# avianphysics/avian

Measured on NVIDIA H100. Metric: physics steps/sec on 100k-cube stack (broad phase + solver stage per step), higher is better.
Workload: dtype f32

## Files before the change

### avian_b200/_build.py

```python
from __future__ import annotations

import os
import shutil
import subprocess
from pathlib import Path

ROOT = Path(__file__).resolve().parent
REPO = ROOT.parent
LIB_DIR = ROOT / "lib"
CUDA_LIB = LIB_DIR / "libavian_b200.so"
HOST_LIB = LIB_DIR / "libavian_host.so"

CUDA_SOURCES = ["abi.cu", "comm.cu", "solver_host.cu", "broadphase.cu", "aabb.cu", "narrow.cu", "contacts.cu", "queries.cu", "ccd.cu"]
CUDA_HEADERS = ["avn_math.cuh", "solver_dev.cuh", "joints_dev.cuh", "solver_kernels.cuh", "context.hpp", "joint_schedule.hpp", "broadphase_cells.cuh", "narrow_math.hpp", "contact_rows.hpp", "query_math.hpp", "ccd_math.hpp", "move_math.hpp"]
GENCODE = ["-gencode", "arch=compute_90a,code=sm_90a"]
NVCC_FLAGS = [
    *GENCODE, "-lineinfo", "-O3", "-std=c++17", "-fmad=false",
    "-Xcompiler", "-fPIC", "-shared",
]
HOST_SOURCES = ["host_api.cpp"]
HOST_FLAGS = ["-O2", "-std=c++17", "-fPIC", "-shared", "-ffp-contract=off", "-Wall"]


def _newer(target: Path, deps: list[Path]) -> bool:
    if not target.exists():
        return False
    t = target.stat().st_mtime
    return all(d.stat().st_mtime <= t for d in deps if d.exists())


def find_nvcc() -> str | None:
    for cand in (os.environ.get("NVCC"), shutil.which("nvcc"), "/usr/local/cuda/bin/nvcc"):
        if cand and Path(cand).exists():
            return cand
    return None


_UNIT_HEADERS = {
    "comm.cu": ["context.hpp"],
    "aabb.cu": ["avn_math.cuh", "context.hpp"],
    "broadphase.cu": ["avn_math.cuh", "context.hpp", "broadphase_cells.cuh", "device_prims.cuh"],
    "narrow.cu": ["avn_math.cuh", "context.hpp", "narrow_math.hpp"],
    "contacts.cu": ["avn_math.cuh", "context.hpp", "narrow_math.hpp", "contact_rows.hpp", "device_prims.cuh"],
    "queries.cu": ["context.hpp", "narrow_math.hpp", "query_math.hpp", "move_math.hpp", "device_prims.cuh"],
    "ccd.cu": ["avn_math.cuh", "context.hpp", "narrow_math.hpp", "query_math.hpp", "ccd_math.hpp", "device_prims.cuh"],
}


def build_cuda(force: bool = False, verbose: bool = False) -> Path:
    src = ROOT / "csrc"
    header = REPO / "include" / "avian_b200.h"
    all_headers = sorted(p.name for p in src.glob("*.cuh")) + sorted(p.name for p in src.glob("*.hpp"))
    deps = [src / s for s in CUDA_SOURCES] + [src / h for h in all_headers] + [header]
    if not force and _newer(CUDA_LIB, deps):
        return CUDA_LIB
    nvcc = find_nvcc()
    if nvcc is None:
        if CUDA_LIB.exists():
            return CUDA_LIB
        raise RuntimeError("nvcc not found and no prebuilt libavian_b200.so: the CUDA path cannot be built")
    LIB_DIR.mkdir(exist_ok=True)
    obj_dir = LIB_DIR / "obj"
    obj_dir.mkdir(exist_ok=True)
    compile_flags = [f for f in NVCC_FLAGS if f != "-shared"]
    jobs = []
    for unit in CUDA_SOURCES:
        obj = obj_dir / (unit + ".o")
        unit_deps = [src / unit, header, Path(__file__)] + [src / h for h in _UNIT_HEADERS.get(unit, all_headers)]
        if force or not _newer(obj, unit_deps):
            jobs.append((unit, [nvcc, *compile_flags, *(["-Xptxas", "-v"] if verbose else []), "-c", "-o", str(obj), str(src / unit)]))
    if jobs:
        from concurrent.futures import ThreadPoolExecutor
        with ThreadPoolExecutor(max_workers=min(len(jobs), os.cpu_count() or 2)) as pool:
            results = list(pool.map(lambda j: (j[0], subprocess.run(j[1], cwd=src, capture_output=True, text=True)), jobs))
        for unit, r in results:
            if verbose or r.returncode != 0:
                print(f"---- {unit}\n{r.stdout}{r.stderr}")
            if r.returncode != 0:
                raise RuntimeError(f"nvcc failed on {unit}")
    subprocess.run([nvcc, "-shared", *GENCODE, "-o", str(CUDA_LIB), *[str(obj_dir / (u + ".o")) for u in CUDA_SOURCES], "-ldl"],
                   check=True, cwd=src)
    return CUDA_LIB


def build_variant(name: str, defines: list[str]) -> Path:
    build_cuda()
    nvcc = find_nvcc()
    src, obj_dir = ROOT / "csrc", LIB_DIR / "obj"
    obj = obj_dir / f"solver_host.{name}.o"
    flags = [f for f in NVCC_FLAGS if f != "-shared"]
    subprocess.run([nvcc, *flags, *[f"-D{d}" for d in defines], "-c", "-o", str(obj), str(src / "solver_host.cu")], check=True, cwd=src)
    out = LIB_DIR / f"libavian_b200_{name}.so"
    objs = [str(obj if u == "solver_host.cu" else obj_dir / (u + ".o")) for u in CUDA_SOURCES]
    subprocess.run([nvcc, "-shared", *GENCODE, "-o", str(out), *objs, "-ldl"], check=True, cwd=src)
    return out


def build_host(force: bool = False) -> Path:
    src = ROOT / "host"
    deps = [p for p in src.glob("*.[ch]pp")] + [REPO / "include" / "avian_b200.h", ROOT / "csrc" / "narrow_math.hpp", ROOT / "csrc" / "contact_rows.hpp",
            ROOT / "csrc" / "query_math.hpp", ROOT / "csrc" / "ccd_math.hpp", ROOT / "csrc" / "move_math.hpp"]
    if not force and _newer(HOST_LIB, deps):
        return HOST_LIB
    cxx = os.environ.get("CXX") or shutil.which("g++")
    if cxx is None:
        if HOST_LIB.exists():
            return HOST_LIB
        raise RuntimeError("g++ not found and no prebuilt libavian_host.so")
    LIB_DIR.mkdir(exist_ok=True)
    subprocess.run([cxx, *HOST_FLAGS, "-o", str(HOST_LIB), *[str(src / s) for s in HOST_SOURCES]], check=True, cwd=src)
    return HOST_LIB


def build_oracle(force: bool = False) -> Path:
    odir = REPO / "oracle"
    target = odir / "_build" / "liboracle.so"
    if force and target.exists():
        target.unlink()
    if shutil.which("make") and (shutil.which("g++") or os.environ.get("CXX")):
        subprocess.run(["make", "-s"], check=True, cwd=odir)
    if not target.exists():
        raise RuntimeError("oracle/_build/liboracle.so missing and cannot be built")
    return target


# ... 5 lines not shown
```

### avian_b200/csrc/broadphase.cu

```cuda
#include <algorithm>
#include <cmath>
#include <cstdlib>
#include <cstring>
#include <vector>

#include "avn_math.cuh"
#include "context.hpp"

#include "device_prims.cuh"

namespace avn {
namespace {

template <class S> struct KeyOf;
template <> struct KeyOf<float> { using type = uint32_t; static constexpr int passes = 4; };
template <> struct KeyOf<double> { using type = uint64_t; static constexpr int passes = 8; };

__device__ __forceinline__ uint32_t sortable(float f) {
    uint32_t b = __float_as_uint(f);
    if (b == 0x80000000u) b = 0;
    return (b & 0x80000000u) ? ~b : (b | 0x80000000u);
}
__device__ __forceinline__ uint64_t sortable(double f) {
    uint64_t b = (uint64_t)__double_as_longlong(f);
    if (b == 0x8000000000000000ull) b = 0;
    return (b & 0x8000000000000000ull) ? ~b : (b | 0x8000000000000000ull);
}

template <class S>
__global__ void make_keys(const S* __restrict__ aabb_min, const S* __restrict__ aabb_max, int n, typename KeyOf<S>::type* __restrict__ keys,
                          uint32_t* __restrict__ vals, unsigned long long* __restrict__ nonfinite) {
    int i = blockIdx.x * blockDim.x + threadIdx.x;
    if (i < n) {
        const S a = aabb_min[3 * i], b = aabb_min[3 * i + 1], c = aabb_min[3 * i + 2], d = aabb_max[3 * i], e = aabb_max[3 * i + 1], f = aabb_max[3 * i + 2];
        const S z = (a - a) + (b - b) + (c - c) + (d - d) + (e - e) + (f - f);
        if (!(z == S(0))) *nonfinite = 1ull;
        keys[i] = sortable(a);
        vals[i] = uint32_t(i);
    }
}

template <class S>
struct Sweep {
    int n;
    const S* minx; const S* maxx;
    const Vec4<S>* yz;
    const uint4* meta;
    const uint8_t* flags;
    const int* end;
    const uint8_t* is_wide;
    const uint64_t* existing; uint64_t existing_mask;
    const uint64_t* jdis; uint64_t jdis_mask;
};

template <class S>
__global__ void gather_sorted(const uint32_t* __restrict__ order, int n, const S* __restrict__ mn, const S* __restrict__ mx,
                              const uint32_t* __restrict__ collider, const uint32_t* __restrict__ body, const uint32_t* __restrict__ memberships,
                              const uint32_t* __restrict__ filters, const uint8_t* __restrict__ flags, S* __restrict__ minx, S* __restrict__ maxx,
                              Vec4<S>* __restrict__ yz, uint4* __restrict__ meta, uint8_t* __restrict__ sflags) {
    int r = blockIdx.x * blockDim.x + threadIdx.x;
    if (r >= n) return;
    uint32_t p = order[r];
    minx[r] = mn[3 * p];
    maxx[r] = mx[3 * p];
    yz[r] = mk4<S>(mn[3 * p + 1], mx[3 * p + 1], mn[3 * p + 2], mx[3 * p + 2]);
    meta[r] = make_uint4(collider[p], body[p], memberships ? memberships[p] : 1u, filters ? filters[p] : 0xFFFFFFFFu);
    sflags[r] = flags ? flags[p] : uint8_t(AVN_AABB_GENERATE_CONSTRAINTS);
}

constexpr int SW_WIDE = 4096;
constexpr int SW_WIDE_CAP = 1 << 14;
template <class S> struct CellGrid;
template <class S> __device__ __forceinline__ long long query_cell_count(const CellGrid<S>& g, Vec4<S> yi);
template <class S>
__global__ void sweep_bounds(const S* __restrict__ minx, const S* __restrict__ maxx, const Vec4<S>* __restrict__ yz, const CellGrid<S>* __restrict__ grid,
                             int n, int* __restrict__ end, int* __restrict__ wide_list, int* __restrict__ wide_count, uint8_t* __restrict__ is_wide,
                             const uint8_t* __restrict__ sflags) {
    int i = blockIdx.x * blockDim.x + threadIdx.x;
    if (i >= n) return;
    if (sflags[i] & AVN_AABB_HALO) {
        end[i] = i + 1;
        is_wide[i] = 0;
        return;
    }
    S m = maxx[i];
    int lo = i + 1, hi = n;
    while (lo < hi) {
        int mid = (lo + hi) >> 1;
        if (minx[mid] > m) hi = mid; else lo = mid + 1;
    }
    end[i] = lo;
    uint8_t wide = 0;
    if (lo - i - 1 > SW_WIDE && query_cell_count(*grid, yz[i]) > 32) {
        int slot = atomicAdd(wide_count, 1);
        if (slot < SW_WIDE_CAP) { wide_list[slot] = i; wide = 1; }
    }
    is_wide[i] = wide;
}

__device__ __forceinline__ uint64_t pair_key(uint32_t a, uint32_t b) {
    return a < b ? (uint64_t(a) << 32) | b : (uint64_t(b) << 32) | a;
}

template <class S>
__device__ __forceinline__ bool pair_filters(const Sweep<S>& s, uint4 mi, uint32_t fi, int j, uint32_t& pair_flags, uint4& mj) {
    mj = s.meta[j];
    uint32_t fj = s.flags[j];
    bool interacts = (mi.z & mj.w) != 0 && (mj.z & mi.w) != 0;
    if ((fi & fj & AVN_AABB_IS_INACTIVE) || !interacts || mi.y == mj.y) return false;
    if ((fj & AVN_AABB_NOT_J) || ((fi & AVN_AABB_SPLIT_I) && (fj & AVN_AABB_HALO))) return false;
    if (s.existing && hash_contains(s.existing, s.existing_mask, pair_key(mi.x, mj.x))) return false;
    if (s.jdis && hash_contains(s.jdis, s.jdis_mask, pair_key(mi.y, mj.y))) return false;
    uint32_t u = fi | fj;
    pair_flags = ((u & AVN_AABB_CONTACT_EVENTS) ? AVN_PAIR_CONTACT_EVENTS : 0u) | ((u & AVN_AABB_MODIFY_CONTACTS) ? AVN_PAIR_MODIFY_CONTACTS : 0u) |
                 ((u & AVN_AABB_GENERATE_CONSTRAINTS) ? AVN_PAIR_GENERATE_CONSTRAINTS : 0u) | ((u & AVN_AABB_CUSTOM_FILTER) ? AVN_PAIR_NEEDS_HOOK : 0u);
    return true;
}

constexpr int SW_THREADS = 256, SW_WARPS = SW_THREADS / 32;

// ... 161 lines not shown
    const uint32_t* d_collider_ = nullptr; const uint32_t* d_body_ = nullptr; const uint32_t* d_memb_ = nullptr; const uint32_t* d_filt_ = nullptr;
    const uint8_t* d_flags_ = nullptr;
    const uint64_t* d_existing_ = nullptr; uint64_t existing_mask_ = 0;
    const uint64_t* d_jdis_ = nullptr; uint64_t jdis_mask_ = 0;
    DevBuf b_min_, b_max_, b_col_, b_body_, b_memb_, b_filt_, b_flags_, b_exk_, b_ext_, b_jdk_, b_jdt_;
    DevBuf k0_, k1_, v0_, v1_, hist_;
    DevBuf s_minx_, s_maxx_, s_yz_, s_meta_, s_flags_, s_end_, counts_, offsets_, block_sums_, wide_, wide_sub_, wide_flag_, grid_, ck0_, ck1_, cv0_, cv1_, cbounds_, pairs_, stats_, stats2_;
    DevBuf o_c1_, o_c2_, o_b1_, o_b2_, o_fl_;
    uint32_t* d_order_ = nullptr;
};

template <class S>
AvnStatus Broadphase<S>::build_set(DevBuf& keys_buf, DevBuf& table_buf, const uint64_t* host_keys, uint64_t count, const uint64_t** table, uint64_t* mask) {
    *table = nullptr;
    *mask = 0;
    if (!host_keys || count == 0) return AVN_OK;
    uint64_t cap = 64;
    while (cap < count * 2) cap <<= 1;
    const uint64_t* dkeys;
    AvnStatus st = up<uint64_t>(keys_buf, host_keys, count, &dkeys);
    if (st != AVN_OK) return st;
    AVN_CUDA(table_buf.ensure(cap * sizeof(uint64_t)));
    AVN_CUDA(cudaMemsetAsync(table_buf.p, 0, cap * sizeof(uint64_t), stream_));
    hash_insert<<<unsigned((count + 255) / 256), 256, 0, stream_>>>(dkeys, count, table_buf.as<uint64_t>(), cap - 1);
    ++launches_;
    *table = table_buf.as<uint64_t>();
    *mask = cap - 1;
    return AVN_OK;
}

template <class S>
AvnStatus Broadphase<S>::upload(AvnAabbColumns* a) {
    if (!a) return err_->fail(AVN_ERR_INVALID_ARGUMENT, "aabbs is required");
    if (a->count && (!a->collider || !a->body || !a->aabb_min || !a->aabb_max))
        return err_->fail(AVN_ERR_INVALID_ARGUMENT, "aabbs: collider, body, aabb_min and aabb_max are required");
    a->retained_count = a->count;
    if (a->count > 0x7fffffffu - RS_TILE) return err_->fail(AVN_ERR_INVALID_ARGUMENT, "aabbs: too many intervals");
    uploaded_ = ran_ = false;
    launches_ = 0;
    upload_launches_ = 0;
    dropped_ = false;
    n_ = int(a->count);
    host_ = *a;
    caller_ = a;
    const size_t n = a->count;
    AvnStatus st;
#define UPB(buf, host, cnt, T, dst) if ((st = up<T>(buf, host, cnt, &dst)) != AVN_OK) return st
    UPB(b_min_, a->aabb_min, 3 * n, S, d_min_);
    UPB(b_max_, a->aabb_max, 3 * n, S, d_max_);
    UPB(b_col_, a->collider, n, uint32_t, d_collider_);
    UPB(b_body_, a->body, n, uint32_t, d_body_);
    UPB(b_memb_, a->memberships, n, uint32_t, d_memb_);
    UPB(b_filt_, a->filters, n, uint32_t, d_filt_);
    UPB(b_flags_, a->flags, n, uint8_t, d_flags_);
#undef UPB
    if ((st = build_set(b_exk_, b_ext_, a->existing_pairs, a->existing_pair_count, &d_existing_, &existing_mask_)) != AVN_OK) return st;
    if (!d_existing_ && ext_existing_) { d_existing_ = ext_existing_; existing_mask_ = ext_existing_mask_; }
    if ((st = build_set(b_jdk_, b_jdt_, a->joint_disabled_body_pairs, a->joint_disabled_pair_count, &d_jdis_, &jdis_mask_)) != AVN_OK) return st;
    upload_launches_ = launches_;
    uploaded_ = true;
    return AVN_OK;
}

template <class S>
AvnStatus Broadphase<S>::ensure_buffers(int n) {
    const int nblocks = (n + RS_TILE - 1) / RS_TILE;
    AVN_CUDA(k0_.ensure(size_t(n) * sizeof(K))); AVN_CUDA(k1_.ensure(size_t(n) * sizeof(K)));
    AVN_CUDA(v0_.ensure(size_t(n) * 4)); AVN_CUDA(v1_.ensure(size_t(n) * 4));
    AVN_CUDA(hist_.ensure(size_t(256) * nblocks * 4));
    AVN_CUDA(s_minx_.ensure(size_t(n) * sizeof(S))); AVN_CUDA(s_maxx_.ensure(size_t(n) * sizeof(S)));
    AVN_CUDA(s_yz_.ensure(size_t(n) * sizeof(Vec4<S>))); AVN_CUDA(s_meta_.ensure(size_t(n) * sizeof(uint4)));
    AVN_CUDA(s_flags_.ensure(size_t(n))); AVN_CUDA(s_end_.ensure(size_t(n) * 4));
    AVN_CUDA(counts_.ensure(size_t(n) * 4)); AVN_CUDA(offsets_.ensure((size_t(n) + 1) * 8));
    AVN_CUDA(grid_.ensure(sizeof(CellGrid<S>)));
    AVN_CUDA(ck0_.ensure(size_t(n) * 4)); AVN_CUDA(ck1_.ensure(size_t(n) * 4)); AVN_CUDA(cv0_.ensure(size_t(n) * 4)); AVN_CUDA(cv1_.ensure(size_t(n) * 4));
    AVN_CUDA(cbounds_.ensure(size_t(2) * 0x10000 * 4));
    AVN_CUDA(stats_.ensure(size_t(YZ_BLOCKS) * sizeof(YzPartial<S>)));
    AVN_CUDA(stats2_.ensure(size_t(2) * YZ_BLOCKS * sizeof(S)));
    AVN_CUDA(wide_.ensure((size_t(SW_WIDE_CAP) + 1) * 4));
    AVN_CUDA(wide_flag_.ensure(size_t(n)));
    const int nsub = (n + SW_SUB - 1) / SW_SUB;
    AVN_CUDA(wide_sub_.ensure(size_t(nsub) * size_t(std::min(n, SW_WIDE_CAP)) * 4));
    AVN_CUDA(block_sums_.ensure(size_t((n + 1023) / 1024) * 8));
    AVN_CUDA(nf_flag_.ensure(8));
    pair_capacity_ = std::max<uint64_t>(pair_capacity_, uint64_t(4) * uint64_t(n) + 1024);
    AVN_CUDA(o_c1_.ensure(pair_capacity_ * 4)); AVN_CUDA(o_c2_.ensure(pair_capacity_ * 4)); AVN_CUDA(o_b1_.ensure(pair_capacity_ * 4)); AVN_CUDA(o_b2_.ensure(pair_capacity_ * 4));
    AVN_CUDA(o_fl_.ensure(pair_capacity_));
    AVN_CUDA(pairs_.ensure(pair_capacity_ * sizeof(uint2)));
    return AVN_OK;
}

template <class S>
typename Broadphase<S>::GraphKey Broadphase<S>::graph_key() const {
    GraphKey k;
    k.n = n_;
    const void* ptrs[] = {d_min_, d_max_, d_collider_, d_body_, d_memb_, d_filt_, d_flags_, d_existing_, d_jdis_, k0_.p, k1_.p, v0_.p, v1_.p, hist_.p,
                          s_minx_.p, s_maxx_.p, s_yz_.p, s_meta_.p, s_flags_.p, s_end_.p, counts_.p, offsets_.p, grid_.p, ck0_.p};
    static_assert(sizeof ptrs == sizeof k.p, "graph key size");
    memcpy(k.p, ptrs, sizeof ptrs);
    k.m[0] = existing_mask_ ^ (uint64_t(uintptr_t(cv0_.p)) << 1) ^ (uint64_t(uintptr_t(wide_sub_.p)) << 2);
    k.m[0] ^= (pair_capacity_ * 0x9e3779b97f4a7c15ull) ^ (uint64_t(uintptr_t(pairs_.p)) << 3) ^ (uint64_t(uintptr_t(o_c1_.p)) << 4) ^ (uint64_t(uintptr_t(o_fl_.p)) << 5);
    k.m[1] = jdis_mask_ ^ (uint64_t(uintptr_t(cbounds_.p)) << 1) ^ (uint64_t(uintptr_t(block_sums_.p)) << 2) ^ (uint64_t(uintptr_t(wide_flag_.p)) << 3);
    return k;
}

template <class S>
void Broadphase<S>::enqueue_front(int n) {
    const int nblocks = (n + RS_TILE - 1) / RS_TILE;
    uint32_t launches = 0;
    K* ka = k0_.as<K>(); K* kb = k1_.as<K>();
    uint32_t* va = v0_.as<uint32_t>(); uint32_t* vb = v1_.as<uint32_t>();
    cudaMemsetAsync(nf_flag_.p, 0, 8, stream_);
    make_keys<S><<<(n + 255) / 256, 256, 0, stream_>>>(d_min_, d_max_, n, ka, va, nf_flag_.as<unsigned long long>());
    ++launches;
    for (int pass = 0; pass < KeyOf<S>::passes; ++pass) {
        const int shift = 8 * pass;
        rs_histogram<K><<<nblocks, RS_THREADS, 0, stream_>>>(ka, n, shift, hist_.as<uint32_t>(), nblocks);
        if (nblocks <= RS_FUSE_MAX_BLOCKS) {
            rs_scatter<K, true><<<nblocks, RS_THREADS, 0, stream_>>>(ka, va, n, shift, hist_.as<uint32_t>(), nblocks, kb, vb);
        } else {
            rs_scan<<<1, 1024, 0, stream_>>>(hist_.as<uint32_t>(), 256 * nblocks);
            rs_scatter<K, false><<<nblocks, RS_THREADS, 0, stream_>>>(ka, va, n, shift, hist_.as<uint32_t>(), nblocks, kb, vb);
        }
        launches += nblocks <= RS_FUSE_MAX_BLOCKS ? 2 : 3;
        std::swap(ka, kb);
        std::swap(va, vb);
    }
    d_order_ = va;
    gather_sorted<S><<<(n + 255) / 256, 256, 0, stream_>>>(d_order_, n, d_min_, d_max_, d_collider_, d_body_, d_memb_, d_filt_, d_flags_,
                                                           s_minx_.as<S>(), s_maxx_.as<S>(), s_yz_.as<Vec4<S>>(), s_meta_.as<uint4>(),
                                                           s_flags_.as<uint8_t>());
    CellGrid<S>* d_grid = grid_.as<CellGrid<S>>();
    int* cstart = cbounds_.as<int>();
    int* cend = cbounds_.as<int>() + 0x10000;
    yz_stats<S><<<YZ_BLOCKS, 256, 0, stream_>>>(s_yz_.as<Vec4<S>>(), n, stats_.as<YzPartial<S>>());
    yz_fold<S><<<1, 32, 0, stream_>>>(stats_.as<YzPartial<S>>(), YZ_BLOCKS, n, d_grid);
    yz_small_max<S><<<YZ_BLOCKS, 256, 0, stream_>>>(s_yz_.as<Vec4<S>>(), n, d_grid, stats2_.as<S>());
    yz_grid<S><<<1, 32, 0, stream_>>>(stats_.as<YzPartial<S>>(), stats2_.as<S>(), YZ_BLOCKS, n, d_grid);
    int* wide_count = wide_.as<int>();
    int* wide_list = wide_.as<int>() + 1;
    cudaMemsetAsync(wide_count, 0, 4, stream_);
    sweep_bounds<S><<<(n + 255) / 256, 256, 0, stream_>>>(s_minx_.as<S>(), s_maxx_.as<S>(), s_yz_.as<Vec4<S>>(), d_grid, n, s_end_.as<int>(), wide_list, wide_count,
                                                          wide_flag_.as<uint8_t>(), s_flags_.as<uint8_t>());
    const Sweep<S> sw = sweep_desc();
    cell_keys<S><<<(n + 255) / 256, 256, 0, stream_>>>(s_yz_.as<Vec4<S>>(), n, d_grid, ck0_.as<uint32_t>(), cv0_.as<uint32_t>());
    {
        uint32_t* cka = ck0_.as<uint32_t>(); uint32_t* ckb = ck1_.as<uint32_t>();
        uint32_t* cva = cv0_.as<uint32_t>(); uint32_t* cvb = cv1_.as<uint32_t>();
        for (int pass = 0; pass < 2; ++pass) {
            rs_histogram<uint32_t><<<nblocks, RS_THREADS, 0, stream_>>>(cka, n, 8 * pass, hist_.as<uint32_t>(), nblocks);
            if (nblocks <= RS_FUSE_MAX_BLOCKS) {
                rs_scatter<uint32_t, true><<<nblocks, RS_THREADS, 0, stream_>>>(cka, cva, n, 8 * pass, hist_.as<uint32_t>(), nblocks, ckb, cvb);
            } else {
                rs_scan<<<1, 1024, 0, stream_>>>(hist_.as<uint32_t>(), 256 * nblocks);
                rs_scatter<uint32_t, false><<<nblocks, RS_THREADS, 0, stream_>>>(cka, cva, n, 8 * pass, hist_.as<uint32_t>(), nblocks, ckb, cvb);
            }
            std::swap(cka, ckb);
            std::swap(cva, cvb);
        }
    }
    cudaMemsetAsync(cstart, 0x7f, size_t(0x10000) * 4, stream_);
    cudaMemsetAsync(cend, 0, size_t(0x10000) * 4, stream_);
    cell_bounds<<<(n + 255) / 256, 256, 0, stream_>>>(ck0_.as<uint32_t>(), n, cstart, cend);
    const CellSweep<S> cs = cell_desc();
    const int grid = std::min((n + (256 / CG_GROUP) - 1) / (256 / CG_GROUP), sm_count_ * 32);
    sweep_cells_kernel<S, false><<<grid, 256, 0, stream_>>>(sw, cs, counts_.as<uint32_t>(), nullptr, nullptr);
    const int nsub = (n + SW_SUB - 1) / SW_SUB;
    sweep_wide_kernel<S, false><<<dim3(nsub, WIDE_ROWS), SW_THREADS, 0, stream_>>>(sw, wide_list, wide_count, wide_sub_.as<uint32_t>(), nsub, nullptr, nullptr, 0);
    wide_finish<<<1, 256, 0, stream_>>>(wide_list, wide_count, wide_sub_.as<uint32_t>(), nsub, counts_.as<uint32_t>());
    launches += nblocks <= RS_FUSE_MAX_BLOCKS ? 15 : 17;
    const int sblocks = (n + 1023) / 1024;
    scan_block_sums<<<sblocks, 1024, 0, stream_>>>(counts_.as<uint32_t>(), n, block_sums_.as<uint64_t>());
    scan_block_offsets<<<1, 1024, 0, stream_>>>(block_sums_.as<uint64_t>(), sblocks, offsets_.as<uint64_t>() + n);
    scan_apply<<<sblocks, 1024, 0, stream_>>>(counts_.as<uint32_t>(), n, block_sums_.as<uint64_t>(), offsets_.as<uint64_t>());
    launches += 3;
    {
        uint2* pairs = pairs_.as<uint2>();
        sweep_cells_kernel<S, true><<<grid, 256, 0, stream_>>>(sw, cs, nullptr, offsets_.as<uint64_t>(), pairs);
        sweep_wide_kernel<S, true><<<dim3(nsub, WIDE_ROWS), SW_THREADS, 0, stream_>>>(sw, wide_list, wide_count, wide_sub_.as<uint32_t>(), nsub,
                                                                                      offsets_.as<uint64_t>(), pairs, pair_capacity_);
        segment_sort<<<(n + 255) / 256, 256, 0, stream_>>>(offsets_.as<uint64_t>(), wide_flag_.as<uint8_t>(), n, pairs, pair_capacity_);
        const unsigned mblocks = unsigned(std::min<uint64_t>((pair_capacity_ + 255) / 256, uint64_t(sm_count_) * 16));
        materialize_pairs<S><<<mblocks, 256, 0, stream_>>>(sw, pairs, offsets_.as<uint64_t>() + n, pair_capacity_, o_c1_.as<uint32_t>(), o_c2_.as<uint32_t>(),
                                                           o_b1_.as<uint32_t>(), o_b2_.as<uint32_t>(), o_fl_.as<uint8_t>());
        launches += 4;
    }
    cudaMemcpyAsync(h_total_, offsets_.as<uint64_t>() + n, sizeof(uint64_t), cudaMemcpyDeviceToHost, stream_);
    cudaMemcpyAsync(h_total_ + 1, nf_flag_.p, sizeof(uint64_t), cudaMemcpyDeviceToHost, stream_);
    front_launches_ = launches;
}

template <class S>
AvnStatus Broadphase<S>::run() {
    if (!uploaded_) return err_->fail(AVN_ERR_INVALID_ARGUMENT, "avn_broadphase_run before avn_broadphase_upload");
    const int n = n_;
    launches_ = upload_launches_;
    cudaEventRecord(ev0_, stream_);
    h_total_[0] = 0;
    h_total_[1] = 0;
    if (n > 0) {
        AvnStatus st = ensure_buffers(n);
        if (st != AVN_OK) return st;
        if (use_graph_) {
            const GraphKey key = graph_key();
            if (!graph_exec_ || !(key == graph_key_)) {
// ... 164 lines not shown
```

### avian_b200/csrc/ccd_math.hpp

```cpp
#pragma once
#include <cmath>
#include <cstdint>

#include "query_math.hpp"

namespace ccd {

using nm::S;
using nm::V3;
using nm::Q;

constexpr int CCD_MAX_ITERATIONS = 64;
constexpr double CCD_EPS_PER_LENGTH_UNIT = 1e-4;
constexpr int MODE_LINEAR = 0, MODE_NON_LINEAR = 1;

NM_HD inline void ccd_sincos(double x, double& s, double& c) {
    const double PIO2_1 = 1.57079632673412561417e+00, PIO2_1T = 6.07710050650619224932e-11, INV_PIO2 = 6.36619772367581382433e-01;
    const double k = rint(x * INV_PIO2);
    const double r = (x - k * PIO2_1) - k * PIO2_1T;
    const double r2 = r * r;
    double ps = 1.0 / 355687428096000.0;
    ps = ps * r2 - 1.0 / 1307674368000.0;
    ps = ps * r2 + 1.0 / 6227020800.0;
    ps = ps * r2 - 1.0 / 39916800.0;
    ps = ps * r2 + 1.0 / 362880.0;
    ps = ps * r2 - 1.0 / 5040.0;
    ps = ps * r2 + 1.0 / 120.0;
    ps = ps * r2 - 1.0 / 6.0;
    const double sr = r + r * (r2 * ps);
    double pc = 1.0 / 6402373705728000.0;
    pc = pc * r2 - 1.0 / 20922789888000.0;
    pc = pc * r2 + 1.0 / 87178291200.0;
    pc = pc * r2 - 1.0 / 479001600.0;
    pc = pc * r2 + 1.0 / 3628800.0;
    pc = pc * r2 - 1.0 / 40320.0;
    pc = pc * r2 + 1.0 / 720.0;
    pc = pc * r2 - 1.0 / 24.0;
    pc = pc * r2 + 0.5;
    const double cr = 1.0 - r2 * pc;
    const long long q = ((static_cast<long long>(k) % 4) + 4) % 4;
    if (q == 0) { s = sr; c = cr; }
    else if (q == 1) { s = cr; c = -sr; }
    else if (q == 2) { s = -sr; c = -cr; }
    else { s = -cr; c = sr; }
}

template <class T> struct V3T { T x, y, z; };
template <class T> struct QT { T x, y, z, w; };
template <class T> NM_HD inline T dot3(V3T<T> a, V3T<T> b) { return (a.x * b.x + a.y * b.y) + a.z * b.z; }
template <class T> NM_HD inline V3T<T> sub3(V3T<T> a, V3T<T> b) { return {a.x - b.x, a.y - b.y, a.z - b.z}; }
template <class T> NM_HD inline V3T<T> scale3(V3T<T> a, T s) { return {a.x * s, a.y * s, a.z * s}; }

template <class T> NM_HD inline QT<T> from_scaled_axis(V3T<T> v) {
    const T l = static_cast<T>(sqrt(static_cast<double>(dot3(v, v))));
    if (l == T(0)) return {T(0), T(0), T(0), T(1)};
    const V3T<T> a{v.x / l, v.y / l, v.z / l};
    double s, c;
    ccd_sincos(static_cast<double>(l * T(0.5)), s, c);
    const T ts = static_cast<T>(s), tc = static_cast<T>(c);
    return {a.x * ts, a.y * ts, a.z * ts, tc};
}
NM_HD inline QT<float> qmul(QT<float> a, QT<float> b) {
    return {(a.w * b.x + a.x * b.w) + (a.y * b.z - a.z * b.y), (a.w * b.y - a.x * b.z) + (a.y * b.w + a.z * b.x),
            (a.w * b.z + a.x * b.y) + (a.z * b.w - a.y * b.x), (a.w * b.w - a.x * b.x) + (-(a.y * b.y) - a.z * b.z)};
}
NM_HD inline QT<double> qmul(QT<double> a, QT<double> b) {
    return {a.w * b.x + a.x * b.w + a.y * b.z - a.z * b.y, a.w * b.y - a.x * b.z + a.y * b.w + a.z * b.x,
            a.w * b.z + a.x * b.y - a.y * b.x + a.z * b.w, a.w * b.w - a.x * b.x - a.y * b.y - a.z * b.z};
}

struct Motion {
    int shape;
    V3 he;
    V3 p;
    Q q;
    V3 lc;
    V3 v, w;
};

NM_HD inline S motion_radius(const Motion& m) {
    if (m.shape == nm::SHAPE_SPHERE) return nm::len(m.lc) + m.he.x;
    const V3 e{fabs(m.lc.x) + m.he.x, fabs(m.lc.y) + m.he.y, fabs(m.lc.z) + m.he.z};
    return nm::len(e);
}

NM_HD inline void pose_at(const Motion& m, S t, V3& origin, nm::M3& r) {
    const QT<double> dq = from_scaled_axis<double>({m.w.x * t, m.w.y * t, m.w.z * t});
    const QT<double> q = qmul(dq, QT<double>{m.q.x, m.q.y, m.q.z, m.q.w});
    const Q qt{q.x, q.y, q.z, q.w};
    const V3 com = (m.p + nm::rot(m.q, m.lc)) + m.v * t;
    origin = com - nm::rot(qt, m.lc);
    r = qm::rot_mat(qt);
}

NM_COLD inline S shape_distance(int sa, V3 ha, V3 ca, const nm::M3& ra, int sb, V3 hb, V3 cb, const nm::M3& rb, V3& n) {
    n = V3{0, 1, 0};
    if (sa == nm::SHAPE_SPHERE && sb == nm::SHAPE_SPHERE) {
        const V3 e = cb - ca;
        const S l = nm::len(e);
        if (l > 0) n = e * (1 / l);
        return nm::smax(l - ha.x - hb.x, 0);
    }
    if (sa == nm::SHAPE_SPHERE || sb == nm::SHAPE_SPHERE) {
        const bool box_a = sb == nm::SHAPE_SPHERE;
        const nm::Box box = box_a ? nm::Box{ca, ra, ha} : nm::Box{cb, rb, hb};
        const V3 centre = box_a ? cb : ca;
        const S r = box_a ? hb.x : ha.x;
        V3 on;
        const S l = sqrt(nm::box_point_closest(box, centre, on));
        if (l > 0) n = (box_a ? centre - on : on - centre) * (1 / l);
        return nm::smax(l - r, 0);
    }
    const V3 s = cb - ca;
    bool separated = false;
NM_ROLLED
    for (int k = 0; k < 15 && !separated; ++k) {
        const V3 L = qm::sat_axis(ra, rb, k);
        if (qm::is_zero3(L)) continue;
        separated = fabs(nm::dot(L, s)) > qm::box_extent(ra, ha, L) + qm::box_extent(rb, hb, L);
    }
    if (!separated) return 0;
    V3 on_a, on_b;
    const S l = nm::box_box_closest(nm::Box{ca, ra, ha}, nm::Box{cb, rb, hb}, on_a, on_b);
    if (l > 0) n = (on_b - on_a) * (1 / l);
    return l;
}

NM_HD inline bool nonlinear_toi(const Motion& A, const Motion& B, S t_max, S eps, S& toi, int* iterations = nullptr) {
    const V3 rel = B.v - A.v;
    const S spin = nm::len(A.w) * motion_radius(A) + nm::len(B.w) * motion_radius(B);
    S t = 0;
NM_ROLLED
    for (int it = 0; it < CCD_MAX_ITERATIONS; ++it) {
        V3 ca, cb, n;
        nm::M3 ra, rb;
        pose_at(A, t, ca, ra);
        pose_at(B, t, cb, rb);
        const S d = shape_distance(A.shape, A.he, ca, ra, B.shape, B.he, cb, rb, n);
        if (iterations) *iterations = it + 1;
        if (d != d) return false;
        if (d <= eps) { toi = t; return true; }
        const S mu = nm::smax(0, -nm::dot(rel, n)) + spin;
        if (!(mu > 0)) return false;
        t = t + d / mu;
        if (!(t <= t_max)) return false;
    }
    toi = t;
    return true;
}

NM_HD inline bool linear_toi(const Motion& A, const Motion& B, S t_max, S& toi) {
    int axis;
    return qm::cast_toi(A.shape, A.he, A.p, A.q, A.v - B.v, t_max, B.shape, B.he, B.p, B.q, toi, axis);
}

template <class T> NM_HD inline T pair_toi(int mode, const Motion& A, const Motion& B, T dt, S eps, S prediction_distance) {
    S t = 0;
    const bool hit = mode == MODE_LINEAR ? linear_toi(A, B, S(dt), t) : nonlinear_toi(A, B, S(dt), eps, t);
    if (!hit) return T(-1);
    const T tt = static_cast<T>(t);
    if (tt != T(0)) return tt;
    Motion ball = B;
    ball.shape = nm::SHAPE_SPHERE;
    ball.he = V3{prediction_distance, 0, 0};
    const bool hit2 = mode == MODE_LINEAR ? linear_toi(A, ball, S(dt), t) : nonlinear_toi(A, ball, S(dt), eps, t);
    return hit2 ? static_cast<T>(t) : T(-1);
}

template <class T> NM_HD inline bool below_thresholds(V3T<T> v1, V3T<T> w1, V3T<T> v2, V3T<T> w2, T linear_threshold, T angular_threshold) {
    const V3T<T> dw = sub3(w1, w2), dv = sub3(v1, v2);
    return dot3(dw, dw) < angular_threshold * angular_threshold && dot3(dv, dv) < linear_threshold * linear_threshold;
}

template <class T> NM_HD inline T overshoot(T min_toi) { return min_toi * T(1.0001); }

template <class T> NM_HD inline void apply_record(T m, V3T<T> v, V3T<T> w, V3T<T>& dp, QT<T>& dq) {
    dp = V3T<T>{m * v.x, m * v.y, m * v.z};
    dq = qmul(from_scaled_axis<T>(V3T<T>{w.x * m, w.y * m, w.z * m}), dq);
// ... 4 lines not shown
```

### avian_b200/csrc/contact_rows.hpp

```cpp
#pragma once
#include <cstdint>

#include "narrow_math.hpp"

namespace avn {

template <class S>
struct EdgeRows {
    int E;
    uint32_t* c1; uint32_t* c2; uint32_t* b1; uint32_t* b2; uint8_t* live;
    uint8_t* count; uint8_t* disjoint; S* normal; S* a1; S* a2; S* pen; S* ns;
    uint8_t* prev_count; double* prev_a1; double* prev_a2;
    S* ws_n_in; S* ws_t_in; S* ws_n_out; S* ws_t_out; S* nimp_in; S* nimp_out;
    const uint8_t* asleep;
};

template <class S>
struct NarrowEdgeArgs {
    EdgeRows<S> r;
    const uint8_t* shape; const S* dims; const S* pos; const S* rot; const S* lv; const S* av; const S* amin; const S* amax;
    double dt, tol, thr2;
    int match;
};

template <class S> NM_HD inline nm::V3 ldd3(const S* p, size_t i) { return {double(p[3 * i]), double(p[3 * i + 1]), double(p[3 * i + 2])}; }
template <class S> NM_HD inline void std3(S* p, size_t i, nm::V3 v) { p[3 * i] = S(v.x); p[3 * i + 1] = S(v.y); p[3 * i + 2] = S(v.z); }

template <class S>
struct BodyFrameCols { const S* pos; const S* rot; const S* com; };

template <class S>
NM_HD inline nm::PairFrames pair_frames(const BodyFrameCols<S>& f, uint32_t ba, nm::V3 pa, uint32_t bb, nm::V3 pb) {
    nm::PairFrames fr;
    fr.offset1 = pa - ldd3(f.pos, ba);
    fr.offset2 = pb - ldd3(f.pos, bb);
    fr.com1 = nm::V3{0, 0, 0};
    fr.com2 = nm::V3{0, 0, 0};
    if (f.com) {
        const nm::Q q1{double(f.rot[4 * size_t(ba)]), double(f.rot[4 * size_t(ba) + 1]), double(f.rot[4 * size_t(ba) + 2]), double(f.rot[4 * size_t(ba) + 3])};
        const nm::Q q2{double(f.rot[4 * size_t(bb)]), double(f.rot[4 * size_t(bb) + 1]), double(f.rot[4 * size_t(bb) + 2]), double(f.rot[4 * size_t(bb) + 3])};
        fr.com1 = nm::rot(q1, ldd3(f.com, ba));
        fr.com2 = nm::rot(q2, ldd3(f.com, bb));
    }
    return fr;
}

template <class S>
NM_HD inline bool capsule_row(const NarrowEdgeArgs<S>& a, int e) {
    return a.shape && a.r.live[e] && (a.shape[a.r.c1[e]] == nm::SHAPE_CAPSULE || a.shape[a.r.c2[e]] == nm::SHAPE_CAPSULE);
}

template <class S, bool CAPSULES = true, bool FRAMES = false>
NM_HD inline void narrow_edge_row(const NarrowEdgeArgs<S>& a, int e, const BodyFrameCols<S>& f = BodyFrameCols<S>{}) {
    const EdgeRows<S>& r = a.r;
    if (r.asleep && r.asleep[e]) return;
    if (!r.live[e]) { r.count[e] = 0; r.disjoint[e] = 0; return; }
    const uint32_t ca = r.c1[e], cb = r.c2[e], ba = r.b1[e], bb = r.b2[e];
    int np = 0;
    nm::V3 normal{0, 0, 0};
    nm::PointOut out[4];
    bool disjoint = false;
    {
        const nm::V3 mina = ldd3(a.amin, ca), maxa = ldd3(a.amax, ca), minb = ldd3(a.amin, cb), maxb = ldd3(a.amax, cb);
        disjoint = (mina.x > maxb.x || maxa.x < minb.x || mina.y > maxb.y || maxa.y < minb.y || mina.z > maxb.z || maxa.z < minb.z);
    }
    r.disjoint[e] = disjoint ? 1 : 0;
    if (!disjoint) {
        const nm::V3 pa = ldd3(a.pos, ca), pb = ldd3(a.pos, cb);
        const nm::Q qa{double(a.rot[4 * size_t(ca)]), double(a.rot[4 * size_t(ca) + 1]), double(a.rot[4 * size_t(ca) + 2]), double(a.rot[4 * size_t(ca) + 3])};
        const nm::Q qb{double(a.rot[4 * size_t(cb)]), double(a.rot[4 * size_t(cb) + 1]), double(a.rot[4 * size_t(cb) + 2]), double(a.rot[4 * size_t(cb) + 3])};
        const nm::V3 v1 = ldd3(a.lv, ba), v2 = ldd3(a.lv, bb), w1 = ldd3(a.av, ba), w2 = ldd3(a.av, bb);
        const nm::V3 rel = v2 - v1;
        const double eff_margin = a.dt * nm::len(rel);
        const double max_dist = nm::smax(eff_margin, a.tol);
        nm::Contacts pts;
        const int ta = a.shape ? a.shape[ca] : nm::SHAPE_CUBOID, tb = a.shape ? a.shape[cb] : nm::SHAPE_CUBOID;
        if (nm::collide<CAPSULES>(ta, ldd3(a.dims, ca), pa, qa, tb, ldd3(a.dims, cb), pb, qb, max_dist, normal, pts)) {
            if (FRAMES) np = nm::manifold_points(pts, normal, pa, pb, rel, w1, w2, a.dt, eff_margin, pair_frames(f, ba, pa, bb, pb), out);
            else np = nm::manifold_points(pts, normal, pa, pb, rel, w1, w2, a.dt, eff_margin, out);
        } else
            normal = nm::V3{0, 0, 0};
    }
    const int oc = r.prev_count[e];
    nm::V3 oa1[4], oa2[4];
    S on[4], otx[4], oty[4];
    for (int k = 0; k < oc; ++k) {
        const size_t q = size_t(e) * 4 + k;
        oa1[k] = nm::V3{r.prev_a1[3 * q], r.prev_a1[3 * q + 1], r.prev_a1[3 * q + 2]};
        oa2[k] = nm::V3{r.prev_a2[3 * q], r.prev_a2[3 * q + 1], r.prev_a2[3 * q + 2]};
        on[k] = r.ws_n_out[q]; otx[k] = r.ws_t_out[2 * q]; oty[k] = r.ws_t_out[2 * q + 1];
    }
    r.count[e] = uint8_t(np);
    std3(r.normal, size_t(e), normal);
    for (int k = 0; k < 4; ++k) {
        const size_t q = size_t(e) * 4 + k;
        S vn = S(0), vx = S(0), vy = S(0);
        if (k < np) {
            const int j = a.match ? nm::match_point(out[k].anchor1, out[k].anchor2, oa1, oa2, oc, a.thr2) : -1;
            if (j >= 0) { vn = on[j]; vx = otx[j]; vy = oty[j]; }
            std3(r.a1, q, out[k].anchor1);
            std3(r.a2, q, out[k].anchor2);
            r.pen[q] = S(out[k].penetration);
            r.ns[q] = S(out[k].normal_speed);
            r.prev_a1[3 * q] = out[k].anchor1.x; r.prev_a1[3 * q + 1] = out[k].anchor1.y; r.prev_a1[3 * q + 2] = out[k].anchor1.z;
            r.prev_a2[3 * q] = out[k].anchor2.x; r.prev_a2[3 * q + 1] = out[k].anchor2.y; r.prev_a2[3 * q + 2] = out[k].anchor2.z;
        } else {
            std3(r.a1, q, nm::V3{0, 0, 0});
            std3(r.a2, q, nm::V3{0, 0, 0});
            r.pen[q] = S(0);
            r.ns[q] = S(0);
        }
        r.ws_n_in[q] = vn;
        r.ws_t_in[2 * q] = vx;
        r.ws_t_in[2 * q + 1] = vy;
        r.ws_n_out[q] = vn;
        r.ws_t_out[2 * q] = vx;
        r.ws_t_out[2 * q + 1] = vy;
    }
    r.prev_count[e] = uint8_t(np);
}


}
```

### avian_b200/csrc/contacts.cu

```cuda
#include <cooperative_groups.h>

#include <algorithm>
#include <cstdlib>
#include <cstring>

#include "context.hpp"
#include "contact_rows.hpp"
#include "device_prims.cuh"

namespace avn {
namespace {
namespace cg = cooperative_groups;

enum { CH_NONE = 0, CH_PUSH = 1, CH_POP = 2, CH_REMOVE = 3, CH_MASK = 3, CH_DONE = 0x10 };
enum { ISL_NONE = 0, ISL_ADD = 1, ISL_REMOVE = 2 };

struct GraphCounters {
    uint32_t removed, started, stopped, changed, rounds, ovf_dirty, manifolds, any_restitution, aborted, bad_pairs;
    uint32_t rows_woken, rows_slept, bodies_asleep;
    uint32_t round_left[3];
    uint32_t color_offsets[AVN_GRAPH_COLOR_COUNT + 1];
    uint32_t ovf_count;
    uint32_t rows_asleep;
};
// ... 282 lines not shown
        if (S(re) != S(0)) g.ctr->any_restitution = 1;
    }
}

__global__ void pair_set_kernel(GraphRows g, uint64_t* __restrict__ table, uint64_t mask) {
    const int e = blockIdx.x * blockDim.x + threadIdx.x;
    if (e >= g.hw || !g.live[e]) return;
    const uint32_t a = g.c1[e], b = g.c2[e];
    const uint64_t k = (a < b ? (uint64_t(a) << 32) | b : (uint64_t(b) << 32) | a) + 1;
    uint64_t h = hash64(k) & mask;
    for (;;) {
        unsigned long long prev = atomicCAS((unsigned long long*)&table[h], 0ull, (unsigned long long)k);
        if (prev == 0ull || prev == k) return;
        h = (h + 1) & mask;
    }
}

__global__ void event_keys_kernel(const uint8_t* __restrict__ event, int n, uint32_t* __restrict__ keys, uint32_t* __restrict__ vals) {
    const int e = blockIdx.x * blockDim.x + threadIdx.x;
    if (e >= n) return;
    const uint8_t v = event[e];
    keys[e] = (v & EV_STARTED) ? 0u : (v & EV_ENDED) ? 1u : 2u;
    vals[e] = uint32_t(e);
}
__global__ void report_keys_kernel(GraphRows g, uint32_t flags, uint32_t* __restrict__ keys, uint32_t* __restrict__ vals) {
    const int e = blockIdx.x * blockDim.x + threadIdx.x;
    if (e >= g.hw) return;
    const bool sel = g.live[e] && g.touching[e] && (!(flags & AVN_REPORT_EVENTS_ONLY) || (g.pflags[e] & AVN_PAIR_CONTACT_EVENTS));
    keys[e] = sel ? 0u : 1u;
    vals[e] = uint32_t(e);
}
__global__ void key_bounds_kernel(const uint32_t* __restrict__ sorted_keys, int n, int nb, uint32_t* __restrict__ out) {
    const int k = threadIdx.x + 1;
    if (k > nb) return;
    int lo = 0, hi = n;
    while (lo < hi) { const int mid = (lo + hi) >> 1; if (sorted_keys[mid] < uint32_t(k)) lo = mid + 1; else hi = mid; }
    out[k - 1] = uint32_t(lo);
}
__global__ void event_gather_kernel(GraphRows g, const uint32_t* __restrict__ list, uint32_t n_started, uint32_t n, uint32_t skip, uint32_t N,
                                    uint32_t* __restrict__ out) {
    const uint32_t i = blockIdx.x * blockDim.x + threadIdx.x;
    if (i >= n) return;
    const uint32_t e = list[i], j = i < n_started ? i : i + skip;
    out[j] = g.c1[e]; out[N + j] = g.c2[e]; out[2 * size_t(N) + j] = g.b1[e]; out[3 * size_t(N) + j] = g.b2[e];
    reinterpret_cast<uint8_t*>(out + 4 * size_t(N))[j] = g.event[e] & EV_FLAGS;
}
__global__ void mark_colliders_kernel(const uint32_t* __restrict__ ids, uint32_t n, uint8_t* __restrict__ removed) {
    const uint32_t k = blockIdx.x * blockDim.x + threadIdx.x;
    if (k < n) removed[ids[k]] = 1;
}
__global__ void queue_ends_kernel(GraphRows g, const uint32_t* __restrict__ list, uint32_t n, uint32_t base, uint32_t cap, uint32_t* __restrict__ pend) {
    const uint32_t i = blockIdx.x * blockDim.x + threadIdx.x;
    if (i >= n) return;
    const uint32_t e = list[i], j = base + i;
    pend[j] = g.c1[e]; pend[cap + j] = g.c2[e]; pend[2 * size_t(cap) + j] = g.b1[e]; pend[3 * size_t(cap) + j] = g.b2[e];
    reinterpret_cast<uint8_t*>(pend + 4 * size_t(cap))[j] = g.pflags[e] & EV_FLAGS;
}
template <class S>
__global__ void report_gather_kernel(GraphRows g, const uint32_t* __restrict__ list, uint32_t n, const S* __restrict__ normal, const S* __restrict__ pen,
                                     const S* __restrict__ nimp, void* __restrict__ out) {
    const uint32_t i = blockIdx.x * blockDim.x + threadIdx.x;
    if (i >= n) return;
    const uint32_t e = list[i];
    S* os = static_cast<S*>(out);
    uint32_t* ou = reinterpret_cast<uint32_t*>(os + 6 * size_t(n));
    uint8_t* ob = reinterpret_cast<uint8_t*>(ou + 5 * size_t(n));
    const int cnt = g.count[e];
    const bool solved = g.colour[e] != 0 || g.asleep[e] != 0;
    S total = S(0), mx = S(0), deep = S(0);
    for (int k = 0; k < cnt; ++k) {
        const S v = solved ? nimp[4 * size_t(e) + k] : S(0);
        total = total + v;
        if (v > mx) mx = v;
        const S p = pen[4 * size_t(e) + k];
        if (k == 0 || p >= deep) deep = p;
    }
    for (int c = 0; c < 3; ++c) os[3 * size_t(i) + c] = normal[3 * size_t(e) + c];
    os[3 * size_t(n) + i] = total; os[4 * size_t(n) + i] = mx; os[5 * size_t(n) + i] = deep;
    ou[i] = e; ou[n + i] = g.c1[e]; ou[2 * size_t(n) + i] = g.c2[e]; ou[3 * size_t(n) + i] = g.b1[e]; ou[4 * size_t(n) + i] = g.b2[e];
    ob[i] = g.pflags[e] & EV_FLAGS; ob[n + i] = uint8_t(cnt);
}

template <class S>
__global__ void __launch_bounds__(128) narrow_edges_kernel(const __grid_constant__ NarrowEdgeArgs<S> a, uint8_t* fresh, int only_fresh, int capsules) {
    const int e = blockIdx.x * blockDim.x + threadIdx.x;
    if (e >= a.r.E) return;
    if (capsules && capsule_row(a, e)) return;
    if (only_fresh) {
        if (!fresh[e]) return;
        fresh[e] = 0;
    }
    narrow_edge_row<S, false>(a, e);
}

template <class S>
__global__ void __launch_bounds__(128) narrow_capsule_edges_kernel(const __grid_constant__ NarrowEdgeArgs<S> a, uint8_t* fresh, int only_fresh) {
    const int e = blockIdx.x * blockDim.x + threadIdx.x;
    if (e >= a.r.E || !capsule_row(a, e)) return;
    if (only_fresh) {
        if (!fresh[e]) return;
        fresh[e] = 0;
    }
    narrow_edge_row<S, true>(a, e);
}

template <class S, bool CAPSULES>
__global__ void __launch_bounds__(128) narrow_framed_edges_kernel(const __grid_constant__ NarrowEdgeArgs<S> a, const BodyFrameCols<S> f, uint8_t* fresh,
                                                                  int only_fresh, int capsules) {
    const int e = blockIdx.x * blockDim.x + threadIdx.x;
    if (e >= a.r.E) return;
    if (capsules && capsule_row(a, e) != CAPSULES) return;
    if (only_fresh) {
        if (!fresh[e]) return;
        fresh[e] = 0;
    }
    narrow_edge_row<S, CAPSULES, true>(a, e, f);
}


struct IslandCounters {
    uint32_t islands, sleeping, put_to_sleep, woken, split_bodies, merges, split_root;
    uint32_t absorbed;
    unsigned long long cand;
};
constexpr uint32_t ISL_NONE_BODY = 0xffffffffu;

struct IslandState {
    int B;
    const uint8_t* kind;
    uint32_t* parent; uint32_t* root; uint32_t* root_prev; uint32_t* removed;
    uint8_t* isl_sleeping; uint8_t* awake; uint8_t* need_wake; uint8_t* touched; uint8_t* in_split;
    float* timer;
    const float* thr_lin; const float* thr_ang; const uint8_t* disabled; const uint8_t* host_wake;
    uint32_t* cand_body;
    IslandCounters* ctr;
    float time_to_sleep, delta_secs;
};
__device__ __forceinline__ bool isl_static(const IslandState& s, uint32_t b) { return b >= uint32_t(s.B) || s.kind[b] == AVN_BODY_STATIC; }
__device__ __forceinline__ uint32_t isl_find(uint32_t* parent, uint32_t x) {
    uint32_t p = *reinterpret_cast<volatile uint32_t*>(&parent[x]);
    while (p != x) {
        const uint32_t gp = *reinterpret_cast<volatile uint32_t*>(&parent[p]);
        if (gp != p) parent[x] = gp;
        x = p; p = gp;
    }
    return x;
}
__device__ __forceinline__ bool isl_union(uint32_t* parent, uint32_t u, uint32_t v) {
    for (;;) {
        uint32_t ru = isl_find(parent, u), rv = isl_find(parent, v);
        if (ru == rv) return false;
        if (ru < rv) { const uint32_t t = ru; ru = rv; rv = t; }
        if (atomicCAS(&parent[ru], ru, rv) == ru) return true;
    }
}
__global__ void isl_init_kernel(IslandState s) {
    const int b = blockIdx.x * blockDim.x + threadIdx.x;
    if (b >= s.B) return;
    s.parent[b] = uint32_t(b); s.root[b] = uint32_t(b); s.root_prev[b] = uint32_t(b); s.removed[b] = 0;
    s.isl_sleeping[b] = 0; s.awake[b] = 0; s.need_wake[b] = 0; s.touched[b] = 0; s.in_split[b] = 0; s.timer[b] = 0.f;
    if (b == 0) { *s.cand_body = ISL_NONE_BODY; }
}
__global__ void isl_joint_kernel(IslandState s, const uint32_t* __restrict__ j1, const uint32_t* __restrict__ j2, int J, int only_split) {
    const int j = blockIdx.x * blockDim.x + threadIdx.x;
    if (j >= J) return;
    const uint32_t a = j1[j], b = j2[j];
    if (isl_static(s, a) || isl_static(s, b)) return;
    if (only_split && !(s.in_split[a] && s.in_split[b])) return;
    isl_union(s.parent, a, b);
}
__global__ void isl_link_existing_kernel(IslandState s, GraphRows g) {
    const int e = blockIdx.x * blockDim.x + threadIdx.x;
    if (e >= g.hw || !g.live[e] || !g.touching[e] || !(g.pflags[e] & AVN_PAIR_GENERATE_CONSTRAINTS)) return;
    const uint32_t a = g.b1[e], b = g.b2[e];
    if (!isl_static(s, a) && !isl_static(s, b)) isl_union(s.parent, a, b);
}
__global__ void isl_add_kernel(IslandState s, GraphRows g) {
    const int e = blockIdx.x * blockDim.x + threadIdx.x;
    if (e >= g.hw || g.isl_event[e] != ISL_ADD) return;
    const uint32_t a = g.b1[e], b = g.b2[e];
    const bool sa = isl_static(s, a), sb = isl_static(s, b);
    if (!sa) s.touched[a] = 1;
    if (!sb) s.touched[b] = 1;
    if (!sa && !sb && isl_union(s.parent, a, b)) atomicAdd(&s.ctr->merges, 1u);
}
__global__ void isl_flatten_kernel(IslandState s, int split_only) {
    const int b = blockIdx.x * blockDim.x + threadIdx.x;
    if (b >= s.B || isl_static(s, uint32_t(b))) return;
    if (split_only) {
        if (!s.in_split[b]) return;
        s.root[b] = isl_find(s.parent, uint32_t(b));
        s.removed[b] = 0;
        return;
    }
    const uint32_t r = isl_find(s.parent, uint32_t(b));
    s.root[b] = r;
    if (s.root_prev[b] == uint32_t(b) && r != uint32_t(b)) {
        if (s.removed[b]) { atomicAdd(&s.removed[r], s.removed[b]); s.removed[b] = 0; }
        if (s.isl_sleeping[b]) { s.isl_sleeping[b] = 0; s.need_wake[r] = 1; s.touched[b] = 1; atomicAdd(&s.ctr->absorbed, 1u); }
// ... 742 lines not shown
                      {&prev_a2_, 12 * sizeof(double)}, {&ws_n_in_, 4 * sizeof(S)}, {&ws_t_in_, 8 * sizeof(S)}, {&ws_n_out_, 4 * sizeof(S)},
                      {&ws_t_out_, 8 * sizeof(S)}, {&nimp_in_, 4 * sizeof(S)}, {&nimp_out_, 4 * sizeof(S)},
                      {&pflags_, 1}, {&touching_, 1}, {&colour_, 1}, {&change_, 1}, {&old_colour_, 1}, {&ovf_pos_, 4}, {&ovf_, 4}, {&isl_event_, 1}, {&fresh_, 1},
                      {&event_, 1}, {&asleep_, 1}};
        for (Col& c : cols) {
            void* fresh = nullptr;
            AVN_CUDA(cudaMalloc(&fresh, n * c.bytes_per_row));
            AVN_CUDA(cudaMemsetAsync(fresh, 0, n * c.bytes_per_row, stream_));
            if (c.buf->p && E_) AVN_CUDA(cudaMemcpyAsync(fresh, c.buf->p, size_t(E_) * c.bytes_per_row, cudaMemcpyDeviceToDevice, stream_));
            AVN_CUDA(cudaStreamSynchronize(stream_));
            if (c.buf->p) cudaFree(c.buf->p);
            c.buf->p = fresh;
            c.buf->cap = n * c.bytes_per_row;
        }
        E_ = capacity;
        const size_t nblocks = (n + RS_TILE - 1) / RS_TILE;
        AVN_CUDA(k0_.ensure(n * 4)); AVN_CUDA(k1_.ensure(n * 4)); AVN_CUDA(v0_.ensure(n * 4)); AVN_CUDA(v1_.ensure(n * 4)); AVN_CUDA(list_.ensure(n * 4));
        AVN_CUDA(evl_.ensure(n * 4));
        AVN_CUDA(hist_.ensure(256 * nblocks * 4));
        AVN_CUDA(m_b1_.ensure(n * 4)); AVN_CUDA(m_b2_.ensure(n * 4)); AVN_CUDA(m_fr_.ensure(n * sizeof(S))); AVN_CUDA(m_re_.ensure(n * sizeof(S)));
        uint64_t cap = 1024;
        while (cap < uint64_t(n) * 2) cap <<= 1;
        AVN_CUDA(table_.ensure(cap * sizeof(uint64_t)));
        table_mask_ = cap - 1;
        table_dirty_ = true;
        return AVN_OK;
    }
    AvnStatus upload_inputs(const AvnNarrowInput* in, bool keep_shapes, cudaStream_t s) {
        const size_t C = in->collider_count, B = in->body_count;
        if (!in->dims || !in->position || !in->rotation || !in->linear_velocity || !in->angular_velocity || !in->aabb_min || !in->aabb_max)
            return err_->fail(AVN_ERR_INVALID_ARGUMENT, "contacts_step: dims, position, rotation, velocities and AABBs are required");
        keep_shapes = keep_shapes && in_.colliders == C && in_.dims != nullptr;
        AvnStatus st;
        up_stream_ = s;
#define UPC(buf, host, cnt, T, dst) if ((st = up<T>(buf, host, cnt, &dst)) != AVN_OK) { up_stream_ = stream_; return st; }
        if (!keep_shapes) {
            UPC(i_shape_, in->shape, C, uint8_t, in_.shape);
            UPC(i_dims_, in->dims, 3 * C, S, in_.dims);
            if (checked_ == in) has_capsule_ = checked_capsule_;
        }
        UPC(i_pos_, in->position, 3 * C, S, in_.pos);
        UPC(i_rot_, in->rotation, 4 * C, S, in_.rot);
        UPC(i_lv_, in->linear_velocity, 3 * B, S, in_.lv);
        UPC(i_av_, in->angular_velocity, 3 * B, S, in_.av);
        UPC(i_amin_, in->aabb_min, 3 * C, S, in_.amin);
        UPC(i_amax_, in->aabb_max, 3 * C, S, in_.amax);
        in_.framed = frames_set_;
        if (frames_set_) {
            UPC(i_fpos_, frames_.position.data(), 3 * B, S, in_.frames.pos);
            UPC(i_frot_, frames_.rotation.data(), 4 * B, S, in_.frames.rot);
            UPC(i_fcom_, frames_.com.empty() ? nullptr : frames_.com.data(), 3 * B, S, in_.frames.com);
        }
#undef UPC
        up_stream_ = stream_;
        in_.colliders = C;
        return AVN_OK;
    }
    AvnStatus launch_narrow(const AvnNarrowParams* prm, const AvnNarrowInput* in, uint32_t match_contacts, double length_unit, uint32_t n) {
        bool only_fresh = false;
        if (prefetched_ == in) {
            AVN_CUDA(cudaStreamWaitEvent(stream_, ev_in_, 0));
            only_fresh = early_rows_ > 0;
            if (only_fresh && n == early_rows_ && !added_this_step_) { prefetched_ = nullptr; early_rows_ = 0; return AVN_OK; }
        } else {
            if (prefetched_) AVN_CUDA(cudaStreamWaitEvent(stream_, ev_in_, 0));
            AvnStatus st = upload_inputs(in, false, stream_);
            if (st != AVN_OK) return st;
        }
        prefetched_ = nullptr;
        early_rows_ = 0;
        AvnStatus st = enqueue_narrow(prm, match_contacts, length_unit, n, stream_, only_fresh);
        if (st == AVN_OK && !only_fresh && n) AVN_CUDA(cudaMemsetAsync(fresh_.p, 0, n, stream_));
        return st;
    }
    AvnStatus enqueue_narrow(const AvnNarrowParams* prm, uint32_t match_contacts, double length_unit, uint32_t n, cudaStream_t s, bool only_fresh) {
        NarrowEdgeArgs<S> a{};
        a.r = rows();
        a.r.E = int(n);
        a.shape = in_.shape; a.dims = in_.dims; a.pos = in_.pos; a.rot = in_.rot; a.lv = in_.lv; a.av = in_.av; a.amin = in_.amin; a.amax = in_.amax;
        a.dt = prm->dt;
        a.tol = prm->contact_tolerance;
        a.thr2 = (0.1 * length_unit) * (0.1 * length_unit);
        a.match = match_contacts ? 1 : 0;
        if (in_.framed) {
            narrow_framed_edges_kernel<S, false><<<(n + 127) / 128, 128, 0, s>>>(a, in_.frames, fresh_.as<uint8_t>(), only_fresh ? 1 : 0, has_capsule_ ? 1 : 0);
            if (has_capsule_) narrow_framed_edges_kernel<S, true><<<(n + 127) / 128, 128, 0, s>>>(a, in_.frames, fresh_.as<uint8_t>(), only_fresh ? 1 : 0, 1);
        } else {
            narrow_edges_kernel<S><<<(n + 127) / 128, 128, 0, s>>>(a, fresh_.as<uint8_t>(), only_fresh ? 1 : 0, has_capsule_ ? 1 : 0);
            if (has_capsule_) narrow_capsule_edges_kernel<S><<<(n + 127) / 128, 128, 0, s>>>(a, fresh_.as<uint8_t>(), only_fresh ? 1 : 0);
        }
        AVN_CUDA(cudaGetLastError());
        return AVN_OK;
    }
    void radix_pass(int n, uint32_t* vals_out = nullptr) {
        uint32_t* vo = vals_out ? vals_out : v1_.as<uint32_t>();
        const int nblocks = (n + RS_TILE - 1) / RS_TILE;
        rs_histogram<uint32_t><<<nblocks, RS_THREADS, 0, stream_>>>(k0_.as<uint32_t>(), n, 0, hist_.as<uint32_t>(), nblocks);
        if (nblocks <= RS_FUSE_MAX_BLOCKS) {
            rs_scatter<uint32_t, true><<<nblocks, RS_THREADS, 0, stream_>>>(k0_.as<uint32_t>(), v0_.as<uint32_t>(), n, 0, hist_.as<uint32_t>(), nblocks, k1_.as<uint32_t>(), vo);
        } else {
            rs_scan<<<1, 1024, 0, stream_>>>(hist_.as<uint32_t>(), 256 * nblocks);
            rs_scatter<uint32_t, false><<<nblocks, RS_THREADS, 0, stream_>>>(k0_.as<uint32_t>(), v0_.as<uint32_t>(), n, 0, hist_.as<uint32_t>(), nblocks, k1_.as<uint32_t>(), vo);
        }
    }
    AvnStatus small_bounds(int nb, uint32_t* out) {
        AVN_CUDA(bounds_.ensure(16));
        key_bounds_kernel<<<1, 32, 0, stream_>>>(k1_.as<uint32_t>(), int(hw_), nb, bounds_.as<uint32_t>());
        AVN_CUDA(cudaGetLastError());
        AVN_CUDA(cudaMemcpyAsync(out, bounds_.p, size_t(nb) * 4, cudaMemcpyDeviceToHost, stream_));
        AVN_CUDA(cudaStreamSynchronize(stream_));
        return AVN_OK;
    }
    AvnStatus pend_reserve(int i, uint32_t need) {
        if (need <= pend_cap_[i]) return AVN_OK;
        const uint32_t cap = std::max(need, std::max(2 * pend_cap_[i], 256u)), old = pend_cap_[i];
        void* p = nullptr;
        AVN_CUDA(cudaMalloc(&p, size_t(cap) * 17));
        if (pend_n_[i]) {
            const uint32_t* src = pend_[i].as<uint32_t>();
            uint32_t* dst = static_cast<uint32_t*>(p);
            for (int c = 0; c < 4; ++c)
                AVN_CUDA(cudaMemcpyAsync(dst + size_t(c) * cap, src + size_t(c) * old, size_t(pend_n_[i]) * 4, cudaMemcpyDeviceToDevice, stream_));
            AVN_CUDA(cudaMemcpyAsync(dst + 4 * size_t(cap), src + 4 * size_t(old), pend_n_[i], cudaMemcpyDeviceToDevice, stream_));
            AVN_CUDA(cudaStreamSynchronize(stream_));
        }
        if (pend_[i].p) cudaFree(pend_[i].p);
        pend_[i].p = p;
        pend_[i].cap = size_t(cap) * 17;
        pend_cap_[i] = cap;
        return AVN_OK;
    }
    AvnStatus remove_rows(uint32_t n, const uint32_t* colliders) {
        if (n == 0 || hw_ == 0) return AVN_OK;
        AVN_CUDA(rm_.ensure(std::max<size_t>(n_colliders_, 1)));
        AVN_CUDA(cudaMemsetAsync(rm_.p, 0, std::max<size_t>(n_colliders_, 1), stream_));
        AVN_CUDA(stage_.ensure(size_t(n) * 4));
        AVN_CUDA(cudaMemcpyAsync(stage_.p, colliders, size_t(n) * 4, cudaMemcpyHostToDevice, stream_));
        mark_colliders_kernel<<<(n + 255) / 256, 256, 0, stream_>>>(stage_.as<uint32_t>(), n, rm_.as<uint8_t>());
        AVN_CUDA(cudaMemsetAsync(ctr_.p, 0, offsetof(GraphCounters, ovf_count), stream_));
        GraphRows g = graph_rows();
        const unsigned rb = (hw_ + 255) / 256;
        const int islands = !isl_configured_ ? 0 : (isl_pending_ && !(apply_ && wake_done_)) ? 2 : 1;
        remove_rows_kernel<<<rb, 256, 0, stream_>>>(g, rm_.as<uint8_t>(), isl_, islands, k0_.as<uint32_t>(), v0_.as<uint32_t>());
        radix_pass(int(hw_), evl_.as<uint32_t>());
        AVN_CUDA(cudaMemcpyAsync(h_ctr_, ctr_.p, sizeof(GraphCounters), cudaMemcpyDeviceToHost, stream_));
        AVN_CUDA(cudaStreamSynchronize(stream_));
        const uint32_t n_rm = h_ctr_->removed, n_end = h_ctr_->stopped;
        if (n_rm == 0) return AVN_OK;
        AvnStatus st = pend_reserve(pend_cur_, pend_n_[pend_cur_] + n_end);
        if (st != AVN_OK) return st;
        if (n_end) {
            queue_ends_kernel<<<(n_end + 255) / 256, 256, 0, stream_>>>(g, evl_.as<uint32_t>(), n_end, pend_n_[pend_cur_], pend_cap_[pend_cur_],
                                                                         pend_[pend_cur_].as<uint32_t>());
            pend_n_[pend_cur_] += n_end;
        }
        overflow_list_kernel<<<1, 32, 0, stream_>>>(g, evl_.as<uint32_t>());
        rebuild_list(g);
        AVN_CUDA(cudaMemsetAsync(table_.p, 0, (table_mask_ + 1) * sizeof(uint64_t), stream_));
        pair_set_kernel<<<rb, 256, 0, stream_>>>(g, table_.as<uint64_t>(), table_mask_);
        AVN_CUDA(cudaGetLastError());
        table_dirty_ = false;
        AVN_CUDA(cudaMemcpyAsync(h_ctr_, ctr_.p, sizeof(GraphCounters), cudaMemcpyDeviceToHost, stream_));
        AVN_CUDA(cudaStreamSynchronize(stream_));
        live_n_ -= n_rm;
        rows_asleep_ = h_ctr_->rows_asleep;
        take_list_counters();
        return AVN_OK;
    }
    AvnStatus apply_pass(bool wakes, bool sleeps) {
        AVN_CUDA(cudaMemsetAsync(ctr_.p, 0, offsetof(GraphCounters, ovf_count), stream_));
        GraphRows g = graph_rows();
        uint8_t* body_asleep = body_asleep_.as<uint8_t>();
// ... 151 lines not shown
```

### avian_b200/csrc/device_prims.cuh

```cuda
#pragma once
#include <cstdint>

namespace avn {
namespace {

constexpr int RS_THREADS = 256;
constexpr int RS_WARPS = RS_THREADS / 32;
constexpr int RS_ROUNDS = 8;
constexpr int RS_TILE = RS_THREADS * RS_ROUNDS;

template <class K>
__global__ void __launch_bounds__(RS_THREADS) rs_histogram(const K* __restrict__ keys, int n, int shift, uint32_t* __restrict__ hist, int nblocks) {
    __shared__ uint32_t cnt[256];
    cnt[threadIdx.x] = 0;
    __syncthreads();
    const int base = blockIdx.x * RS_TILE;
#pragma unroll
    for (int r = 0; r < RS_ROUNDS; ++r) {
        int i = base + r * RS_THREADS + threadIdx.x;
        if (i < n) atomicAdd(&cnt[(keys[i] >> shift) & 0xff], 1u);
    }
    __syncthreads();
    hist[threadIdx.x * nblocks + blockIdx.x] = cnt[threadIdx.x];
}

constexpr int RS_SCAN_ITEMS = 16;
__global__ void __launch_bounds__(1024) rs_scan(uint32_t* data, int len) {
    __shared__ uint32_t warp_sums[32];
    __shared__ uint32_t carry;
    if (threadIdx.x == 0) carry = 0;
    __syncthreads();
    for (int base = 0; base < len; base += 1024 * RS_SCAN_ITEMS) {
        const int i0 = base + threadIdx.x * RS_SCAN_ITEMS;
        uint32_t item[RS_SCAN_ITEMS];
        uint32_t v = 0;
#pragma unroll
        for (int k = 0; k < RS_SCAN_ITEMS; ++k) {
            item[k] = (i0 + k < len) ? data[i0 + k] : 0u;
            v += item[k];
        }
        uint32_t x = v;
#pragma unroll
        for (int o = 1; o < 32; o <<= 1) {
            uint32_t y = __shfl_up_sync(0xffffffffu, x, o);
            if ((threadIdx.x & 31) >= o) x += y;
        }
        if ((threadIdx.x & 31) == 31) warp_sums[threadIdx.x >> 5] = x;
        __syncthreads();
        if (threadIdx.x < 32) {
            uint32_t w = warp_sums[threadIdx.x], z = w;
#pragma unroll
            for (int o = 1; o < 32; o <<= 1) {
                uint32_t y = __shfl_up_sync(0xffffffffu, z, o);
                if (threadIdx.x >= o) z += y;
            }
            warp_sums[threadIdx.x] = z - w;
        }
        __syncthreads();
        uint32_t run = x - v + warp_sums[threadIdx.x >> 5] + carry;
#pragma unroll
        for (int k = 0; k < RS_SCAN_ITEMS; ++k) {
            if (i0 + k < len) data[i0 + k] = run;
            run += item[k];
        }
        __syncthreads();
        if (threadIdx.x == 1023) carry = run;
        __syncthreads();
    }
}

constexpr int RS_FUSE_MAX_BLOCKS = 128;
template <class K, bool FUSED>
__global__ void __launch_bounds__(RS_THREADS) rs_scatter(const K* __restrict__ keys_in, const uint32_t* __restrict__ vals_in, int n, int shift,
                                                         const uint32_t* __restrict__ offsets, int nblocks, K* __restrict__ keys_out,
                                                         uint32_t* __restrict__ vals_out) {
    __shared__ uint32_t wcnt[RS_WARPS][256];
    __shared__ uint32_t digit_base[256];
    __shared__ uint32_t scan_warp[8];
    if (FUSED) {
        const int d = threadIdx.x;
        uint32_t total = 0, before_blk = 0;
        const uint32_t* row = offsets + size_t(d) * nblocks;
        for (int b = 0; b < nblocks; ++b) {
            const uint32_t c = row[b];
            total += c;
            if (b < int(blockIdx.x)) before_blk += c;
        }
        uint32_t x = total;
#pragma unroll
        for (int o = 1; o < 32; o <<= 1) {
            uint32_t y = __shfl_up_sync(0xffffffffu, x, o);
            if ((threadIdx.x & 31) >= o) x += y;
        }
        if ((threadIdx.x & 31) == 31) scan_warp[threadIdx.x >> 5] = x;
        __syncthreads();
        uint32_t warp_before = 0;
        for (int w = 0; w < (threadIdx.x >> 5); ++w) warp_before += scan_warp[w];
        digit_base[d] = (x - total) + warp_before + before_blk;
    }
    const int warp = threadIdx.x >> 5, lane = threadIdx.x & 31;
    for (int d = threadIdx.x; d < RS_WARPS * 256; d += RS_THREADS) (&wcnt[0][0])[d] = 0;
    __syncthreads();
    const int base = blockIdx.x * RS_TILE + warp * (32 * RS_ROUNDS);
    K key[RS_ROUNDS];
    uint32_t val[RS_ROUNDS], rank[RS_ROUNDS];
#pragma unroll
    for (int r = 0; r < RS_ROUNDS; ++r) {
        int i = base + r * 32 + lane;
        bool ok = i < n;
        key[r] = ok ? keys_in[i] : K(0);
        val[r] = ok ? vals_in[i] : 0u;
        uint32_t digit = uint32_t(key[r] >> shift) & 0xff;
        uint32_t active = __ballot_sync(0xffffffffu, ok);
        uint32_t same = __match_any_sync(0xffffffffu, ok ? digit : 0x100u + lane) & active;
        uint32_t before = __popc(same & ((1u << lane) - 1u));
        uint32_t prev = ok ? wcnt[warp][digit] : 0u;
        rank[r] = prev + before;
        __syncwarp();
        if (ok && before == 0) wcnt[warp][digit] = prev + __popc(same);
        __syncwarp();
    }
    __syncthreads();
    {
        const int d = threadIdx.x;
        uint32_t run = FUSED ? digit_base[d] : offsets[d * nblocks + blockIdx.x];
#pragma unroll
        for (int w = 0; w < RS_WARPS; ++w) {
            uint32_t c = wcnt[w][d];
            wcnt[w][d] = run;
            run += c;
        }
    }
    __syncthreads();
#pragma unroll
    for (int r = 0; r < RS_ROUNDS; ++r) {
        int i = base + r * 32 + lane;
        if (i < n) {
            uint32_t digit = uint32_t(key[r] >> shift) & 0xff;
            uint32_t pos = wcnt[warp][digit] + rank[r];
            keys_out[pos] = key[r];
            vals_out[pos] = val[r];
        }
    }
}

__device__ __forceinline__ uint64_t block_exclusive_scan_1024(uint64_t v, uint64_t* warp_sums, uint64_t& block_total) {
    uint64_t x = v;
#pragma unroll
    for (int o = 1; o < 32; o <<= 1) {
        uint64_t y = __shfl_up_sync(0xffffffffu, x, o);
        if ((threadIdx.x & 31) >= o) x += y;
    }
    if ((threadIdx.x & 31) == 31) warp_sums[threadIdx.x >> 5] = x;
    __syncthreads();
    if (threadIdx.x < 32) {
        uint64_t w = warp_sums[threadIdx.x], z = w;
#pragma unroll
        for (int o = 1; o < 32; o <<= 1) {
// ... 71 lines not shown
```

### avian_b200/csrc/move_math.hpp

```cpp
#pragma once
#include <cmath>
#include <cstdint>

#include "narrow_math.hpp"
#include "query_math.hpp"

namespace mv {

using nm::Q;
using nm::V3;

constexpr int MAX_PLANES = 32;
constexpr int MOVE_WINDOW = 16;
constexpr double DOT_EPSILON = 0.005;
constexpr double MIN_DISTANCE = 1e-4;

template <class T> struct T3 { T x, y, z; };
template <class T> NM_HD inline T3<T> add(T3<T> a, T3<T> b) { return {a.x + b.x, a.y + b.y, a.z + b.z}; }
template <class T> NM_HD inline T3<T> sub(T3<T> a, T3<T> b) { return {a.x - b.x, a.y - b.y, a.z - b.z}; }
template <class T> NM_HD inline T3<T> neg(T3<T> a) { return {-a.x, -a.y, -a.z}; }
template <class T> NM_HD inline T3<T> scale(T s, T3<T> a) { return {s * a.x, s * a.y, s * a.z}; }
template <class T> NM_HD inline T3<T> divs(T3<T> a, T s) { return {a.x / s, a.y / s, a.z / s}; }
template <class T> NM_HD inline T dot(T3<T> a, T3<T> b) { return a.x * b.x + a.y * b.y + a.z * b.z; }
template <class T> NM_HD inline T3<T> cross(T3<T> a, T3<T> b) { return {a.y * b.z - b.y * a.z, a.z * b.x - b.z * a.x, a.x * b.y - b.x * a.y}; }
template <class T> NM_HD inline T3<T> wide(T3<float> a) { return {T(a.x), T(a.y), T(a.z)}; }
template <class T> NM_HD inline T3<float> narrow(T3<T> a) { return {float(a.x), float(a.y), float(a.z)}; }
template <class T> NM_HD inline V3 to_v3(T3<T> a) { return V3{double(a.x), double(a.y), double(a.z)}; }
template <class T> NM_HD inline T3<T> from_v3(V3 a) { return {T(a.x), T(a.y), T(a.z)}; }
template <class T> NM_HD inline T smax0(T a) { return a < T(0) ? T(0) : a; }
template <class T> NM_HD inline bool total_lt(T a, T b) { return a < b || (a == b && std::signbit(a) && !std::signbit(b)); }

template <class T>
struct Config {
    T dt, length_unit, skin_width, max_depenetration_error, penetration_rejection_threshold, plane_similarity_dot_threshold;
    uint32_t iterations, depenetration_iterations, max_planes;
};

template <class T>
NM_HD inline T3<T> project_velocity(T3<T> v, const T3<float>* normals, int n) {
    const T eps = T(DOT_EPSILON);
    const T3<T> x0 = neg(v);
    int kind = 0;
    T3<float> n1{0, 0, 0}, n2{0, 0, 0};
    T3<T> sv = x0;
    int iters = 0;
    for (;;) {
        if (dot(sv, sv) < eps * eps) break;
        if (n == 0) break;
        int bi = 0;
        T best = dot(wide<T>(normals[0]), sv);
        for (int k = 1; k < n; ++k) {
            const T d = dot(wide<T>(normals[k]), sv);
            if (!total_lt(d, best)) { best = d; bi = k; }
        }
        if (best <= eps) break;
        const T3<float> nd = normals[bi];
        const T3<T> ndv = wide<T>(nd);
        if (kind == 0) {
            const T d = dot(ndv, x0);
            sv = sub(x0, scale(d, ndv));
            n1 = nd;
            kind = 1;
        } else if (kind == 1) {
            const T3<T> c = cross(ndv, wide<T>(n1));
            const T d = dot(x0, c);
            sv = divs(scale(d, c), dot(c, c));
            if (d > T(0)) { n2 = n1; n1 = nd; } else { n2 = nd; }
            kind = 2;
        } else {
            const T3<T> c1 = cross(wide<T>(n1), ndv);
            const T c1sq = dot(c1, c1), d1 = dot(x0, c1);
            const T3<T> c2 = cross(ndv, wide<T>(n2));
            const T c2sq = dot(c2, c2), d2 = dot(x0, c2);
            if (d1 <= T(0) && d2 <= T(0)) { sv = T3<T>{0, 0, 0}; break; }
            if (d1 * std::fabs(d1) * c2sq > d2 * std::fabs(d2) * c1sq) {
                sv = divs(scale(d1, c1), c1sq);
                n2 = nd;
            } else {
                sv = divs(scale(d2, c2), c2sq);
                n1 = nd;
            }
        }
        if (++iters >= 10) break;
    }
    return neg(sv);
}

template <class T>
NM_COLD inline bool contact_plane(int sa, V3 ha, V3 pa, Q qa, int sb, V3 hb, V3 pb, Q qb, double prediction, T3<float>& normal, T& penetration) {
    V3 n;
    nm::Contacts pts;
    if (!nm::collide<false>(sa, ha, pa, qa, sb, hb, pb, qb, prediction, n, pts) || pts.n == 0) return false;
    T best = T(nm::dot(pts.p[0].a - pts.p[0].b, n));
    for (int k = 1; k < pts.n; ++k) {
        const T p = T(nm::dot(pts.p[k].a - pts.p[k].b, n));
        if (!(p < best)) best = p;
    }
    penetration = best;
    normal = T3<float>{float(-n.x), float(-n.y), float(-n.z)};
    return true;
}

template <class T> NM_HD inline T3<float> plane_dir(T3<T> p) { const T3<float> f = narrow(p); return divs(f, std::sqrt(dot(f, f))); }

struct Body { int shape; V3 he; Q q; };

template <class T>
NM_HD inline void grown_aabb(const Body& b, T3<T> pos, T grow, T lo[3], T hi[3]) {
    V3 mn, mx;
    qm::collider_aabb(b.shape, b.he, to_v3(pos), b.q, mn, mx);
    lo[0] = T(mn.x) - grow; lo[1] = T(mn.y) - grow; lo[2] = T(mn.z) - grow;
    hi[0] = T(mx.x) + grow; hi[1] = T(mx.y) + grow; hi[2] = T(mx.z) + grow;
}

template <class T, class Scene, class Fn>
NM_HD inline void intersections(const Scene& sc, const Body& b, T3<T> pos, T pred, Fn fn) {
    T lo[3], hi[3];
    grown_aabb(b, pos, pred, lo, hi);
    const V3 p = to_v3(pos);
    sc.candidates(lo, hi, [&](uint32_t c) {
        int s;
        V3 he, cp;
        Q cq;
        sc.collider(c, s, he, cp, cq);
        T3<float> n;
        T pen;
        if (contact_plane<T>(b.shape, b.he, p, b.q, s, he, cp, cq, double(pred), n, pen)) fn(n, pen);
    });
}

template <class T, class Scene>
NM_HD inline T3<T> depenetrate(const Scene& sc, const Config<T>& cfg, const Body& b, T3<T> pos) {
    T3<T> fixup{0, 0, 0};
    if (cfg.depenetration_iterations == 0) return fixup;
    const T skin = cfg.length_unit * cfg.skin_width;
    const T reject = cfg.length_unit * cfg.penetration_rejection_threshold;
    const T target = cfg.length_unit * cfg.max_depenetration_error;
    T3<float> ln[MOVE_WINDOW];
    T ld[MOVE_WINDOW];
    uint32_t count = 0;
    intersections<T>(sc, b, pos, skin, [&](T3<float> n, T pen) {
        if (count < uint32_t(MOVE_WINDOW)) { ln[count] = n; ld[count] = pen + skin; }
        ++count;
    });
    const bool kept = count <= uint32_t(MOVE_WINDOW);
    T total = T(0);
    auto relax = [&](T3<float> n, T dist) {
        if (dist > reject) return;
        const T3<T> nv = wide<T>(n);
        const T err = smax0(dist - dot(fixup, nv));
        total += err;
        fixup = add(fixup, scale(err, nv));
    };
NM_ROLLED
    for (uint32_t it = 0; it < cfg.depenetration_iterations; ++it) {
        total = T(0);
        if (kept) {
            for (uint32_t k = 0; k < count; ++k) relax(ln[k], ld[k]);
        } else {
            intersections<T>(sc, b, pos, skin, [&](T3<float> n, T pen) { relax(n, pen + skin); });
        }
        if (total < target) break;
    }
    return fixup;
}

template <class T, class Scene, class Hits>
NM_HD inline void move_and_slide(const Scene& sc, const Config<T>& cfg, const Body& b, T3<T>& pos, T3<T>& vel, const T3<float>* init, int n_init,
                                 Hits& hits) {
    T time_left = cfg.dt;
    const T skin = cfg.length_unit * cfg.skin_width;
    pos = add(pos, depenetrate(sc, cfg, b, pos));
    T3<float> planes[MAX_PLANES + 1];
NM_ROLLED
    for (uint32_t it = 0; it < cfg.iterations; ++it) {
        const T3<T> sweep = scale(time_left, vel);
        const T3<float> sf = narrow(sweep);
        const float lf = std::sqrt(dot(sf, sf));
// ... 95 lines not shown
```

### avian_b200/csrc/narrow.cu

```cuda
#include "context.hpp"
#include "contact_rows.hpp"

namespace avn {
namespace {

template <class S>
struct NarrowArgs {
    int n;
    const uint32_t* c1; const uint32_t* c2; const uint32_t* b1; const uint32_t* b2;
    const uint8_t* shape; const S* dims; const S* pos; const S* rot;
    const S* lv; const S* av;
    const S* amin; const S* amax;
    uint8_t* count; uint8_t* disjoint; S* normal; S* anchor1; S* anchor2; S* penetration; S* normal_speed;
    double dt, tol;
};

template <class S> __device__ __forceinline__ nm::V3 ld3(const S* p, uint32_t i) { return {double(p[3 * i]), double(p[3 * i + 1]), double(p[3 * i + 2])}; }
template <class S> __device__ __forceinline__ void st3(S* p, size_t i, nm::V3 v) { p[3 * i] = S(v.x); p[3 * i + 1] = S(v.y); p[3 * i + 2] = S(v.z); }

template <class S, bool CAPSULES, bool FRAMES = false>
__device__ __forceinline__ void narrow_pair(const NarrowArgs<S>& a, int capsules, const BodyFrameCols<S>& f = BodyFrameCols<S>{}) {
    const int k = blockIdx.x * blockDim.x + threadIdx.x;
    if (k >= a.n) return;
    const uint32_t ca = a.c1[k], cb = a.c2[k], ba = a.b1[k], bb = a.b2[k];
    if (capsules && (a.shape[ca] == nm::SHAPE_CAPSULE || a.shape[cb] == nm::SHAPE_CAPSULE) != CAPSULES) return;
    a.count[k] = 0;
    if (a.amin) {
        const nm::V3 mina = ld3(a.amin, ca), maxa = ld3(a.amax, ca), minb = ld3(a.amin, cb), maxb = ld3(a.amax, cb);
        const bool overlap = !(mina.x > maxb.x || maxa.x < minb.x || mina.y > maxb.y || maxa.y < minb.y || mina.z > maxb.z || maxa.z < minb.z);
        a.disjoint[k] = overlap ? 0 : 1;
        if (!overlap) return;
    } else if (a.disjoint) {
        a.disjoint[k] = 0;
    }
    const nm::V3 pa = ld3(a.pos, ca), pb = ld3(a.pos, cb);
    const nm::Q qa{double(a.rot[4 * ca]), double(a.rot[4 * ca + 1]), double(a.rot[4 * ca + 2]), double(a.rot[4 * ca + 3])};
    const nm::Q qb{double(a.rot[4 * cb]), double(a.rot[4 * cb + 1]), double(a.rot[4 * cb + 2]), double(a.rot[4 * cb + 3])};
    const nm::V3 v1 = ld3(a.lv, ba), v2 = ld3(a.lv, bb), w1 = ld3(a.av, ba), w2 = ld3(a.av, bb);
    const nm::V3 rel = v2 - v1;
    const double eff_margin = a.dt * nm::len(rel);
    const double max_dist = nm::smax(eff_margin, a.tol);
    nm::V3 normal;
    nm::Contacts pts;
    const int ta = a.shape ? a.shape[ca] : nm::SHAPE_CUBOID, tb = a.shape ? a.shape[cb] : nm::SHAPE_CUBOID;
    if (!nm::collide<CAPSULES>(ta, ld3(a.dims, ca), pa, qa, tb, ld3(a.dims, cb), pb, qb, max_dist, normal, pts)) return;
    nm::PointOut out[4];
    const int np = FRAMES ? nm::manifold_points(pts, normal, pa, pb, rel, w1, w2, a.dt, eff_margin, pair_frames(f, ba, pa, bb, pb), out)
                          : nm::manifold_points(pts, normal, pa, pb, rel, w1, w2, a.dt, eff_margin, out);
    a.count[k] = uint8_t(np);
    st3(a.normal, k, normal);
    for (int p = 0; p < np; ++p) {
        st3(a.anchor1, size_t(4) * k + p, out[p].anchor1);
        st3(a.anchor2, size_t(4) * k + p, out[p].anchor2);
        a.penetration[size_t(4) * k + p] = S(out[p].penetration);
        a.normal_speed[size_t(4) * k + p] = S(out[p].normal_speed);
    }
}

template <class S>
__global__ void __launch_bounds__(128) narrow_phase_kernel(const __grid_constant__ NarrowArgs<S> a, int capsules) { narrow_pair<S, false>(a, capsules); }
template <class S>
__global__ void __launch_bounds__(128) narrow_capsule_kernel(const __grid_constant__ NarrowArgs<S> a) { narrow_pair<S, true>(a, 1); }
template <class S, bool CAPSULES>
__global__ void __launch_bounds__(128) narrow_framed_kernel(const __grid_constant__ NarrowArgs<S> a, const BodyFrameCols<S> f, int capsules) {
    narrow_pair<S, CAPSULES, true>(a, capsules, f);
}

template <class S>
class Narrow final : public NarrowBase {
   public:
    Narrow(cudaStream_t stream, ErrorSink* err) : stream_(stream), err_(err) {}
    AvnStatus run(const AvnNarrowParams* prm, const AvnNarrowInput* in, AvnRawManifolds* out, const BodyFrames* frames) override {
        if (!prm || !in || !out) return err_->fail(AVN_ERR_INVALID_ARGUMENT, "params, input and output are required");
        const size_t n = in->pair_count, C = in->collider_count, B = in->body_count;
        if (n == 0) return AVN_OK;
        if (!in->collider1 || !in->collider2 || !in->body1 || !in->body2 || !in->dims || !in->position || !in->rotation || !in->linear_velocity ||
            !in->angular_velocity)
            return err_->fail(AVN_ERR_INVALID_ARGUMENT, "narrow phase: pair columns, dims, position, rotation and the body velocities are required");
        if (!out->point_count || !out->normal || !out->anchor1 || !out->anchor2 || !out->penetration || !out->normal_speed)
            return err_->fail(AVN_ERR_INVALID_ARGUMENT, "narrow phase: every output column except disjoint is required");
        if ((in->aabb_min == nullptr) != (in->aabb_max == nullptr)) return err_->fail(AVN_ERR_INVALID_ARGUMENT, "narrow phase: aabb_min and aabb_max go together");
        if (frames && frames->body_count != B)
            return err_->fail(AVN_ERR_INVALID_ARGUMENT, "narrow phase: the body frames have %u bodies, the input %zu", frames->body_count, B);
        for (size_t k = 0; k < n; ++k)
            if (in->collider1[k] >= C || in->collider2[k] >= C || in->body1[k] >= B || in->body2[k] >= B)
                return err_->fail(AVN_ERR_INVALID_ARGUMENT, "narrow phase: pair %zu indexes past the collider / body columns", k);
        size_t at = 0;
        bool capsules = false;
        if (const char* why = check_shape_column(in->shape, in->dims, C, sizeof(S) == 8 ? 64 : 32, &at, &capsules))
            return err_->fail(AVN_ERR_INVALID_ARGUMENT, "narrow phase: collider %zu: %s", at, why);
        NarrowArgs<S> a{};
        a.n = int(n);
        AvnStatus st;
#define UPN(buf, host, cnt, T, dst) if ((st = up<T>(buf, host, cnt, &dst)) != AVN_OK) return st
        UPN(i_c1_, in->collider1, n, uint32_t, a.c1);
        UPN(i_c2_, in->collider2, n, uint32_t, a.c2);
        UPN(i_b1_, in->body1, n, uint32_t, a.b1);
        UPN(i_b2_, in->body2, n, uint32_t, a.b2);
        UPN(i_shape_, in->shape, C, uint8_t, a.shape);
        UPN(i_dims_, in->dims, 3 * C, S, a.dims);
        UPN(i_pos_, in->position, 3 * C, S, a.pos);
        UPN(i_rot_, in->rotation, 4 * C, S, a.rot);
        UPN(i_lv_, in->linear_velocity, 3 * B, S, a.lv);
        UPN(i_av_, in->angular_velocity, 3 * B, S, a.av);
        UPN(i_amin_, in->aabb_min, 3 * C, S, a.amin);
        UPN(i_amax_, in->aabb_max, 3 * C, S, a.amax);
        BodyFrameCols<S> f{};
        if (frames) {
            UPN(i_fpos_, frames->position.data(), 3 * B, S, f.pos);
            UPN(i_frot_, frames->rotation.data(), 4 * B, S, f.rot);
            if (!frames->com.empty()) UPN(i_fcom_, frames->com.data(), 3 * B, S, f.com);
        }
#undef UPN
        AVN_CUDA(o_cnt_.ensure(n));
        AVN_CUDA(o_dis_.ensure(n));
        AVN_CUDA(o_nrm_.ensure(3 * n * sizeof(S)));
        AVN_CUDA(o_a1_.ensure(12 * n * sizeof(S)));
        AVN_CUDA(o_a2_.ensure(12 * n * sizeof(S)));
        AVN_CUDA(o_pen_.ensure(4 * n * sizeof(S)));
        AVN_CUDA(o_ns_.ensure(4 * n * sizeof(S)));
        a.count = o_cnt_.as<uint8_t>(); a.disjoint = o_dis_.as<uint8_t>(); a.normal = o_nrm_.as<S>(); a.anchor1 = o_a1_.as<S>(); a.anchor2 = o_a2_.as<S>();
        a.penetration = o_pen_.as<S>(); a.normal_speed = o_ns_.as<S>();
        a.dt = prm->dt;
        a.tol = prm->contact_tolerance;
        AVN_CUDA(cudaMemsetAsync(a.normal, 0, 3 * n * sizeof(S), stream_));
        AVN_CUDA(cudaMemsetAsync(a.anchor1, 0, 12 * n * sizeof(S), stream_));
        AVN_CUDA(cudaMemsetAsync(a.anchor2, 0, 12 * n * sizeof(S), stream_));
        AVN_CUDA(cudaMemsetAsync(a.penetration, 0, 4 * n * sizeof(S), stream_));
        AVN_CUDA(cudaMemsetAsync(a.normal_speed, 0, 4 * n * sizeof(S), stream_));
        if (frames) {
            narrow_framed_kernel<S, false><<<unsigned((n + 127) / 128), 128, 0, stream_>>>(a, f, capsules ? 1 : 0);
            if (capsules) narrow_framed_kernel<S, true><<<unsigned((n + 127) / 128), 128, 0, stream_>>>(a, f, 1);
        } else {
            narrow_phase_kernel<S><<<unsigned((n + 127) / 128), 128, 0, stream_>>>(a, capsules ? 1 : 0);
            if (capsules) narrow_capsule_kernel<S><<<unsigned((n + 127) / 128), 128, 0, stream_>>>(a);
        }
        AVN_CUDA(cudaGetLastError());
        AVN_CUDA(cudaMemcpyAsync(out->point_count, a.count, n, cudaMemcpyDeviceToHost, stream_));
        if (out->disjoint) AVN_CUDA(cudaMemcpyAsync(out->disjoint, a.disjoint, n, cudaMemcpyDeviceToHost, stream_));
        AVN_CUDA(cudaMemcpyAsync(out->normal, a.normal, 3 * n * sizeof(S), cudaMemcpyDeviceToHost, stream_));
        AVN_CUDA(cudaMemcpyAsync(out->anchor1, a.anchor1, 12 * n * sizeof(S), cudaMemcpyDeviceToHost, stream_));
        AVN_CUDA(cudaMemcpyAsync(out->anchor2, a.anchor2, 12 * n * sizeof(S), cudaMemcpyDeviceToHost, stream_));
        AVN_CUDA(cudaMemcpyAsync(out->penetration, a.penetration, 4 * n * sizeof(S), cudaMemcpyDeviceToHost, stream_));
        AVN_CUDA(cudaMemcpyAsync(out->normal_speed, a.normal_speed, 4 * n * sizeof(S), cudaMemcpyDeviceToHost, stream_));
        AVN_CUDA(cudaStreamSynchronize(stream_));
        return AVN_OK;
    }

   private:
    template <class T> AvnStatus up(DevBuf& buf, const void* host, size_t count, const T** dev) {
        *dev = nullptr;
        if (!host || count == 0) return AVN_OK;
        AVN_CUDA(buf.ensure(count * sizeof(T)));
        AVN_CUDA(cudaMemcpyAsync(buf.p, host, count * sizeof(T), cudaMemcpyHostToDevice, stream_));
        *dev = buf.as<T>();
        return AVN_OK;
    }
    cudaStream_t stream_;
    ErrorSink* err_;
    DevBuf i_c1_, i_c2_, i_b1_, i_b2_, i_shape_, i_dims_, i_pos_, i_rot_, i_lv_, i_av_, i_amin_, i_amax_, i_fpos_, i_frot_, i_fcom_;
    DevBuf o_cnt_, o_dis_, o_nrm_, o_a1_, o_a2_, o_pen_, o_ns_;
};

}

NarrowBase* make_narrow(uint32_t scalar_bits, cudaStream_t stream, ErrorSink* err) {
    if (scalar_bits == 32) return new Narrow<float>(stream, err);
    if (scalar_bits == 64) return new Narrow<double>(stream, err);
    return nullptr;
}

}
```

### avian_b200/csrc/narrow_math.hpp

```cpp
#pragma once
#include <cmath>

#if defined(__CUDACC__)
#define NM_HD __host__ __device__
#define NM_COLD __host__ __device__ __noinline__
#define NM_ROLLED _Pragma("unroll 1")
#else
#define NM_HD
#define NM_COLD
#define NM_ROLLED
#endif

namespace nm {

using S = double;

struct V3 { S x, y, z; };
NM_HD inline V3 operator+(V3 a, V3 b) { return {a.x + b.x, a.y + b.y, a.z + b.z}; }
NM_HD inline V3 operator-(V3 a, V3 b) { return {a.x - b.x, a.y - b.y, a.z - b.z}; }
NM_HD inline V3 operator-(V3 a) { return {-a.x, -a.y, -a.z}; }
NM_HD inline V3 operator*(V3 a, S s) { return {a.x * s, a.y * s, a.z * s}; }
NM_HD inline S dot(V3 a, V3 b) { return a.x * b.x + a.y * b.y + a.z * b.z; }
NM_HD inline V3 cross(V3 a, V3 b) { return {a.y * b.z - a.z * b.y, a.z * b.x - a.x * b.z, a.x * b.y - a.y * b.x}; }
NM_HD inline S len(V3 a) { return sqrt(dot(a, a)); }
NM_HD inline S comp(V3 a, int i) { return i == 0 ? a.x : (i == 1 ? a.y : a.z); }
NM_HD inline S smax(S a, S b) { return a < b ? b : a; }
NM_HD inline S smin(S a, S b) { return b < a ? b : a; }

struct Q { S x, y, z, w; };
NM_HD inline V3 rot(Q q, V3 v) {
    V3 b{q.x, q.y, q.z};
    S b2 = dot(b, b);
    return v * (q.w * q.w - b2) + b * (dot(v, b) * 2) + cross(b, v) * (q.w * 2);
}
struct M3 { V3 c[3]; };
NM_HD inline M3 to_mat(Q q) { return {{rot(q, {1, 0, 0}), rot(q, {0, 1, 0}), rot(q, {0, 0, 1})}}; }

enum ShapeType { SHAPE_CUBOID = 0, SHAPE_SPHERE = 1, SHAPE_CAPSULE = 2 };
struct Box { V3 c; M3 r; V3 he; };

constexpr int MAX_RAW_POINTS = 8;
struct Witness { V3 a, b; };
struct Contacts {
    int n;
    Witness p[MAX_RAW_POINTS];
    NM_HD void clear() { n = 0; }
    NM_HD void push(V3 on_a, V3 on_b) { p[n].a = on_a; p[n].b = on_b; ++n; }
};

NM_HD inline void box_face(const Box& b, int axis, S sign, V3 out[4]) {
    int u = (axis + 1) % 3, v = (axis + 2) % 3;
    V3 n = b.r.c[axis] * (sign * comp(b.he, axis));
    V3 eu = b.r.c[u] * comp(b.he, u), ev = b.r.c[v] * comp(b.he, v);
    V3 fc = b.c + n;
    out[0] = fc + eu + ev; out[1] = fc - eu + ev; out[2] = fc - eu - ev; out[3] = fc + eu - ev;
}

NM_HD inline int clip_poly(const V3* in, int n, V3 plane_n, S plane_d, V3* out) {
    int m = 0;
    for (int i = 0; i < n; ++i) {
        V3 a = in[i], b = in[(i + 1) % n];
        S da = dot(plane_n, a) - plane_d, db = dot(plane_n, b) - plane_d;
        if (da <= 0) out[m++] = a;
        if ((da < 0 && db > 0) || (da > 0 && db < 0)) out[m++] = a + (b - a) * (da / (da - db));
    }
    return m;
}

NM_HD inline S box_radius(const Box& b, V3 n) {
    return fabs(dot(b.r.c[0], n)) * b.he.x + fabs(dot(b.r.c[1], n)) * b.he.y + fabs(dot(b.r.c[2], n)) * b.he.z;
}

NM_HD inline bool segment_closest(V3 p, V3 u, S hu, V3 q, V3 w, S hw, S& s, S& t) {
    V3 r = p - q;
    S a = dot(u, u), e = dot(w, w), f = dot(w, r), c = dot(u, r), b = dot(u, w);
    S den = a * e - b * b;
    S s0 = den > 1e-12 ? (b * f - c * e) / den : 0;
    s = smax(-hu, smin(hu, s0));
    bool end = den <= 1e-12 || s != s0;
    t = (b * s + f) / e;
    if (t < -hw || t > hw) {
        t = t < -hw ? -hw : hw;
        s = smax(-hu, smin(hu, (b * t - c) / a));
        end = true;
    }
    return end;
}

NM_HD inline S box_point_closest(const Box& b, V3 p, V3& on) {
    V3 d = p - b.c;
    on = b.c;
    for (int k = 0; k < 3; ++k) on = on + b.r.c[k] * smax(-comp(b.he, k), smin(comp(b.he, k), dot(d, b.r.c[k])));
    V3 e = p - on;
    return dot(e, e);
}

NM_COLD inline S box_box_closest(const Box& A, const Box& B, V3& on_a, V3& on_b) {
    S best = 1e300;
NM_ROLLED
    for (int side = 0; side < 2; ++side) {
        const Box& P = side == 0 ? A : B;
        const Box& O = side == 0 ? B : A;
NM_ROLLED
        for (int m = 0; m < 8; ++m) {
            V3 v = P.c + P.r.c[0] * (m & 1 ? P.he.x : -P.he.x) + P.r.c[1] * (m & 2 ? P.he.y : -P.he.y) + P.r.c[2] * (m & 4 ? P.he.z : -P.he.z);
            V3 on;
            S d2 = box_point_closest(O, v, on);
            if (d2 < best) { best = d2; on_a = side == 0 ? v : on; on_b = side == 0 ? on : v; }
        }
    }
    auto edge_mid = [](const Box& b, int k, int m) {
        int u = (k + 1) % 3, v = (k + 2) % 3;
        return b.c + b.r.c[u] * (m & 1 ? comp(b.he, u) : -comp(b.he, u)) + b.r.c[v] * (m & 2 ? comp(b.he, v) : -comp(b.he, v));
    };
NM_ROLLED
    for (int ei = 0; ei < 12; ++ei) {
        const int i = ei >> 2, mi = ei & 3;
        V3 pa = edge_mid(A, i, mi);
NM_ROLLED
        for (int ej = 0; ej < 12; ++ej) {
            const int j = ej >> 2, mj = ej & 3;
            V3 pb = edge_mid(B, j, mj);
            S s, t;
            segment_closest(pa, A.r.c[i], comp(A.he, i), pb, B.r.c[j], comp(B.he, j), s, t);
            V3 qa = pa + A.r.c[i] * s, qb = pb + B.r.c[j] * t, e = qb - qa;
            S d2 = dot(e, e);
            if (d2 < best) { best = d2; on_a = qa; on_b = qb; }
        }
    }
    return sqrt(best);
}

NM_HD inline bool closest_pair(V3 on_a, V3 on_b, S dist, S max_dist, V3& normal, Contacts& pts) {
    pts.clear();
    if (dist > max_dist) return false;
    if (dist > 1e-12) normal = (on_b - on_a) * (1 / dist);
    pts.push(on_a, on_b);
    return true;
}

constexpr S FACE_GAP_SLACK = 1e-4;

NM_HD inline bool box_box(const Box& A, const Box& B, S max_dist, V3& normal, Contacts& pts) {
    pts.clear();
    V3 d = B.c - A.c;
    S best_sep = -1e300;
    int best_kind = -1, best_i = 0, best_j = 0;
    V3 best_n{0, 1, 0};
    auto consider = [&](V3 n, int kind, int i, int j, S bias) {
        S l = len(n);
        if (l < 1e-9) return;
        n = n * (1 / l);
        if (dot(n, d) < 0) n = -n;
        S sep = dot(n, d) - box_radius(A, n) - box_radius(B, n);
        if (sep - bias > best_sep + 1e-9) { best_sep = sep - bias; best_kind = kind; best_i = i; best_j = j; best_n = n; }
    };
    for (int i = 0; i < 3; ++i) consider(A.r.c[i], 0, i, 0, 0);
    for (int i = 0; i < 3; ++i) consider(B.r.c[i], 1, i, 0, 0);
    const S face_sep = best_sep;
    const int face_kind = best_kind, face_i = best_i;
    const V3 face_n = best_n;
    for (int i = 0; i < 3; ++i)
        for (int j = 0; j < 3; ++j) consider(cross(A.r.c[i], B.r.c[j]), 2, i, j, 1e-4);
    S sep = best_kind == 2 ? best_sep + 1e-4 : best_sep;
    if (sep > max_dist) return false;
    normal = best_n;
    if (best_kind == 2) {
        V3 ea = A.r.c[best_i], eb = B.r.c[best_j];
        V3 pa = A.c, pb = B.c;
        for (int k = 0; k < 3; ++k) {
            if (k != best_i) pa = pa + A.r.c[k] * (comp(A.he, k) * (dot(A.r.c[k], normal) > 0 ? 1 : -1));
            if (k != best_j) pb = pb + B.r.c[k] * (comp(B.he, k) * (dot(B.r.c[k], normal) < 0 ? 1 : -1));
        }
        S s, t;
        if (!segment_closest(pa, ea, comp(A.he, best_i), pb, eb, comp(B.he, best_j), s, t)) {
            pts.push(pa + ea * s, pb + eb * t);
            return true;
        }
        if (sep > 0) {
            V3 on_a, on_b;
            S dist = box_box_closest(A, B, on_a, on_b);
            return closest_pair(on_a, on_b, dist, max_dist, normal, pts);
        }
        sep = face_sep; best_kind = face_kind; best_i = face_i; normal = face_n;
    }
    const bool ref_is_a = best_kind == 0;
    const Box& R = ref_is_a ? A : B;
    const Box& I = ref_is_a ? B : A;
    V3 rn = ref_is_a ? normal : -normal;
    int inc_axis = 0;
    S inc_best = -1;
    for (int k = 0; k < 3; ++k) {
        S v = fabs(dot(I.r.c[k], rn));
        if (v > inc_best) { inc_best = v; inc_axis = k; }
    }
    S isign = dot(I.r.c[inc_axis], rn) > 0 ? -1 : 1;
    V3 poly[16], tmp[16];
    box_face(I, inc_axis, isign, poly);
    int np = 4;
    int u = (best_i + 1) % 3, v = (best_i + 2) % 3;
    const int axes[2] = {u, v};
    for (int a = 0; a < 2 && np > 0; ++a) {
        V3 sn = R.r.c[axes[a]];
        S he = comp(R.he, axes[a]);
        np = clip_poly(poly, np, sn, dot(sn, R.c) + he, tmp);
        np = clip_poly(tmp, np, -sn, -dot(sn, R.c) + he, poly);
    }
    S face_d = dot(rn, R.c) + comp(R.he, best_i) * 1.0;
    S nearest = 1e300;
    for (int k = 0; k < np; ++k) {
        S dist = dot(rn, poly[k]) - face_d;
        if (dist > max_dist) continue;
        nearest = smin(nearest, dist);
        V3 on_ref = poly[k] - rn * dist;
        bool dup = false;
        for (int q = 0; q < pts.n; ++q) {
            V3 e = (ref_is_a ? pts.p[q].b : pts.p[q].a) - poly[k];
            if (dot(e, e) < 1e-12) { dup = true; break; }
        }
        if (dup) continue;
        if (pts.n == MAX_RAW_POINTS) break;
        if (ref_is_a) pts.push(on_ref, poly[k]); else pts.push(poly[k], on_ref);
    }
    if (sep > 0 && nearest > sep + FACE_GAP_SLACK) {
        V3 on_a, on_b;
        S dist = box_box_closest(A, B, on_a, on_b);
        if (nearest > dist + FACE_GAP_SLACK) return closest_pair(on_a, on_b, dist, max_dist, normal, pts);
    }
    return pts.n != 0;
}

NM_HD inline void prune4(Contacts& pts, V3 n) {
    if (pts.n <= 4) return;
    auto depth = [&](int i) { return dot(pts.p[i].a - pts.p[i].b, n); };
    int p0 = 0;
    for (int i = 1; i < pts.n; ++i) if (depth(i) > depth(p0) + 1e-12) p0 = i;
    int p1 = p0;
    S best = -1;
    for (int i = 0; i < pts.n; ++i) { V3 e = pts.p[i].a - pts.p[p0].a; S v = dot(e, e); if (v > best) { best = v; p1 = i; } }
    V3 dir = cross(pts.p[p1].a - pts.p[p0].a, n);
    int p2 = p0, p3 = p0;
    S mx = 0, mn = 0;
    for (int i = 0; i < pts.n; ++i) {
        S v = dot(pts.p[i].a - pts.p[p0].a, dir);
        if (v > mx) { mx = v; p2 = i; }
        if (v < mn) { mn = v; p3 = i; }
    }
    bool keep[MAX_RAW_POINTS] = {false, false, false, false, false, false, false, false};
    keep[p0] = keep[p1] = keep[p2] = keep[p3] = true;
    int m = 0;
    for (int i = 0; i < pts.n; ++i)
        if (keep[i]) pts.p[m++] = pts.p[i];
    pts.n = m;
}

NM_HD inline bool sphere_sphere(V3 ca, S ra, V3 cb, S rb, S max_dist, V3& normal, Contacts& pts) {
    pts.clear();
    V3 d = cb - ca;
    S l = len(d);
    if (l - ra - rb > max_dist) return false;
    normal = l > 1e-12 ? d * (1 / l) : V3{0, 1, 0};
    pts.push(ca + normal * ra, cb - normal * rb);
    return true;
}

NM_HD inline bool box_sphere(const Box& A, V3 cs, S rs, S max_dist, V3& normal, Contacts& pts) {
    pts.clear();
    V3 d = cs - A.c;
    V3 local{dot(d, A.r.c[0]), dot(d, A.r.c[1]), dot(d, A.r.c[2])};
    V3 cl{smax(-A.he.x, smin(A.he.x, local.x)), smax(-A.he.y, smin(A.he.y, local.y)), smax(-A.he.z, smin(A.he.z, local.z))};
    V3 on_box = A.c + A.r.c[0] * cl.x + A.r.c[1] * cl.y + A.r.c[2] * cl.z;
    V3 e = cs - on_box;
    S l = len(e);
    const bool inside = fabs(local.x) <= A.he.x && fabs(local.y) <= A.he.y && fabs(local.z) <= A.he.z;
    if (!inside && l > 1e-9) {
        if (l - rs > max_dist) return false;
        normal = e * (1 / l);
    } else {
        int ax = 0; S best = 1e300;
        for (int k = 0; k < 3; ++k) { S v = comp(A.he, k) - fabs(comp(local, k)); if (v < best) { best = v; ax = k; } }
        S sgn = comp(local, ax) >= 0 ? 1 : -1;
        normal = A.r.c[ax] * sgn;
        on_box = cs + normal * best;
    }
    pts.push(on_box, cs - normal * rs);
    return true;
}


constexpr S CAPSULE_PARALLEL_SIN = 1e-3;
constexpr S CAPSULE_EDGE_AXIS_MIN = 1e-6;

struct Capsule { V3 c, u; S h, r; };

NM_HD inline V3 capsule_perpendicular(V3 u) {
    const V3 e = (fabs(u.x) <= fabs(u.y) && fabs(u.x) <= fabs(u.z)) ? V3{1, 0, 0} : (fabs(u.y) <= fabs(u.z) ? V3{0, 1, 0} : V3{0, 0, 1});
    const V3 n = cross(u, e);
    return n * (1 / len(n));
}

NM_COLD inline bool capsule_round(const Capsule& A, V3 q, V3 w, S hw, S rb, S max_dist, V3& normal, Contacts& pts) {
    S s, t;
    segment_closest(A.c, A.u, A.h, q, w, hw, s, t);
    const V3 p = A.c + A.u * s, qq = q + w * t, d = qq - p;
    const S l = len(d);
    if (l - A.r - rb > max_dist) return false;
    const V3 x = cross(A.u, w);
    const S lx = len(x);
    const bool parallel = !(hw > 0) || lx <= CAPSULE_PARALLEL_SIN;
    if (l > 1e-12) {
        normal = d * (1 / l);
    } else if (!parallel) {
        normal = x * (1 / lx);
        if (dot(normal, q - A.c) < 0) normal = -normal;
    } else {
        normal = capsule_perpendicular(A.u);
    }
    if (hw > 0 && parallel) {
        const S t0 = dot(q - w * hw - A.c, A.u), t1 = dot(q + w * hw - A.c, A.u);
        const S lo = smax(-A.h, smin(t0, t1)), hi = smin(A.h, smax(t0, t1));
        if (lo < hi) {
NM_ROLLED
            for (int i = 0; i < 2; ++i) {
                const V3 pi = A.c + A.u * (i == 0 ? lo : hi);
                const S ti = smax(-hw, smin(hw, dot(pi - q, w)));
                pts.push(pi + normal * A.r, q + w * ti - normal * rb);
            }
            return true;
        }
    }
    pts.push(p + normal * A.r, qq - normal * rb);
    return true;
}

NM_COLD inline S segment_box_closest(const Box& b, const Capsule& C, V3& on_seg, V3& on_box) {
    S best = 1e300;
NM_ROLLED
    for (int i = 0; i < 2; ++i) {
        const V3 p = C.c + C.u * (i == 0 ? -C.h : C.h);
        V3 on;
        const S d2 = box_point_closest(b, p, on);
        if (d2 < best) { best = d2; on_seg = p; on_box = on; }
    }
NM_ROLLED
    for (int ei = 0; ei < 12; ++ei) {
        const int k = ei >> 2, m = ei & 3, u = (k + 1) % 3, v = (k + 2) % 3;
        const V3 e = b.c + b.r.c[u] * (m & 1 ? comp(b.he, u) : -comp(b.he, u)) + b.r.c[v] * (m & 2 ? comp(b.he, v) : -comp(b.he, v));
        S s, t;
        segment_closest(C.c, C.u, C.h, e, b.r.c[k], comp(b.he, k), s, t);
        const V3 qs = C.c + C.u * s, qe = e + b.r.c[k] * t, d = qs - qe;
        const S d2 = dot(d, d);
        if (d2 < best) { best = d2; on_seg = qs; on_box = qe; }
    }
    return sqrt(best);
}

NM_HD inline bool capsule_face_clip(const Box& b, int k, const Capsule& C, S& lo, S& hi) {
    lo = -C.h; hi = C.h;
NM_ROLLED
    for (int i = 1; i < 3; ++i) {
        const int j = (k + i) % 3;
        const S a = dot(b.r.c[j], C.c - b.c), g = dot(b.r.c[j], C.u), he = comp(b.he, j);
        if (fabs(g) < 1e-12) {
            if (fabs(a) > he) return false;
            continue;
        }
        const S s0 = (-he - a) / g, s1 = (he - a) / g;
        lo = smax(lo, smin(s0, s1));
        hi = smin(hi, smax(s0, s1));
    }
    return lo <= hi;
}

NM_COLD inline bool box_capsule(const Box& b, const Capsule& C, S max_dist, V3& normal, Contacts& pts) {
    const V3 d = C.c - b.c;
    S max_sep = -1e300, best = -1e300, face_best = -1e300;
    int best_k = 0, face_k = 0;
    bool best_edge = false;
    V3 best_n{0, 1, 0}, face_n{0, 1, 0};
NM_ROLLED
    for (int i = 0; i < 6; ++i) {
        V3 n = i < 3 ? b.r.c[i] : cross(b.r.c[i - 3], C.u);
        const S l = len(n);
        if (l < CAPSULE_EDGE_AXIS_MIN) continue;
        n = n * (1 / l);
        if (dot(n, d) < 0) n = -n;
        const S sep = dot(n, d) - box_radius(b, n) - C.h * fabs(dot(C.u, n));
        max_sep = smax(max_sep, sep);
        const S biased = i < 3 ? sep : sep - 1e-4;
        if (biased > best + 1e-9) { best = biased; best_k = i % 3; best_edge = i >= 3; best_n = n; }
        if (i < 3 && sep > face_best + 1e-9) { face_best = sep; face_k = i; face_n = n; }
    }
    int fk = -1;
    if (max_sep > 0) {
        V3 on_seg, on_box;
        const S dist = segment_box_closest(b, C, on_seg, on_box);
        if (dist - C.r > max_dist) return false;
        normal = (on_seg - on_box) * (1 / dist);
NM_ROLLED
        for (int k = 0; k < 3; ++k)
            if (fabs(dot(normal, b.r.c[k])) >= 1 - 0.5 * CAPSULE_PARALLEL_SIN * CAPSULE_PARALLEL_SIN) fk = k;
        if (fk < 0 || fabs(dot(C.u, b.r.c[fk])) > CAPSULE_PARALLEL_SIN) {
            pts.push(on_box, on_seg - normal * C.r);
            return true;
        }
        normal = b.r.c[fk] * (dot(normal, b.r.c[fk]) < 0 ? -1 : 1);
    } else {
        if (best_edge) {
            const V3 n = best_n;
            V3 e = b.c;
NM_ROLLED
            for (int j = 0; j < 3; ++j)
                if (j != best_k) e = e + b.r.c[j] * (comp(b.he, j) * (dot(b.r.c[j], n) > 0 ? 1 : -1));
            S s, t;
            if (!segment_closest(C.c, C.u, C.h, e, b.r.c[best_k], comp(b.he, best_k), s, t)) {
                normal = n;
                pts.push(e + b.r.c[best_k] * t, C.c + C.u * s - n * C.r);
                return true;
            }
        }
        fk = face_k;
        normal = face_n;
    }
    const S face_d = dot(normal, b.c) + comp(b.he, fk);
    S lo, hi;
    if (!capsule_face_clip(b, fk, C, lo, hi)) {
        lo = hi = dot(C.u, normal) > 0 ? -C.h : C.h;
    } else if (fabs(dot(C.u, normal)) > CAPSULE_PARALLEL_SIN || !(lo < hi)) {
        lo = hi = dot(C.u, normal) > 0 ? lo : hi;
    }
NM_ROLLED
    for (int i = 0; i < (lo < hi ? 2 : 1); ++i) {
        const V3 q = C.c + C.u * (i == 0 ? lo : hi);
        pts.push(q - normal * (dot(normal, q) - face_d), q - normal * C.r);
    }
    return true;
}

NM_COLD inline V3 capsule_pair(int type_a, V3 dims_a, Q qa, int type_b, V3 dims_b, V3 pb, Q qb, S max_dist, Contacts& pts) {
    pts.clear();
    const bool cap_b = type_a != SHAPE_CAPSULE;
    const int to = cap_b ? type_a : type_b;
    const V3 dc = cap_b ? dims_b : dims_a, dn = cap_b ? dims_a : dims_b;
    const Q qc = cap_b ? qb : qa, qo = cap_b ? qa : qb;
    const V3 pc = cap_b ? pb : V3{0, 0, 0}, po = cap_b ? V3{0, 0, 0} : pb;
    const Capsule C{pc, rot(qc, {0, 1, 0}), dc.y, dc.x};
    V3 normal{0, 1, 0};
    bool flip;
    if (to == SHAPE_CUBOID) {
        const Box X{po, to_mat(qo), dn};
        box_capsule(X, C, max_dist, normal, pts);
        flip = !cap_b;
    } else {
        if (to == SHAPE_CAPSULE) capsule_round(C, po, rot(qo, {0, 1, 0}), dn.y, dn.x, max_dist, normal, pts);
        else capsule_round(C, po, C.u, 0, dn.x, max_dist, normal, pts);
        flip = cap_b;
    }
    if (flip) {
        normal = -normal;
NM_ROLLED
        for (int k = 0; k < pts.n; ++k) { V3 t = pts.p[k].a; pts.p[k].a = pts.p[k].b; pts.p[k].b = t; }
    }
    return normal;
}

template <bool CAPSULES = true>
NM_HD inline bool collide(int type_a, V3 he_a, V3 pa, Q qa, int type_b, V3 he_b, V3 pb, Q qb, S max_dist, V3& normal, Contacts& pts) {
    pb = pb - pa;
    pa = V3{0, 0, 0};
    bool hit;
    if (type_a == SHAPE_CUBOID && type_b == SHAPE_CUBOID) {
        Box A{pa, to_mat(qa), he_a}, B{pb, to_mat(qb), he_b};
        hit = box_box(A, B, max_dist, normal, pts);
        if (hit) prune4(pts, normal);
    } else if (type_a == SHAPE_SPHERE && type_b == SHAPE_SPHERE) {
        hit = sphere_sphere(pa, he_a.x, pb, he_b.x, max_dist, normal, pts);
    } else if (CAPSULES && (type_a == SHAPE_CAPSULE || type_b == SHAPE_CAPSULE)) {
        normal = capsule_pair(type_a, he_a, qa, type_b, he_b, pb, qb, max_dist, pts);
        hit = pts.n != 0;
    } else if (type_a == SHAPE_CUBOID) {
        Box A{pa, to_mat(qa), he_a};
        hit = box_sphere(A, pb, he_b.x, max_dist, normal, pts);
    } else {
        Box B{pb, to_mat(qb), he_b};
        hit = box_sphere(B, pa, he_a.x, max_dist, normal, pts);
        if (hit) {
            normal = -normal;
            for (int k = 0; k < pts.n; ++k) { V3 t = pts.p[k].a; pts.p[k].a = pts.p[k].b; pts.p[k].b = t; }
        }
    }
    return hit;
}

struct PointOut { V3 anchor1, anchor2; S penetration, normal_speed; };

struct PairFrames { V3 offset1, com1, offset2, com2; };

template <bool FRAMES>
NM_HD inline int manifold_points_in(const Contacts& pts, V3 normal, V3 pa, V3 pb, V3 rel, V3 w1, V3 w2, S dt, S eff_margin, const PairFrames* fr,
                                    PointOut out[4]) {
    int m = 0;
    for (int k = 0; k < pts.n && m < 4; ++k) {
        PointOut pt;
        pt.anchor1 = pts.p[k].a;
        pt.anchor2 = pts.p[k].b - (pb - pa);
        if (FRAMES) {
            pt.anchor1 = (pt.anchor1 + fr->offset1) - fr->com1;
            pt.anchor2 = (pt.anchor2 + fr->offset2) - fr->com2;
        }
        pt.penetration = dot(pts.p[k].a - pts.p[k].b, normal);
        V3 rv = rel + cross(w2, pt.anchor2) - cross(w1, pt.anchor1);
        pt.normal_speed = dot(rv, normal);
        bool keep = -pt.penetration < eff_margin || (pt.normal_speed * dt - pt.penetration < eff_margin);
        if (!keep) continue;
        out[m++] = pt;
    }
    return m;
}
NM_HD inline int manifold_points(const Contacts& pts, V3 normal, V3 pa, V3 pb, V3 rel, V3 w1, V3 w2, S dt, S eff_margin, PointOut out[4]) {
    return manifold_points_in<false>(pts, normal, pa, pb, rel, w1, w2, dt, eff_margin, nullptr, out);
}
NM_HD inline int manifold_points(const Contacts& pts, V3 normal, V3 pa, V3 pb, V3 rel, V3 w1, V3 w2, S dt, S eff_margin, const PairFrames& fr,
                                 PointOut out[4]) {
    return manifold_points_in<true>(pts, normal, pa, pb, rel, w1, w2, dt, eff_margin, &fr, out);
}

NM_HD inline int match_point(V3 anchor1, V3 anchor2, const V3* old_anchor1, const V3* old_anchor2, int n_old, S thr2) {
    for (int k = 0; k < n_old; ++k) {
        V3 e11 = anchor1 - old_anchor1[k], e22 = anchor2 - old_anchor2[k], e12 = anchor1 - old_anchor2[k], e21 = anchor2 - old_anchor1[k];
        if ((dot(e11, e11) < thr2 && dot(e22, e22) < thr2) || (dot(e12, e12) < thr2 && dot(e21, e21) < thr2)) return k;
    }
    return -1;
}

}
```

### avian_b200/host/host_api.cpp

```cpp
#include <algorithm>
#include <cmath>
#include <cstdint>
#include <cstdio>
#include <cstring>
#include <queue>
#include <unordered_map>
#include <vector>

#include "../../include/avian_b200.h"
#include "../csrc/narrow_math.hpp"
#include "../csrc/contact_rows.hpp"
#include "../csrc/query_math.hpp"
#include "../csrc/ccd_math.hpp"
#include "../csrc/move_math.hpp"

namespace {

using namespace nm;

inline Q qmul(Q a, Q b) {
    return {a.w * b.x + a.x * b.w + a.y * b.z - a.z * b.y, a.w * b.y - a.x * b.z + a.y * b.w + a.z * b.x,
            a.w * b.z + a.x * b.y - a.y * b.x + a.z * b.w, a.w * b.w - a.x * b.x - a.y * b.y - a.z * b.z};
}
inline Q q_from_scaled_axis(V3 v) {
// ... 42 lines not shown
    void unset(uint32_t i) { if (i < body_set.size()) body_set[i] = 0; }
};

struct Pipeline {
    uint32_t n = 0;
    std::vector<Shape> shapes;
    std::vector<uint32_t> order;
    std::vector<Pair> pairs;
    std::priority_queue<uint32_t, std::vector<uint32_t>, std::greater<uint32_t>> free_ids;
    std::unordered_map<uint64_t, uint32_t> pair_set;
    std::vector<uint32_t> active;
    std::vector<uint8_t> sensor;
    struct Event { uint32_t c1, c2, b1, b2; uint8_t flags; };
    std::vector<Event> started, ended;
    std::vector<Event> pending_ended;
    Color colors[AVN_GRAPH_COLOR_COUNT];
    S contact_tolerance = 0.005, length_unit = 1.0;
    struct Ref { uint32_t id, mi, pi; };
    std::vector<Ref> export_refs;
};

inline uint64_t pair_key(uint32_t a, uint32_t b) { return a < b ? (uint64_t(a) << 32) | b : (uint64_t(b) << 32) | a; }

void push_manifold(Pipeline& P, uint32_t id) {
    Pair& pr = P.pairs[id];
    int color = AVN_COLOR_OVERFLOW;
    if (!pr.static1 && !pr.static2) {
        for (int i = 0; i < AVN_DYNAMIC_COLOR_COUNT; ++i) {
            Color& c = P.colors[i];
            if (c.get(pr.body1) || c.get(pr.body2)) continue;
            c.set(pr.body1); c.set(pr.body2); color = i; break;
        }
    } else if (!pr.static1) {
        for (int i = AVN_COLOR_OVERFLOW - 1; i >= 1; --i) {
            Color& c = P.colors[i];
            if (c.get(pr.body1)) continue;
            c.set(pr.body1); color = i; break;
        }
    } else if (!pr.static2) {
        for (int i = AVN_COLOR_OVERFLOW - 1; i >= 1; --i) {
            Color& c = P.colors[i];
            if (c.get(pr.body2)) continue;
            c.set(pr.body2); color = i; break;
        }
    }
    Color& c = P.colors[color];
    uint32_t manifold_index = uint32_t(pr.handles.size());
    pr.handles.push_back({color, uint32_t(c.handles.size())});
    c.handles.push_back({id, manifold_index});
}
void pop_manifold(Pipeline& P, uint32_t id) {
    Pair& pr = P.pairs[id];
    if (pr.handles.empty()) return;
    Handle h = pr.handles.back();
    pr.handles.pop_back();
    Color& c = P.colors[h.color];
    if (h.color != AVN_COLOR_OVERFLOW) { c.unset(pr.body1); c.unset(pr.body2); }
    uint32_t moved = uint32_t(c.handles.size()) - 1;
    c.handles[h.local] = c.handles[moved];
    c.handles.pop_back();
    if (moved != h.local) {
        auto mh = c.handles[h.local];
        P.pairs[mh.first].handles[mh.second].local = h.local;
    }
}

template <class T>
static void rows_narrow(uint32_t E, uint32_t* c1, uint32_t* c2, uint32_t* b1, uint32_t* b2, uint8_t* live, uint8_t* count, uint8_t* disjoint, void* normal, void* a1,
                        void* a2, void* pen, void* ns, uint8_t* prev_count, double* prev_a1, double* prev_a2, void* ws_n_in, void* ws_t_in, void* ws_n_out,
                        void* ws_t_out, const uint8_t* shape, const void* dims, const void* pos, const void* rot, const void* lv, const void* av,
                        const void* amin, const void* amax, double dt, double tol, double length_unit, uint32_t match, const void* body_pos = nullptr,
                        const void* body_rot = nullptr, const void* body_com = nullptr) {
    avn::NarrowEdgeArgs<T> a{};
    a.r.E = int(E);
    a.r.c1 = c1; a.r.c2 = c2; a.r.b1 = b1; a.r.b2 = b2; a.r.live = live; a.r.count = count; a.r.disjoint = disjoint;
    a.r.normal = static_cast<T*>(normal); a.r.a1 = static_cast<T*>(a1); a.r.a2 = static_cast<T*>(a2); a.r.pen = static_cast<T*>(pen); a.r.ns = static_cast<T*>(ns);
    a.r.prev_count = prev_count; a.r.prev_a1 = prev_a1; a.r.prev_a2 = prev_a2;
    a.r.ws_n_in = static_cast<T*>(ws_n_in); a.r.ws_t_in = static_cast<T*>(ws_t_in); a.r.ws_n_out = static_cast<T*>(ws_n_out); a.r.ws_t_out = static_cast<T*>(ws_t_out);
    a.r.nimp_in = nullptr; a.r.nimp_out = nullptr;
    a.shape = shape; a.dims = static_cast<const T*>(dims); a.pos = static_cast<const T*>(pos); a.rot = static_cast<const T*>(rot);
    a.lv = static_cast<const T*>(lv); a.av = static_cast<const T*>(av); a.amin = static_cast<const T*>(amin); a.amax = static_cast<const T*>(amax);
    a.dt = dt; a.tol = tol; a.thr2 = (0.1 * length_unit) * (0.1 * length_unit); a.match = match ? 1 : 0;
    const avn::BodyFrameCols<T> f{static_cast<const T*>(body_pos), static_cast<const T*>(body_rot), static_cast<const T*>(body_com)};
    for (uint32_t e = 0; e < E; ++e) {
        if (body_pos) avn::narrow_edge_row<T, true, true>(a, int(e), f);
        else avn::narrow_edge_row<T>(a, int(e));
    }
}

nm::PairFrames host_pair_frames(bool f64, const void* body_pos, const void* body_rot, const void* body_com, uint32_t ba, V3 pa, uint32_t bb, V3 pb) {
    if (f64) return avn::pair_frames(avn::BodyFrameCols<double>{static_cast<const double*>(body_pos), static_cast<const double*>(body_rot),
                                                                static_cast<const double*>(body_com)}, ba, pa, bb, pb);
    return avn::pair_frames(avn::BodyFrameCols<float>{static_cast<const float*>(body_pos), static_cast<const float*>(body_rot),
                                                      static_cast<const float*>(body_com)}, ba, pa, bb, pb);
}

}

extern "C" {

struct AvhPipeline;

AvhPipeline* avh_create(uint32_t n_bodies) {
    Pipeline* p = new Pipeline();
    p->n = n_bodies;
    p->shapes.assign(n_bodies, Shape{SHAPE_CUBOID, {0.5, 0.5, 0.5}, 0.5, 0.0});
    return reinterpret_cast<AvhPipeline*>(p);
}
void avh_destroy(AvhPipeline* h) { delete reinterpret_cast<Pipeline*>(h); }

void avh_set_shapes(AvhPipeline* h, const int32_t* shape_type, const double* dims, const double* friction, const double* restitution) {
    Pipeline& P = *reinterpret_cast<Pipeline*>(h);
    for (uint32_t i = 0; i < P.n; ++i)
        P.shapes[i] = Shape{shape_type[i], {dims[3 * i], dims[3 * i + 1], dims[3 * i + 2]}, friction[i], restitution[i]};
}

void avh_update_aabbs(AvhPipeline* h, uint32_t scalar_bits, const void* position, const void* rotation, const void* linvel, const void* angvel,
                      double dt, void* out_min, void* out_max) {
    Pipeline& P = *reinterpret_cast<Pipeline*>(h);
    const bool f64 = scalar_bits == 64;
    Col pos{position, f64}, rt{rotation, f64}, lv{linvel, f64}, av{angvel, f64};
    ColW omin{out_min, f64}, omax{out_max, f64};
    const S tol = P.contact_tolerance * P.length_unit;
    for (uint32_t i = 0; i < P.n; ++i) {
        const Shape& sh = P.shapes[i];
        V3 p0 = pos.v3(i), v = lv.v3(i), w = av.v3(i);
        Q q0 = rt.q(i);
        Q q1 = qmul(q_from_scaled_axis(w * dt), q0);
        S l2 = q1.x * q1.x + q1.y * q1.y + q1.z * q1.z + q1.w * q1.w, k = 0.5 * (3 - l2);
        q1 = {q1.x * k, q1.y * k, q1.z * k, q1.w * k};
        V3 p1 = p0 + v * dt;
        V3 lo{1e300, 1e300, 1e300}, hi{-1e300, -1e300, -1e300};
        for (int e = 0; e < 2; ++e) {
            V3 c = e ? p1 : p0;
            V3 ext;
            if (sh.type == SHAPE_CAPSULE) {
                const Q q = e ? q1 : q0;
                const V3 b{q.x, q.y, q.z};
                V3 ends[2];
                for (int i = 0; i < 2; ++i) {
                    const V3 v{0, i ? sh.he.y : -sh.he.y, 0};
                    const V3 t = cross(b, v) * 2.0;
                    ends[i] = ((v + cross(b, t)) + t * q.w) + c;
                }
                lo = {std::min(lo.x, std::min(ends[0].x, ends[1].x) - sh.he.x), std::min(lo.y, std::min(ends[0].y, ends[1].y) - sh.he.x),
                      std::min(lo.z, std::min(ends[0].z, ends[1].z) - sh.he.x)};
                hi = {std::max(hi.x, std::max(ends[0].x, ends[1].x) + sh.he.x), std::max(hi.y, std::max(ends[0].y, ends[1].y) + sh.he.x),
                      std::max(hi.z, std::max(ends[0].z, ends[1].z) + sh.he.x)};
                continue;
            }
            if (sh.type == SHAPE_SPHERE) {
                ext = {sh.he.x, sh.he.x, sh.he.x};
            } else {
                M3 m = to_mat(e ? q1 : q0);
                ext = {std::fabs(m.c[0].x) * sh.he.x + std::fabs(m.c[1].x) * sh.he.y + std::fabs(m.c[2].x) * sh.he.z,
                       std::fabs(m.c[0].y) * sh.he.x + std::fabs(m.c[1].y) * sh.he.y + std::fabs(m.c[2].y) * sh.he.z,
                       std::fabs(m.c[0].z) * sh.he.x + std::fabs(m.c[1].z) * sh.he.y + std::fabs(m.c[2].z) * sh.he.z};
            }
            lo = {std::min(lo.x, c.x - ext.x), std::min(lo.y, c.y - ext.y), std::min(lo.z, c.z - ext.z)};
            hi = {std::max(hi.x, c.x + ext.x), std::max(hi.y, c.y + ext.y), std::max(hi.z, c.z + ext.z)};
        }
        omin.set3(i, {lo.x - tol, lo.y - tol, lo.z - tol});
        omax.set3(i, {hi.x + tol, hi.y + tol, hi.z + tol});
    }
}

uint32_t avh_get_order(AvhPipeline* h, uint32_t* out) {
    Pipeline& P = *reinterpret_cast<Pipeline*>(h);
    if (P.order.size() != P.n) {
// ... 125 lines not shown
    for (uint32_t id = 0; id < P.pairs.size(); ++id) {
        const Pair& pr = P.pairs[id];
        if (!pr.alive) continue;
        if (ids) { ids[n] = id; touching[n] = pr.touching; asleep[n] = pr.asleep; }
        ++n;
    }
    return n;
}

void avh_set_sensors(AvhPipeline* h, const uint8_t* sensor) {
    Pipeline& P = *reinterpret_cast<Pipeline*>(h);
    std::vector<uint8_t> now(P.n, 0);
    if (sensor) for (uint32_t c = 0; c < P.n; ++c) now[c] = sensor[c] ? 1 : 0;
    std::vector<uint32_t> changed;
    for (uint32_t c = 0; c < P.n; ++c)
        if (now[c] != (P.sensor.empty() ? 0 : P.sensor[c])) changed.push_back(c);
    P.sensor = std::find(now.begin(), now.end(), uint8_t(1)) != now.end() ? now : std::vector<uint8_t>();
    avh_remove_colliders(h, uint32_t(changed.size()), changed.data());
}

uint32_t avh_events(AvhPipeline* h, uint32_t which, uint32_t* c1, uint32_t* c2, uint32_t* b1, uint32_t* b2, uint8_t* flags) {
    Pipeline& P = *reinterpret_cast<Pipeline*>(h);
    const auto& list = which ? P.ended : P.started;
    for (size_t i = 0; i < list.size(); ++i) {
        if (c1) c1[i] = list[i].c1;
        if (c2) c2[i] = list[i].c2;
        if (b1) b1[i] = list[i].b1;
        if (b2) b2[i] = list[i].b2;
        if (flags) flags[i] = list[i].flags;
    }
    return uint32_t(list.size());
}

}
template <class T>
static uint32_t report_rows(Pipeline& P, uint32_t events_only, uint32_t* contact_id, uint32_t* c1, uint32_t* c2, uint32_t* b1, uint32_t* b2, uint8_t* flags,
                            uint8_t* point_count, T* normal, T* total, T* mx, T* deep) {
    uint32_t n = 0;
    for (uint32_t id = 0; id < P.pairs.size(); ++id) {
        const Pair& pr = P.pairs[id];
        if (!pr.alive || !pr.touching || (events_only && !(pr.flags & AVN_PAIR_CONTACT_EVENTS))) continue;
        if (contact_id) {
            contact_id[n] = id; c1[n] = pr.collider1; c2[n] = pr.collider2; b1[n] = pr.body1; b2[n] = pr.body2; flags[n] = uint8_t(pr.flags & 0x0f);
            const Manifold* m = pr.manifolds.empty() ? nullptr : &pr.manifolds[0];
            const int cnt = m ? int(m->pts.size()) : 0;
            point_count[n] = uint8_t(cnt);
            T tot = T(0), big = T(0), d = T(0);
            for (int k = 0; k < cnt; ++k) {
                const T v = T(m->pts[k].normal_impulse);
                tot = tot + v;
                if (v > big) big = v;
                const T p = T(m->pts[k].penetration);
                if (k == 0 || p >= d) d = p;
            }
            const V3 nv = m ? m->normal : V3{0, 0, 0};
            normal[3 * n] = T(nv.x); normal[3 * n + 1] = T(nv.y); normal[3 * n + 2] = T(nv.z);
            total[n] = tot; mx[n] = big; deep[n] = d;
        }
        ++n;
    }
    return n;
}
extern "C" {
uint32_t avh_report(AvhPipeline* h, uint32_t scalar_bits, uint32_t events_only, uint32_t* contact_id, uint32_t* c1, uint32_t* c2, uint32_t* b1, uint32_t* b2,
                    uint8_t* flags, uint8_t* point_count, void* normal, void* total, void* mx, void* deep) {
    Pipeline& P = *reinterpret_cast<Pipeline*>(h);
    if (scalar_bits == 64)
        return report_rows<double>(P, events_only, contact_id, c1, c2, b1, b2, flags, point_count, static_cast<double*>(normal), static_cast<double*>(total),
                                   static_cast<double*>(mx), static_cast<double*>(deep));
    return report_rows<float>(P, events_only, contact_id, c1, c2, b1, b2, flags, point_count, static_cast<float*>(normal), static_cast<float*>(total),
                              static_cast<float*>(mx), static_cast<float*>(deep));
}

uint32_t avh_narrow_phase(AvhPipeline* h, uint32_t scalar_bits, const uint8_t* kind, const void* position, const void* rotation, const void* linvel,
                          const void* angvel, const void* aabb_min, const void* aabb_max, double dt, uint32_t match_contacts, uint32_t* out_points,
                          const void* body_pos, const void* body_rot, const void* body_com) {
    Pipeline& P = *reinterpret_cast<Pipeline*>(h);
    const bool f64 = scalar_bits == 64;
    Col pos{position, f64}, rt{rotation, f64}, lv{linvel, f64}, av{angvel, f64}, amin{aabb_min, f64}, amax{aabb_max, f64};
    const S tol = P.contact_tolerance * P.length_unit;
    std::vector<uint32_t> changed;
    std::vector<uint8_t> disjoint(P.pairs.size(), 0), started(P.pairs.size(), 0), stopped(P.pairs.size(), 0);
    std::vector<int> count_change(P.pairs.size(), 0);
    Contacts pts;
    for (uint32_t id : P.active) {
        Pair& pr = P.pairs[id];
        if (pr.asleep) continue;
        const uint32_t a = pr.collider1, b = pr.collider2;
        V3 mina = amin.v3(a), maxa = amax.v3(a), minb = amin.v3(b), maxb = amax.v3(b);
        bool overlap = !(mina.x > maxb.x || maxa.x < minb.x || mina.y > maxb.y || maxa.y < minb.y || mina.z > maxb.z || maxa.z < minb.z);
        if (!overlap) { disjoint[id] = 1; changed.push_back(id); continue; }
        pr.static1 = kind[pr.body1] == AVN_BODY_STATIC;
        pr.static2 = kind[pr.body2] == AVN_BODY_STATIC;
        const Shape& sa = P.shapes[a];
        const Shape& sb = P.shapes[b];
        V3 v1 = lv.v3(pr.body1), v2 = lv.v3(pr.body2), w1 = av.v3(pr.body1), w2 = av.v3(pr.body2);
        V3 rel = v2 - v1;
        S eff_margin = dt * len(rel);
        S max_dist = std::max(eff_margin, tol);
        std::vector<Manifold> old = std::move(pr.manifolds);
        pr.manifolds.clear();
        V3 normal;
        V3 pa = pos.v3(a), pb = pos.v3(b);
        const bool hit = collide(sa.type, sa.he, pa, rt.q(a), sb.type, sb.he, pb, rt.q(b), max_dist, normal, pts);
        if (hit) {
            PointOut out[4];
            const int np = body_pos ? manifold_points(pts, normal, pa, pb, rel, w1, w2, dt, eff_margin,
                                                      host_pair_frames(f64, body_pos, body_rot, body_com, pr.body1, pa, pr.body2, pb), out)
                                    : manifold_points(pts, normal, pa, pb, rel, w1, w2, dt, eff_margin, out);
            if (np > 0) {
                Manifold m;
                m.normal = normal;
                for (int k = 0; k < np; ++k) {
                    Point pt;
                    pt.anchor1 = out[k].anchor1;
                    pt.anchor2 = out[k].anchor2;
                    pt.penetration = out[k].penetration;
                    pt.normal_speed = out[k].normal_speed;
                    m.pts.push_back(pt);
                }
                pr.manifolds.push_back(std::move(m));
            }
        }
        bool touching = !pr.manifolds.empty();
        if (touching && match_contacts && pr.manifolds.size() <= 4) {
            const S thr2 = (0.1 * P.length_unit) * (0.1 * P.length_unit);
            for (Manifold& m : pr.manifolds)
                for (const Manifold& om : old) {
                    V3 oa1[8], oa2[8];
                    const int n_old = int(std::min<size_t>(om.pts.size(), 8));
                    for (int k = 0; k < n_old; ++k) { oa1[k] = om.pts[k].anchor1; oa2[k] = om.pts[k].anchor2; }
                    for (Point& c : m.pts) {
                        const int k = match_point(c.anchor1, c.anchor2, oa1, oa2, n_old, thr2);
                        if (k >= 0) { c.ws_normal = om.pts[k].ws_normal; c.ws_tx = om.pts[k].ws_tx; c.ws_ty = om.pts[k].ws_ty; }
                    }
                }
        }
        count_change[id] = int(pr.manifolds.size()) - int(old.size());
        if (touching && !pr.touching) { started[id] = 1; changed.push_back(id); }
        else if (!touching && pr.touching) { stopped[id] = 1; changed.push_back(id); }
        else if (count_change[id] != 0) changed.push_back(id);
    }
    return apply_status_changes(P, changed, disjoint, started, stopped, count_change, out_points);
}

void avh_export_manifolds(AvhPipeline* h, uint32_t scalar_bits, uint32_t* color_offsets , int32_t* body1, int32_t* body2, void* normal,
                          void* friction, void* restitution, uint32_t* point_offsets, void* anchor1, void* anchor2, void* penetration,
                          void* normal_speed, void* ws_normal, void* ws_tangent) {
    Pipeline& P = *reinterpret_cast<Pipeline*>(h);
    const bool f64 = scalar_bits == 64;
    ColW wn{normal, f64}, wf{friction, f64}, wr{restitution, f64}, wa1{anchor1, f64}, wa2{anchor2, f64}, wp{penetration, f64}, ws{normal_speed, f64},
        wwn{ws_normal, f64}, wwt{ws_tangent, f64};
    P.export_refs.clear();
    uint32_t m = 0, p = 0;
    for (int c = 0; c < AVN_GRAPH_COLOR_COUNT; ++c) {
        color_offsets[c] = m;
        for (auto& hnd : P.colors[c].handles) {
            const Pair& pr = P.pairs[hnd.first];
            const Manifold& mf = pr.manifolds[hnd.second];
            body1[m] = int32_t(pr.body1);
            body2[m] = int32_t(pr.body2);
            wn.set3(m, mf.normal);
            wf.set(m, (P.shapes[pr.collider1].friction + P.shapes[pr.collider2].friction) * 0.5);
            wr.set(m, (P.shapes[pr.collider1].restitution + P.shapes[pr.collider2].restitution) * 0.5);
            point_offsets[m] = p;
            for (uint32_t k = 0; k < mf.pts.size(); ++k) {
                const Point& pt = mf.pts[k];
                wa1.set3(p, pt.anchor1); wa2.set3(p, pt.anchor2);
                wp.set(p, pt.penetration); ws.set(p, pt.normal_speed);
                wwn.set(p, pt.ws_normal); wwt.set(2 * p, pt.ws_tx); wwt.set(2 * p + 1, pt.ws_ty);
                P.export_refs.push_back({hnd.first, hnd.second, k});
                ++p;
            }
            ++m;
        }
    }
    color_offsets[AVN_GRAPH_COLOR_COUNT] = m;
    point_offsets[m] = p;
}

void avh_store_impulses(AvhPipeline* h, uint32_t scalar_bits, const void* ws_normal, const void* ws_tangent, const void* normal_impulse) {
    Pipeline& P = *reinterpret_cast<Pipeline*>(h);
    const bool f64 = scalar_bits == 64;
    Col n{ws_normal, f64}, t{ws_tangent, f64}, ni{normal_impulse, f64};
    for (size_t p = 0; p < P.export_refs.size(); ++p) {
        auto r = P.export_refs[p];
        Point& pt = P.pairs[r.id].manifolds[r.mi].pts[r.pi];
        pt.ws_normal = n.at(p); pt.ws_tx = t.at(2 * p); pt.ws_ty = t.at(2 * p + 1); pt.normal_impulse = ni.at(p);
    }
}

void avh_raw_manifolds(uint32_t scalar_bits, uint32_t pair_count, const uint32_t* c1, const uint32_t* c2, const uint32_t* b1, const uint32_t* b2,
                       const uint8_t* shape, const void* dims, const void* position, const void* rotation, const void* linvel, const void* angvel,
                       const void* aabb_min, const void* aabb_max, double dt, double tol, uint8_t* point_count, uint8_t* disjoint, void* normal,
                       void* anchor1, void* anchor2, void* penetration, void* normal_speed, double* anchor1_f64, double* anchor2_f64, const void* body_pos,
                       const void* body_rot, const void* body_com) {
    const bool f64 = scalar_bits == 64;
    Col dm{dims, f64}, pos{position, f64}, rt{rotation, f64}, lv{linvel, f64}, av{angvel, f64}, amin{aabb_min, f64}, amax{aabb_max, f64};
    ColW on{normal, f64}, oa1{anchor1, f64}, oa2{anchor2, f64}, op{penetration, f64}, os{normal_speed, f64};
    for (uint32_t k = 0; k < pair_count; ++k) {
        const uint32_t a = c1[k], b = c2[k];
        point_count[k] = 0;
        on.set3(k, V3{0, 0, 0});
        for (int p = 0; p < 4; ++p) { oa1.set3(4 * size_t(k) + p, V3{0, 0, 0}); oa2.set3(4 * size_t(k) + p, V3{0, 0, 0}); op.set(4 * size_t(k) + p, 0); os.set(4 * size_t(k) + p, 0); }
        if (aabb_min) {
            V3 mina = amin.v3(a), maxa = amax.v3(a), minb = amin.v3(b), maxb = amax.v3(b);
            bool overlap = !(mina.x > maxb.x || maxa.x < minb.x || mina.y > maxb.y || maxa.y < minb.y || mina.z > maxb.z || maxa.z < minb.z);
            if (disjoint) disjoint[k] = overlap ? 0 : 1;
            if (!overlap) continue;
        } else if (disjoint) {
            disjoint[k] = 0;
        }
        V3 pa = pos.v3(a), pb = pos.v3(b);
        V3 v1 = lv.v3(b1[k]), v2 = lv.v3(b2[k]), w1 = av.v3(b1[k]), w2 = av.v3(b2[k]);
        V3 rel = v2 - v1;
        S eff_margin = dt * len(rel);
        S max_dist = smax(eff_margin, tol);
        V3 nrm;
        Contacts pts;
        int ta = shape ? shape[a] : SHAPE_CUBOID, tb = shape ? shape[b] : SHAPE_CUBOID;
        if (!collide(ta, dm.v3(a), pa, rt.q(a), tb, dm.v3(b), pb, rt.q(b), max_dist, nrm, pts)) continue;
        PointOut out[4];
        int np = body_pos ? manifold_points(pts, nrm, pa, pb, rel, w1, w2, dt, eff_margin, host_pair_frames(f64, body_pos, body_rot, body_com, b1[k], pa, b2[k], pb), out)
                          : manifold_points(pts, nrm, pa, pb, rel, w1, w2, dt, eff_margin, out);
        point_count[k] = uint8_t(np);
        on.set3(k, nrm);
        for (int p = 0; p < np; ++p) {
            oa1.set3(4 * size_t(k) + p, out[p].anchor1);
            oa2.set3(4 * size_t(k) + p, out[p].anchor2);
            if (anchor1_f64)
                for (int c = 0; c < 3; ++c) {
                    anchor1_f64[(4 * size_t(k) + p) * 3 + c] = comp(out[p].anchor1, c);
                    anchor2_f64[(4 * size_t(k) + p) * 3 + c] = comp(out[p].anchor2, c);
                }
            op.set(4 * size_t(k) + p, out[p].penetration);
            os.set(4 * size_t(k) + p, out[p].normal_speed);
        }
    }
}

uint32_t avh_active_edges(AvhPipeline* h, uint32_t* ids, uint32_t* c1, uint32_t* c2, uint32_t* b1, uint32_t* b2) {
    Pipeline& P = *reinterpret_cast<Pipeline*>(h);
    uint32_t n = 0;
    for (uint32_t id : P.active) {
        const Pair& pr = P.pairs[id];
        ids[n] = id; c1[n] = pr.collider1; c2[n] = pr.collider2; b1[n] = pr.body1; b2[n] = pr.body2;
        ++n;
    }
    return n;
}

void avh_export_edges(AvhPipeline* h, uint32_t* color_offsets , uint32_t* edge, int32_t* body1, int32_t* body2, double* friction, double* restitution) {
    Pipeline& P = *reinterpret_cast<Pipeline*>(h);
    uint32_t m = 0;
    for (int c = 0; c < AVN_GRAPH_COLOR_COUNT; ++c) {
        color_offsets[c] = m;
        for (auto& hnd : P.colors[c].handles) {
            const Pair& pr = P.pairs[hnd.first];
            edge[m] = hnd.first;
            body1[m] = int32_t(pr.body1);
            body2[m] = int32_t(pr.body2);
            friction[m] = (P.shapes[pr.collider1].friction + P.shapes[pr.collider2].friction) * 0.5;
            restitution[m] = (P.shapes[pr.collider1].restitution + P.shapes[pr.collider2].restitution) * 0.5;
            ++m;
        }
    }
    color_offsets[AVN_GRAPH_COLOR_COUNT] = m;
}

void avh_match_raw(uint32_t scalar_bits, uint32_t n, const uint32_t* ids, const uint8_t* new_count, const double* new_a1, const double* new_a2,
                   double length_unit, uint32_t match_contacts, uint8_t* prev_count, double* prev_a1, double* prev_a2, void* ws_n, void* ws_t) {
    const bool f64 = scalar_bits == 64;
    Col rn{ws_n, f64}, rtg{ws_t, f64};
    ColW wn{ws_n, f64}, wt{ws_t, f64};
    const S thr2 = (0.1 * length_unit) * (0.1 * length_unit);
    for (uint32_t i = 0; i < n; ++i) {
        const size_t e = ids[i];
        const int nc = new_count[i], oc = prev_count[e];
        V3 oa1[4], oa2[4];
        S on[4], otx[4], oty[4];
        for (int k = 0; k < oc; ++k) {
            oa1[k] = V3{prev_a1[(e * 4 + k) * 3], prev_a1[(e * 4 + k) * 3 + 1], prev_a1[(e * 4 + k) * 3 + 2]};
            oa2[k] = V3{prev_a2[(e * 4 + k) * 3], prev_a2[(e * 4 + k) * 3 + 1], prev_a2[(e * 4 + k) * 3 + 2]};
            on[k] = rn.at(e * 4 + k); otx[k] = rtg.at((e * 4 + k) * 2); oty[k] = rtg.at((e * 4 + k) * 2 + 1);
        }
        for (int k = 0; k < 4; ++k) {
            S vn = 0, vx = 0, vy = 0;
            if (k < nc) {
                const V3 a1{new_a1[(size_t(i) * 4 + k) * 3], new_a1[(size_t(i) * 4 + k) * 3 + 1], new_a1[(size_t(i) * 4 + k) * 3 + 2]};
                const V3 a2{new_a2[(size_t(i) * 4 + k) * 3], new_a2[(size_t(i) * 4 + k) * 3 + 1], new_a2[(size_t(i) * 4 + k) * 3 + 2]};
                const int j = match_contacts ? match_point(a1, a2, oa1, oa2, oc, thr2) : -1;
                if (j >= 0) { vn = on[j]; vx = otx[j]; vy = oty[j]; }
                for (int c = 0; c < 3; ++c) { prev_a1[(e * 4 + k) * 3 + c] = comp(a1, c); prev_a2[(e * 4 + k) * 3 + c] = comp(a2, c); }
            }
            wn.set(e * 4 + k, vn);
            wt.set((e * 4 + k) * 2, vx);
            wt.set((e * 4 + k) * 2 + 1, vy);
        }
        prev_count[e] = uint8_t(nc);
    }
}

void avh_rows_narrow(uint32_t scalar_bits, uint32_t E, uint32_t* c1, uint32_t* c2, uint32_t* b1, uint32_t* b2, uint8_t* live, uint8_t* count, uint8_t* disjoint,
                     void* normal, void* a1, void* a2, void* pen, void* ns, uint8_t* prev_count, double* prev_a1, double* prev_a2, void* ws_n_in, void* ws_t_in,
                     void* ws_n_out, void* ws_t_out, const uint8_t* shape, const void* dims, const void* pos, const void* rot, const void* lv, const void* av,
                     const void* amin, const void* amax, double dt, double tol, double length_unit, uint32_t match) {
    if (scalar_bits == 64)
        rows_narrow<double>(E, c1, c2, b1, b2, live, count, disjoint, normal, a1, a2, pen, ns, prev_count, prev_a1, prev_a2, ws_n_in, ws_t_in, ws_n_out, ws_t_out,
                            shape, dims, pos, rot, lv, av, amin, amax, dt, tol, length_unit, match);
    else
        rows_narrow<float>(E, c1, c2, b1, b2, live, count, disjoint, normal, a1, a2, pen, ns, prev_count, prev_a1, prev_a2, ws_n_in, ws_t_in, ws_n_out, ws_t_out,
                           shape, dims, pos, rot, lv, av, amin, amax, dt, tol, length_unit, match);
}
void avh_rows_narrow_framed(uint32_t scalar_bits, uint32_t E, uint32_t* c1, uint32_t* c2, uint32_t* b1, uint32_t* b2, uint8_t* live, uint8_t* count,
                            uint8_t* disjoint, void* normal, void* a1, void* a2, void* pen, void* ns, uint8_t* prev_count, double* prev_a1, double* prev_a2,
                            void* ws_n_in, void* ws_t_in, void* ws_n_out, void* ws_t_out, const uint8_t* shape, const void* dims, const void* pos,
                            const void* rot, const void* lv, const void* av, const void* amin, const void* amax, double dt, double tol, double length_unit,
                            uint32_t match, const void* body_pos, const void* body_rot, const void* body_com) {
    if (scalar_bits == 64)
        rows_narrow<double>(E, c1, c2, b1, b2, live, count, disjoint, normal, a1, a2, pen, ns, prev_count, prev_a1, prev_a2, ws_n_in, ws_t_in, ws_n_out, ws_t_out,
                            shape, dims, pos, rot, lv, av, amin, amax, dt, tol, length_unit, match, body_pos, body_rot, body_com);
    else
        rows_narrow<float>(E, c1, c2, b1, b2, live, count, disjoint, normal, a1, a2, pen, ns, prev_count, prev_a1, prev_a2, ws_n_in, ws_t_in, ws_n_out, ws_t_out,
                           shape, dims, pos, rot, lv, av, amin, amax, dt, tol, length_unit, match, body_pos, body_rot, body_com);
}

uint32_t avh_pair_count(AvhPipeline* h) { return uint32_t(reinterpret_cast<Pipeline*>(h)->active.size()); }

}

namespace {
thread_local char g_query_error[256];
int query_fail(AvnStatus st, const char* why) {
    snprintf(g_query_error, sizeof g_query_error, "%s", why);
    return st;
}

struct QueryScene {
    const AvnQueryColliders* c; bool f64;
    Col dims, pos, rot;
    QueryScene(const AvnQueryColliders* cc, bool f) : c(cc), f64(f), dims{cc->dims, f}, pos{cc->position, f}, rot{cc->rotation, f} {}
    bool valid(uint32_t i) const { return qm::collider_valid(dims.v3(i), pos.v3(i), rot.q(i)); }
    uint32_t memb(uint32_t i) const { return c->memberships ? c->memberships[i] : 1u; }
};
struct RayView {
    V3 o, d; S maxd; bool solid, ok; uint32_t mask; const uint32_t* xs; uint32_t nx;
};
RayView ray_at(const AvnRayBatch* r, bool f64, uint32_t i) {
    Col o{r->origin, f64}, d{r->direction, f64}, m{r->max_distance, f64};
    RayView v;
    v.o = o.v3(i); v.d = d.v3(i); v.maxd = m.at(i);
    v.solid = r->solid ? r->solid[i] != 0 : true;
    v.mask = r->mask ? r->mask[i] : 0xffffffffu;
    v.xs = r->exclude_offsets ? r->exclude + r->exclude_offsets[i] : nullptr;
    v.nx = r->exclude_offsets ? r->exclude_offsets[i + 1] - r->exclude_offsets[i] : 0u;
    v.ok = qm::ray_finite(v.o, v.d, v.maxd);
    return v;
}
struct RayHit { S t; uint32_t c; V3 n; };
void all_hits(const QueryScene& sc, const RayView& v, std::vector<RayHit>& out) {
    out.clear();
    if (!v.ok) return;
    for (uint32_t c = 0; c < sc.c->count; ++c) {
        if (!sc.valid(c) || !qm::passes_filter(sc.memb(c), v.mask, v.xs, v.nx, c)) continue;
        RayHit h{0, c, V3{0, 0, 0}};
        if (qm::ray_collider(sc.c->shape[c], sc.dims.v3(c), sc.pos.v3(c), sc.rot.q(c), v.o, v.d, v.maxd, v.solid, h.t, h.n)) out.push_back(h);
    }
    std::sort(out.begin(), out.end(), [](const RayHit& a, const RayHit& b) { return qm::hit_before(a.t, a.c, b.t, b.c); });
}
template <class T>
void query_aabbs(const QueryScene& sc, uint32_t n, const T* mn, const T* mx, std::vector<std::vector<uint32_t>>& per) {
    for (uint32_t c = 0; c < sc.c->count; ++c) {
        if (!sc.valid(c)) continue;
        V3 a, b;
// ... 561 lines not shown
```

Before: 441.6.

## Move narrow-phase contact scratch to shared memory and skip radix sort when presorted

```diff
diff --git a/avian_b200/_build.py b/avian_b200/_build.py
--- a/avian_b200/_build.py
+++ b/avian_b200/_build.py
@@ -40,7 +40,7 @@
     "comm.cu": ["context.hpp"],
     "aabb.cu": ["avn_math.cuh", "context.hpp"],
     "broadphase.cu": ["avn_math.cuh", "context.hpp", "broadphase_cells.cuh", "device_prims.cuh"],
-    "narrow.cu": ["avn_math.cuh", "context.hpp", "narrow_math.hpp"],
+    "narrow.cu": ["avn_math.cuh", "context.hpp", "narrow_math.hpp", "contact_rows.hpp"],
     "contacts.cu": ["avn_math.cuh", "context.hpp", "narrow_math.hpp", "contact_rows.hpp", "device_prims.cuh"],
     "queries.cu": ["context.hpp", "narrow_math.hpp", "query_math.hpp", "move_math.hpp", "device_prims.cuh"],
     "ccd.cu": ["avn_math.cuh", "context.hpp", "narrow_math.hpp", "query_math.hpp", "ccd_math.hpp", "device_prims.cuh"],
diff --git a/avian_b200/csrc/broadphase.cu b/avian_b200/csrc/broadphase.cu
--- a/avian_b200/csrc/broadphase.cu
+++ b/avian_b200/csrc/broadphase.cu
@@ -29,13 +29,15 @@
 
 template <class S>
 __global__ void make_keys(const S* __restrict__ aabb_min, const S* __restrict__ aabb_max, int n, typename KeyOf<S>::type* __restrict__ keys,
-                          uint32_t* __restrict__ vals, unsigned long long* __restrict__ nonfinite) {
+                          uint32_t* __restrict__ vals, unsigned long long* __restrict__ nonfinite, unsigned long long* __restrict__ unsorted) {
     int i = blockIdx.x * blockDim.x + threadIdx.x;
     if (i < n) {
         const S a = aabb_min[3 * i], b = aabb_min[3 * i + 1], c = aabb_min[3 * i + 2], d = aabb_max[3 * i], e = aabb_max[3 * i + 1], f = aabb_max[3 * i + 2];
         const S z = (a - a) + (b - b) + (c - c) + (d - d) + (e - e) + (f - f);
         if (!(z == S(0))) *nonfinite = 1ull;
-        keys[i] = sortable(a);
+        const typename KeyOf<S>::type k = sortable(a);
+        if (i > 0 && sortable(aabb_min[3 * (i - 1)]) > k) *unsorted = 1ull;
+        keys[i] = k;
         vals[i] = uint32_t(i);
     }
 }
@@ -363,7 +365,7 @@
     const int nsub = (n + SW_SUB - 1) / SW_SUB;
     AVN_CUDA(wide_sub_.ensure(size_t(nsub) * size_t(std::min(n, SW_WIDE_CAP)) * 4));
     AVN_CUDA(block_sums_.ensure(size_t((n + 1023) / 1024) * 8));
-    AVN_CUDA(nf_flag_.ensure(8));
+    AVN_CUDA(nf_flag_.ensure(16));
     pair_capacity_ = std::max<uint64_t>(pair_capacity_, uint64_t(4) * uint64_t(n) + 1024);
     AVN_CUDA(o_c1_.ensure(pair_capacity_ * 4)); AVN_CUDA(o_c2_.ensure(pair_capacity_ * 4)); AVN_CUDA(o_b1_.ensure(pair_capacity_ * 4)); AVN_CUDA(o_b2_.ensure(pair_capacity_ * 4));
     AVN_CUDA(o_fl_.ensure(pair_capacity_));
@@ -391,17 +393,19 @@
     uint32_t launches = 0;
     K* ka = k0_.as<K>(); K* kb = k1_.as<K>();
     uint32_t* va = v0_.as<uint32_t>(); uint32_t* vb = v1_.as<uint32_t>();
-    cudaMemsetAsync(nf_flag_.p, 0, 8, stream_);
-    make_keys<S><<<(n + 255) / 256, 256, 0, stream_>>>(d_min_, d_max_, n, ka, va, nf_flag_.as<unsigned long long>());
+    cudaMemsetAsync(nf_flag_.p, 0, 16, stream_);
+    const unsigned long long* unsorted = nf_flag_.as<unsigned long long>() + 1;
+    make_keys<S><<<(n + 255) / 256, 256, 0, stream_>>>(d_min_, d_max_, n, ka, va, nf_flag_.as<unsigned long long>(), nf_flag_.as<unsigned long long>() + 1);
     ++launches;
+    static_assert(KeyOf<S>::passes % 2 == 0, "skipped passes leave the identity order in buffer 0");
     for (int pass = 0; pass < KeyOf<S>::passes; ++pass) {
         const int shift = 8 * pass;
-        rs_histogram<K><<<nblocks, RS_THREADS, 0, stream_>>>(ka, n, shift, hist_.as<uint32_t>(), nblocks);
+        rs_histogram<K><<<nblocks, RS_THREADS, 0, stream_>>>(ka, n, shift, hist_.as<uint32_t>(), nblocks, unsorted);
         if (nblocks <= RS_FUSE_MAX_BLOCKS) {
-            rs_scatter<K, true><<<nblocks, RS_THREADS, 0, stream_>>>(ka, va, n, shift, hist_.as<uint32_t>(), nblocks, kb, vb);
+            rs_scatter<K, true><<<nblocks, RS_THREADS, 0, stream_>>>(ka, va, n, shift, hist_.as<uint32_t>(), nblocks, kb, vb, unsorted);
         } else {
             rs_scan<<<1, 1024, 0, stream_>>>(hist_.as<uint32_t>(), 256 * nblocks);
-            rs_scatter<K, false><<<nblocks, RS_THREADS, 0, stream_>>>(ka, va, n, shift, hist_.as<uint32_t>(), nblocks, kb, vb);
+            rs_scatter<K, false><<<nblocks, RS_THREADS, 0, stream_>>>(ka, va, n, shift, hist_.as<uint32_t>(), nblocks, kb, vb, unsorted);
         }
         launches += nblocks <= RS_FUSE_MAX_BLOCKS ? 2 : 3;
         std::swap(ka, kb);
diff --git a/avian_b200/csrc/ccd_math.hpp b/avian_b200/csrc/ccd_math.hpp
--- a/avian_b200/csrc/ccd_math.hpp
+++ b/avian_b200/csrc/ccd_math.hpp
@@ -93,7 +93,7 @@
     r = qm::rot_mat(qt);
 }
 
-NM_COLD inline S shape_distance(int sa, V3 ha, V3 ca, const nm::M3& ra, int sb, V3 hb, V3 cb, const nm::M3& rb, V3& n) {
+NM_NOINLINE inline S shape_distance(int sa, V3 ha, V3 ca, const nm::M3& ra, int sb, V3 hb, V3 cb, const nm::M3& rb, V3& n) {
     n = V3{0, 1, 0};
     if (sa == nm::SHAPE_SPHERE && sb == nm::SHAPE_SPHERE) {
         const V3 e = cb - ca;
diff --git a/avian_b200/csrc/contact_rows.hpp b/avian_b200/csrc/contact_rows.hpp
--- a/avian_b200/csrc/contact_rows.hpp
+++ b/avian_b200/csrc/contact_rows.hpp
@@ -50,8 +50,25 @@
     return a.shape && a.r.live[e] && (a.shape[a.r.c1[e]] == nm::SHAPE_CAPSULE || a.shape[a.r.c2[e]] == nm::SHAPE_CAPSULE);
 }
 
+#if defined(__CUDACC__)
+constexpr int NARROW_THREADS = 128;
+constexpr int NARROW_MIN_BLOCKS = 2;
+constexpr size_t NARROW_TILE_BYTES = sizeof(double) * nm::SCRATCH_SLOTS * NARROW_THREADS;
+constexpr int NARROW_CARVEOUT_PERCENT = int((NARROW_MIN_BLOCKS * (NARROW_TILE_BYTES + 1024) * 100 + 228 * 1024 - 1) / (228 * 1024));
+__device__ __forceinline__ nm::Contacts tile_contacts() {
+    extern __shared__ double narrow_tile[];
+    return nm::Contacts(nm::Slots{narrow_tile + threadIdx.x, NARROW_THREADS});
+}
+template <class K>
+inline cudaError_t narrow_tile_attributes(K kernel) {
+    cudaError_t st = cudaFuncSetAttribute(kernel, cudaFuncAttributeMaxDynamicSharedMemorySize, int(NARROW_TILE_BYTES));
+    if (st == cudaSuccess) st = cudaFuncSetAttribute(kernel, cudaFuncAttributePreferredSharedMemoryCarveout, NARROW_CARVEOUT_PERCENT);
+    return st;
+}
+#endif
+
 template <class S, bool CAPSULES = true, bool FRAMES = false>
-NM_HD inline void narrow_edge_row(const NarrowEdgeArgs<S>& a, int e, const BodyFrameCols<S>& f = BodyFrameCols<S>{}) {
+NM_HD inline void narrow_edge_row(const NarrowEdgeArgs<S>& a, int e, nm::Contacts& pts, const BodyFrameCols<S>& f = BodyFrameCols<S>{}) {
     const EdgeRows<S>& r = a.r;
     if (r.asleep && r.asleep[e]) return;
     if (!r.live[e]) { r.count[e] = 0; r.disjoint[e] = 0; return; }
@@ -73,7 +90,6 @@
         const nm::V3 rel = v2 - v1;
         const double eff_margin = a.dt * nm::len(rel);
         const double max_dist = nm::smax(eff_margin, a.tol);
-        nm::Contacts pts;
         const int ta = a.shape ? a.shape[ca] : nm::SHAPE_CUBOID, tb = a.shape ? a.shape[cb] : nm::SHAPE_CUBOID;
         if (nm::collide<CAPSULES>(ta, ldd3(a.dims, ca), pa, qa, tb, ldd3(a.dims, cb), pb, qb, max_dist, normal, pts)) {
             if (FRAMES) np = nm::manifold_points(pts, normal, pa, pb, rel, w1, w2, a.dt, eff_margin, pair_frames(f, ba, pa, bb, pb), out);
@@ -84,7 +100,9 @@
     const int oc = r.prev_count[e];
     nm::V3 oa1[4], oa2[4];
     S on[4], otx[4], oty[4];
-    for (int k = 0; k < oc; ++k) {
+NM_UNROLLED
+    for (int k = 0; k < 4; ++k) {
+        if (k >= oc) break;
         const size_t q = size_t(e) * 4 + k;
         oa1[k] = nm::V3{r.prev_a1[3 * q], r.prev_a1[3 * q + 1], r.prev_a1[3 * q + 2]};
         oa2[k] = nm::V3{r.prev_a2[3 * q], r.prev_a2[3 * q + 1], r.prev_a2[3 * q + 2]};
@@ -92,12 +110,15 @@
     }
     r.count[e] = uint8_t(np);
     std3(r.normal, size_t(e), normal);
+NM_UNROLLED
     for (int k = 0; k < 4; ++k) {
         const size_t q = size_t(e) * 4 + k;
         S vn = S(0), vx = S(0), vy = S(0);
         if (k < np) {
-            const int j = a.match ? nm::match_point(out[k].anchor1, out[k].anchor2, oa1, oa2, oc, a.thr2) : -1;
-            if (j >= 0) { vn = on[j]; vx = otx[j]; vy = oty[j]; }
+            const int j = a.match ? nm::match_point<4>(out[k].anchor1, out[k].anchor2, oa1, oa2, oc, a.thr2) : -1;
+NM_UNROLLED
+            for (int i = 0; i < 4; ++i)
+                if (i == j) { vn = on[i]; vx = otx[i]; vy = oty[i]; }
             std3(r.a1, q, out[k].anchor1);
             std3(r.a2, q, out[k].anchor2);
             r.pen[q] = S(out[k].penetration);
diff --git a/avian_b200/csrc/contacts.cu b/avian_b200/csrc/contacts.cu
--- a/avian_b200/csrc/contacts.cu
+++ b/avian_b200/csrc/contacts.cu
@@ -388,7 +388,7 @@
 }
 
 template <class S>
-__global__ void __launch_bounds__(128) narrow_edges_kernel(const __grid_constant__ NarrowEdgeArgs<S> a, uint8_t* fresh, int only_fresh, int capsules) {
+__global__ void __launch_bounds__(NARROW_THREADS, NARROW_MIN_BLOCKS) narrow_edges_kernel(const __grid_constant__ NarrowEdgeArgs<S> a, uint8_t* fresh, int only_fresh, int capsules) {
     const int e = blockIdx.x * blockDim.x + threadIdx.x;
     if (e >= a.r.E) return;
     if (capsules && capsule_row(a, e)) return;
@@ -396,22 +396,24 @@
         if (!fresh[e]) return;
         fresh[e] = 0;
     }
-    narrow_edge_row<S, false>(a, e);
+    nm::Contacts pts = tile_contacts();
+    narrow_edge_row<S, false>(a, e, pts);
 }
 
 template <class S>
-__global__ void __launch_bounds__(128) narrow_capsule_edges_kernel(const __grid_constant__ NarrowEdgeArgs<S> a, uint8_t* fresh, int only_fresh) {
+__global__ void __launch_bounds__(NARROW_THREADS, NARROW_MIN_BLOCKS) narrow_capsule_edges_kernel(const __grid_constant__ NarrowEdgeArgs<S> a, uint8_t* fresh, int only_fresh) {
     const int e = blockIdx.x * blockDim.x + threadIdx.x;
     if (e >= a.r.E || !capsule_row(a, e)) return;
     if (only_fresh) {
         if (!fresh[e]) return;
         fresh[e] = 0;
     }
-    narrow_edge_row<S, true>(a, e);
+    nm::Contacts pts = tile_contacts();
+    narrow_edge_row<S, true>(a, e, pts);
 }
 
 template <class S, bool CAPSULES>
-__global__ void __launch_bounds__(128) narrow_framed_edges_kernel(const __grid_constant__ NarrowEdgeArgs<S> a, const BodyFrameCols<S> f, uint8_t* fresh,
+__global__ void __launch_bounds__(NARROW_THREADS, NARROW_MIN_BLOCKS) narrow_framed_edges_kernel(const __grid_constant__ NarrowEdgeArgs<S> a, const BodyFrameCols<S> f, uint8_t* fresh,
                                                                   int only_fresh, int capsules) {
     const int e = blockIdx.x * blockDim.x + threadIdx.x;
     if (e >= a.r.E) return;
@@ -420,7 +422,8 @@
         if (!fresh[e]) return;
         fresh[e] = 0;
     }
-    narrow_edge_row<S, CAPSULES, true>(a, e, f);
+    nm::Contacts pts = tile_contacts();
+    narrow_edge_row<S, CAPSULES, true>(a, e, pts, f);
 }
 
 
@@ -1329,12 +1332,21 @@
         a.tol = prm->contact_tolerance;
         a.thr2 = (0.1 * length_unit) * (0.1 * length_unit);
         a.match = match_contacts ? 1 : 0;
+        const unsigned nb = (n + NARROW_THREADS - 1) / NARROW_THREADS;
         if (in_.framed) {
-            narrow_framed_edges_kernel<S, false><<<(n + 127) / 128, 128, 0, s>>>(a, in_.frames, fresh_.as<uint8_t>(), only_fresh ? 1 : 0, has_capsule_ ? 1 : 0);
-            if (has_capsule_) narrow_framed_edges_kernel<S, true><<<(n + 127) / 128, 128, 0, s>>>(a, in_.frames, fresh_.as<uint8_t>(), only_fresh ? 1 : 0, 1);
+            AVN_CUDA(narrow_tile_attributes(narrow_framed_edges_kernel<S, false>));
+            narrow_framed_edges_kernel<S, false><<<nb, NARROW_THREADS, NARROW_TILE_BYTES, s>>>(a, in_.frames, fresh_.as<uint8_t>(), only_fresh ? 1 : 0, has_capsule_ ? 1 : 0);
+            if (has_capsule_) {
+                AVN_CUDA(narrow_tile_attributes(narrow_framed_edges_kernel<S, true>));
+                narrow_framed_edges_kernel<S, true><<<nb, NARROW_THREADS, NARROW_TILE_BYTES, s>>>(a, in_.frames, fresh_.as<uint8_t>(), only_fresh ? 1 : 0, 1);
+            }
         } else {
-            narrow_edges_kernel<S><<<(n + 127) / 128, 128, 0, s>>>(a, fresh_.as<uint8_t>(), only_fresh ? 1 : 0, has_capsule_ ? 1 : 0);
-            if (has_capsule_) narrow_capsule_edges_kernel<S><<<(n + 127) / 128, 128, 0, s>>>(a, fresh_.as<uint8_t>(), only_fresh ? 1 : 0);
+            AVN_CUDA(narrow_tile_attributes(narrow_edges_kernel<S>));
+            narrow_edges_kernel<S><<<nb, NARROW_THREADS, NARROW_TILE_BYTES, s>>>(a, fresh_.as<uint8_t>(), only_fresh ? 1 : 0, has_capsule_ ? 1 : 0);
+            if (has_capsule_) {
+                AVN_CUDA(narrow_tile_attributes(narrow_capsule_edges_kernel<S>));
+                narrow_capsule_edges_kernel<S><<<nb, NARROW_THREADS, NARROW_TILE_BYTES, s>>>(a, fresh_.as<uint8_t>(), only_fresh ? 1 : 0);
+            }
         }
         AVN_CUDA(cudaGetLastError());
         return AVN_OK;
diff --git a/avian_b200/csrc/device_prims.cuh b/avian_b200/csrc/device_prims.cuh
--- a/avian_b200/csrc/device_prims.cuh
+++ b/avian_b200/csrc/device_prims.cuh
@@ -10,7 +10,9 @@
 constexpr int RS_TILE = RS_THREADS * RS_ROUNDS;
 
 template <class K>
-__global__ void __launch_bounds__(RS_THREADS) rs_histogram(const K* __restrict__ keys, int n, int shift, uint32_t* __restrict__ hist, int nblocks) {
+__global__ void __launch_bounds__(RS_THREADS) rs_histogram(const K* __restrict__ keys, int n, int shift, uint32_t* __restrict__ hist, int nblocks,
+                                                           const unsigned long long* __restrict__ unsorted = nullptr) {
+    if (unsorted && *unsorted == 0ull) return;
     __shared__ uint32_t cnt[256];
     cnt[threadIdx.x] = 0;
     __syncthreads();
@@ -73,7 +75,8 @@
 template <class K, bool FUSED>
 __global__ void __launch_bounds__(RS_THREADS) rs_scatter(const K* __restrict__ keys_in, const uint32_t* __restrict__ vals_in, int n, int shift,
                                                          const uint32_t* __restrict__ offsets, int nblocks, K* __restrict__ keys_out,
-                                                         uint32_t* __restrict__ vals_out) {
+                                                         uint32_t* __restrict__ vals_out, const unsigned long long* __restrict__ unsorted = nullptr) {
+    if (unsorted && *unsorted == 0ull) return;
     __shared__ uint32_t wcnt[RS_WARPS][256];
     __shared__ uint32_t digit_base[256];
     __shared__ uint32_t scan_warp[8];
diff --git a/avian_b200/csrc/move_math.hpp b/avian_b200/csrc/move_math.hpp
--- a/avian_b200/csrc/move_math.hpp
+++ b/avian_b200/csrc/move_math.hpp
@@ -87,13 +87,13 @@
 }
 
 template <class T>
-NM_COLD inline bool contact_plane(int sa, V3 ha, V3 pa, Q qa, int sb, V3 hb, V3 pb, Q qb, double prediction, T3<float>& normal, T& penetration) {
+NM_NOINLINE inline bool contact_plane(int sa, V3 ha, V3 pa, Q qa, int sb, V3 hb, V3 pb, Q qb, double prediction, T3<float>& normal, T& penetration) {
     V3 n;
-    nm::Contacts pts;
+    nm::LocalContacts pts;
     if (!nm::collide<false>(sa, ha, pa, qa, sb, hb, pb, qb, prediction, n, pts) || pts.n == 0) return false;
-    T best = T(nm::dot(pts.p[0].a - pts.p[0].b, n));
+    T best = T(nm::dot(pts.a(0) - pts.b(0), n));
     for (int k = 1; k < pts.n; ++k) {
-        const T p = T(nm::dot(pts.p[k].a - pts.p[k].b, n));
+        const T p = T(nm::dot(pts.a(k) - pts.b(k), n));
         if (!(p < best)) best = p;
     }
     penetration = best;
diff --git a/avian_b200/csrc/narrow.cu b/avian_b200/csrc/narrow.cu
--- a/avian_b200/csrc/narrow.cu
+++ b/avian_b200/csrc/narrow.cu
@@ -41,7 +41,7 @@
     const double eff_margin = a.dt * nm::len(rel);
     const double max_dist = nm::smax(eff_margin, a.tol);
     nm::V3 normal;
-    nm::Contacts pts;
+    nm::Contacts pts = tile_contacts();
     const int ta = a.shape ? a.shape[ca] : nm::SHAPE_CUBOID, tb = a.shape ? a.shape[cb] : nm::SHAPE_CUBOID;
     if (!nm::collide<CAPSULES>(ta, ld3(a.dims, ca), pa, qa, tb, ld3(a.dims, cb), pb, qb, max_dist, normal, pts)) return;
     nm::PointOut out[4];
@@ -49,7 +49,9 @@
                           : nm::manifold_points(pts, normal, pa, pb, rel, w1, w2, a.dt, eff_margin, out);
     a.count[k] = uint8_t(np);
     st3(a.normal, k, normal);
-    for (int p = 0; p < np; ++p) {
+#pragma unroll
+    for (int p = 0; p < 4; ++p) {
+        if (p >= np) break;
         st3(a.anchor1, size_t(4) * k + p, out[p].anchor1);
         st3(a.anchor2, size_t(4) * k + p, out[p].anchor2);
         a.penetration[size_t(4) * k + p] = S(out[p].penetration);
@@ -58,11 +60,11 @@
 }
 
 template <class S>
-__global__ void __launch_bounds__(128) narrow_phase_kernel(const __grid_constant__ NarrowArgs<S> a, int capsules) { narrow_pair<S, false>(a, capsules); }
+__global__ void __launch_bounds__(NARROW_THREADS, NARROW_MIN_BLOCKS) narrow_phase_kernel(const __grid_constant__ NarrowArgs<S> a, int capsules) { narrow_pair<S, false>(a, capsules); }
 template <class S>
-__global__ void __launch_bounds__(128) narrow_capsule_kernel(const __grid_constant__ NarrowArgs<S> a) { narrow_pair<S, true>(a, 1); }
+__global__ void __launch_bounds__(NARROW_THREADS, NARROW_MIN_BLOCKS) narrow_capsule_kernel(const __grid_constant__ NarrowArgs<S> a) { narrow_pair<S, true>(a, 1); }
 template <class S, bool CAPSULES>
-__global__ void __launch_bounds__(128) narrow_framed_kernel(const __grid_constant__ NarrowArgs<S> a, const BodyFrameCols<S> f, int capsules) {
+__global__ void __launch_bounds__(NARROW_THREADS, NARROW_MIN_BLOCKS) narrow_framed_kernel(const __grid_constant__ NarrowArgs<S> a, const BodyFrameCols<S> f, int capsules) {
     narrow_pair<S, CAPSULES, true>(a, capsules, f);
 }
 
@@ -128,12 +130,21 @@
         AVN_CUDA(cudaMemsetAsync(a.anchor2, 0, 12 * n * sizeof(S), stream_));
         AVN_CUDA(cudaMemsetAsync(a.penetration, 0, 4 * n * sizeof(S), stream_));
         AVN_CUDA(cudaMemsetAsync(a.normal_speed, 0, 4 * n * sizeof(S), stream_));
+        const unsigned nb = unsigned((n + NARROW_THREADS - 1) / NARROW_THREADS);
         if (frames) {
-            narrow_framed_kernel<S, false><<<unsigned((n + 127) / 128), 128, 0, stream_>>>(a, f, capsules ? 1 : 0);
-            if (capsules) narrow_framed_kernel<S, true><<<unsigned((n + 127) / 128), 128, 0, stream_>>>(a, f, 1);
+            AVN_CUDA(narrow_tile_attributes(narrow_framed_kernel<S, false>));
+            narrow_framed_kernel<S, false><<<nb, NARROW_THREADS, NARROW_TILE_BYTES, stream_>>>(a, f, capsules ? 1 : 0);
+            if (capsules) {
+                AVN_CUDA(narrow_tile_attributes(narrow_framed_kernel<S, true>));
+                narrow_framed_kernel<S, true><<<nb, NARROW_THREADS, NARROW_TILE_BYTES, stream_>>>(a, f, 1);
+            }
         } else {
-            narrow_phase_kernel<S><<<unsigned((n + 127) / 128), 128, 0, stream_>>>(a, capsules ? 1 : 0);
-            if (capsules) narrow_capsule_kernel<S><<<unsigned((n + 127) / 128), 128, 0, stream_>>>(a);
+            AVN_CUDA(narrow_tile_attributes(narrow_phase_kernel<S>));
+            narrow_phase_kernel<S><<<nb, NARROW_THREADS, NARROW_TILE_BYTES, stream_>>>(a, capsules ? 1 : 0);
+            if (capsules) {
+                AVN_CUDA(narrow_tile_attributes(narrow_capsule_kernel<S>));
+                narrow_capsule_kernel<S><<<nb, NARROW_THREADS, NARROW_TILE_BYTES, stream_>>>(a);
+            }
         }
         AVN_CUDA(cudaGetLastError());
         AVN_CUDA(cudaMemcpyAsync(out->point_count, a.count, n, cudaMemcpyDeviceToHost, stream_));
diff --git a/avian_b200/csrc/narrow_math.hpp b/avian_b200/csrc/narrow_math.hpp
--- a/avian_b200/csrc/narrow_math.hpp
+++ b/avian_b200/csrc/narrow_math.hpp
@@ -3,12 +3,16 @@
 
 #if defined(__CUDACC__)
 #define NM_HD __host__ __device__
-#define NM_COLD __host__ __device__ __noinline__
+#define NM_COLD __host__ __device__ __attribute__((always_inline))
+#define NM_NOINLINE __host__ __device__ __noinline__
 #define NM_ROLLED _Pragma("unroll 1")
+#define NM_UNROLLED _Pragma("unroll")
 #else
 #define NM_HD
 #define NM_COLD
+#define NM_NOINLINE
 #define NM_ROLLED
+#define NM_UNROLLED
 #endif
 
 namespace nm {
@@ -34,35 +38,66 @@
     return v * (q.w * q.w - b2) + b * (dot(v, b) * 2) + cross(b, v) * (q.w * 2);
 }
 struct M3 { V3 c[3]; };
+NM_HD inline V3 col(const M3& m, int i) { return i == 0 ? m.c[0] : (i == 1 ? m.c[1] : m.c[2]); }
 NM_HD inline M3 to_mat(Q q) { return {{rot(q, {1, 0, 0}), rot(q, {0, 1, 0}), rot(q, {0, 0, 1})}}; }
 
 enum ShapeType { SHAPE_CUBOID = 0, SHAPE_SPHERE = 1, SHAPE_CAPSULE = 2 };
 struct Box { V3 c; M3 r; V3 he; };
 
+struct Slots {
+    double* p;
+    int stride;
+    NM_HD double& operator[](int i) const { return p[i * stride]; }
+    NM_HD Slots at(int first) const { return {p + first * stride, stride}; }
+};
+NM_HD inline V3 vget(Slots s, int i) { return {s[3 * i], s[3 * i + 1], s[3 * i + 2]}; }
+NM_HD inline void vset(Slots s, int i, V3 v) { s[3 * i] = v.x; s[3 * i + 1] = v.y; s[3 * i + 2] = v.z; }
+NM_HD inline V3 vget(const V3* p, int i) { return p[i]; }
+NM_HD inline void vset(V3* p, int i, V3 v) { p[i] = v; }
+
 constexpr int MAX_RAW_POINTS = 8;
-struct Witness { V3 a, b; };
+constexpr int CLIP_MAX = 8;
+constexpr int WITNESS_SLOTS = 6 * MAX_RAW_POINTS;
+constexpr int SCRATCH_SLOTS = WITNESS_SLOTS + 3 * CLIP_MAX;
 struct Contacts {
     int n;
-    Witness p[MAX_RAW_POINTS];
+    Slots s;
+    NM_HD explicit Contacts(Slots scratch) : n(0), s(scratch) {}
+    NM_HD V3 a(int i) const { return {s[6 * i], s[6 * i + 1], s[6 * i + 2]}; }
+    NM_HD V3 b(int i) const { return {s[6 * i + 3], s[6 * i + 4], s[6 * i + 5]}; }
+    NM_HD void set(int i, V3 on_a, V3 on_b) {
+        s[6 * i] = on_a.x; s[6 * i + 1] = on_a.y; s[6 * i + 2] = on_a.z;
+        s[6 * i + 3] = on_b.x; s[6 * i + 4] = on_b.y; s[6 * i + 5] = on_b.z;
+    }
     NM_HD void clear() { n = 0; }
-    NM_HD void push(V3 on_a, V3 on_b) { p[n].a = on_a; p[n].b = on_b; ++n; }
+    NM_HD void push(V3 on_a, V3 on_b) { set(n, on_a, on_b); ++n; }
+    NM_HD Slots clip_poly() const { return s.at(WITNESS_SLOTS); }
+    NM_HD Slots clip_tmp() const { return s; }
 };
-
-NM_HD inline void box_face(const Box& b, int axis, S sign, V3 out[4]) {
+struct LocalContacts : Contacts {
+    double buf[SCRATCH_SLOTS];
+    NM_HD LocalContacts() : Contacts(Slots{buf, 1}) {}
+    LocalContacts(const LocalContacts&) = delete;
+    LocalContacts& operator=(const LocalContacts&) = delete;
+};
+
+template <class Out>
+NM_HD inline void box_face(const Box& b, int axis, S sign, Out out) {
     int u = (axis + 1) % 3, v = (axis + 2) % 3;
-    V3 n = b.r.c[axis] * (sign * comp(b.he, axis));
-    V3 eu = b.r.c[u] * comp(b.he, u), ev = b.r.c[v] * comp(b.he, v);
+    V3 n = col(b.r, axis) * (sign * comp(b.he, axis));
+    V3 eu = col(b.r, u) * comp(b.he, u), ev = col(b.r, v) * comp(b.he, v);
     V3 fc = b.c + n;
-    out[0] = fc + eu + ev; out[1] = fc - eu + ev; out[2] = fc - eu - ev; out[3] = fc + eu - ev;
-}
-
-NM_HD inline int clip_poly(const V3* in, int n, V3 plane_n, S plane_d, V3* out) {
+    vset(out, 0, fc + eu + ev); vset(out, 1, fc - eu + ev); vset(out, 2, fc - eu - ev); vset(out, 3, fc + eu - ev);
+}
+
+template <class In, class Out>
+NM_HD inline int clip_poly(In in, int n, V3 plane_n, S plane_d, Out out) {
     int m = 0;
     for (int i = 0; i < n; ++i) {
-        V3 a = in[i], b = in[(i + 1) % n];
+        V3 a = vget(in, i), b = vget(in, i + 1 == n ? 0 : i + 1);
         S da = dot(plane_n, a) - plane_d, db = dot(plane_n, b) - plane_d;
-        if (da <= 0) out[m++] = a;
-        if ((da < 0 && db > 0) || (da > 0 && db < 0)) out[m++] = a + (b - a) * (da / (da - db));
+        if (da <= 0 && m < CLIP_MAX) vset(out, m++, a);
+        if (((da < 0 && db > 0) || (da > 0 && db < 0)) && m < CLIP_MAX) vset(out, m++, a + (b - a) * (da / (da - db)));
     }
     return m;
 }
@@ -90,7 +125,7 @@
 NM_HD inline S box_point_closest(const Box& b, V3 p, V3& on) {
     V3 d = p - b.c;
     on = b.c;
-    for (int k = 0; k < 3; ++k) on = on + b.r.c[k] * smax(-comp(b.he, k), smin(comp(b.he, k), dot(d, b.r.c[k])));
+    for (int k = 0; k < 3; ++k) on = on + col(b.r, k) * smax(-comp(b.he, k), smin(comp(b.he, k), dot(d, col(b.r, k))));
     V3 e = p - on;
     return dot(e, e);
 }
@@ -99,8 +134,8 @@
     S best = 1e300;
 NM_ROLLED
     for (int side = 0; side < 2; ++side) {
-        const Box& P = side == 0 ? A : B;
-        const Box& O = side == 0 ? B : A;
+        const Box P = side == 0 ? A : B;
+        const Box O = side == 0 ? B : A;
 NM_ROLLED
         for (int m = 0; m < 8; ++m) {
             V3 v = P.c + P.r.c[0] * (m & 1 ? P.he.x : -P.he.x) + P.r.c[1] * (m & 2 ? P.he.y : -P.he.y) + P.r.c[2] * (m & 4 ? P.he.z : -P.he.z);
@@ -111,7 +146,7 @@
     }
     auto edge_mid = [](const Box& b, int k, int m) {
         int u = (k + 1) % 3, v = (k + 2) % 3;
-        return b.c + b.r.c[u] * (m & 1 ? comp(b.he, u) : -comp(b.he, u)) + b.r.c[v] * (m & 2 ? comp(b.he, v) : -comp(b.he, v));
+        return b.c + col(b.r, u) * (m & 1 ? comp(b.he, u) : -comp(b.he, u)) + col(b.r, v) * (m & 2 ? comp(b.he, v) : -comp(b.he, v));
     };
 NM_ROLLED
     for (int ei = 0; ei < 12; ++ei) {
@@ -122,8 +157,8 @@
             const int j = ej >> 2, mj = ej & 3;
             V3 pb = edge_mid(B, j, mj);
             S s, t;
-            segment_closest(pa, A.r.c[i], comp(A.he, i), pb, B.r.c[j], comp(B.he, j), s, t);
-            V3 qa = pa + A.r.c[i] * s, qb = pb + B.r.c[j] * t, e = qb - qa;
+            segment_closest(pa, col(A.r, i), comp(A.he, i), pb, col(B.r, j), comp(B.he, j), s, t);
+            V3 qa = pa + col(A.r, i) * s, qb = pb + col(B.r, j) * t, e = qb - qa;
             S d2 = dot(e, e);
             if (d2 < best) { best = d2; on_a = qa; on_b = qb; }
         }
@@ -155,102 +190,101 @@
         S sep = dot(n, d) - box_radius(A, n) - box_radius(B, n);
         if (sep - bias > best_sep + 1e-9) { best_sep = sep - bias; best_kind = kind; best_i = i; best_j = j; best_n = n; }
     };
-    for (int i = 0; i < 3; ++i) consider(A.r.c[i], 0, i, 0, 0);
-    for (int i = 0; i < 3; ++i) consider(B.r.c[i], 1, i, 0, 0);
+    for (int i = 0; i < 3; ++i) consider(col(A.r, i), 0, i, 0, 0);
+    for (int i = 0; i < 3; ++i) consider(col(B.r, i), 1, i, 0, 0);
     const S face_sep = best_sep;
     const int face_kind = best_kind, face_i = best_i;
     const V3 face_n = best_n;
     for (int i = 0; i < 3; ++i)
-        for (int j = 0; j < 3; ++j) consider(cross(A.r.c[i], B.r.c[j]), 2, i, j, 1e-4);
+        for (int j = 0; j < 3; ++j) consider(cross(col(A.r, i), col(B.r, j)), 2, i, j, 1e-4);
     S sep = best_kind == 2 ? best_sep + 1e-4 : best_sep;
     if (sep > max_dist) return false;
     normal = best_n;
+    bool edge_end = false;
+    S nearest = 1e300;
     if (best_kind == 2) {
-        V3 ea = A.r.c[best_i], eb = B.r.c[best_j];
+        V3 ea = col(A.r, best_i), eb = col(B.r, best_j);
         V3 pa = A.c, pb = B.c;
         for (int k = 0; k < 3; ++k) {
-            if (k != best_i) pa = pa + A.r.c[k] * (comp(A.he, k) * (dot(A.r.c[k], normal) > 0 ? 1 : -1));
-            if (k != best_j) pb = pb + B.r.c[k] * (comp(B.he, k) * (dot(B.r.c[k], normal) < 0 ? 1 : -1));
+            if (k != best_i) pa = pa + col(A.r, k) * (comp(A.he, k) * (dot(col(A.r, k), normal) > 0 ? 1 : -1));
+            if (k != best_j) pb = pb + col(B.r, k) * (comp(B.he, k) * (dot(col(B.r, k), normal) < 0 ? 1 : -1));
         }
         S s, t;
         if (!segment_closest(pa, ea, comp(A.he, best_i), pb, eb, comp(B.he, best_j), s, t)) {
             pts.push(pa + ea * s, pb + eb * t);
             return true;
         }
-        if (sep > 0) {
-            V3 on_a, on_b;
-            S dist = box_box_closest(A, B, on_a, on_b);
-            return closest_pair(on_a, on_b, dist, max_dist, normal, pts);
-        }
-        sep = face_sep; best_kind = face_kind; best_i = face_i; normal = face_n;
-    }
-    const bool ref_is_a = best_kind == 0;
-    const Box& R = ref_is_a ? A : B;
-    const Box& I = ref_is_a ? B : A;
-    V3 rn = ref_is_a ? normal : -normal;
-    int inc_axis = 0;
-    S inc_best = -1;
-    for (int k = 0; k < 3; ++k) {
-        S v = fabs(dot(I.r.c[k], rn));
-        if (v > inc_best) { inc_best = v; inc_axis = k; }
-    }
-    S isign = dot(I.r.c[inc_axis], rn) > 0 ? -1 : 1;
-    V3 poly[16], tmp[16];
-    box_face(I, inc_axis, isign, poly);
-    int np = 4;
-    int u = (best_i + 1) % 3, v = (best_i + 2) % 3;
-    const int axes[2] = {u, v};
-    for (int a = 0; a < 2 && np > 0; ++a) {
-        V3 sn = R.r.c[axes[a]];
-        S he = comp(R.he, axes[a]);
-        np = clip_poly(poly, np, sn, dot(sn, R.c) + he, tmp);
-        np = clip_poly(tmp, np, -sn, -dot(sn, R.c) + he, poly);
-    }
-    S face_d = dot(rn, R.c) + comp(R.he, best_i) * 1.0;
-    S nearest = 1e300;
-    for (int k = 0; k < np; ++k) {
-        S dist = dot(rn, poly[k]) - face_d;
-        if (dist > max_dist) continue;
-        nearest = smin(nearest, dist);
-        V3 on_ref = poly[k] - rn * dist;
-        bool dup = false;
-        for (int q = 0; q < pts.n; ++q) {
-            V3 e = (ref_is_a ? pts.p[q].b : pts.p[q].a) - poly[k];
-            if (dot(e, e) < 1e-12) { dup = true; break; }
-        }
-        if (dup) continue;
-        if (pts.n == MAX_RAW_POINTS) break;
-        if (ref_is_a) pts.push(on_ref, poly[k]); else pts.push(poly[k], on_ref);
-    }
-    if (sep > 0 && nearest > sep + FACE_GAP_SLACK) {
-        V3 on_a, on_b;
-        S dist = box_box_closest(A, B, on_a, on_b);
-        if (nearest > dist + FACE_GAP_SLACK) return closest_pair(on_a, on_b, dist, max_dist, normal, pts);
-    }
+        if (sep > 0) edge_end = true;
+        else { sep = face_sep; best_kind = face_kind; best_i = face_i; normal = face_n; }
+    }
+    if (!edge_end) {
+        const bool ref_is_a = best_kind == 0;
+        const Box R = ref_is_a ? A : B;
+        const Box I = ref_is_a ? B : A;
+        V3 rn = ref_is_a ? normal : -normal;
+        int inc_axis = 0;
+        S inc_best = -1;
+        for (int k = 0; k < 3; ++k) {
+            S v = fabs(dot(col(I.r, k), rn));
+            if (v > inc_best) { inc_best = v; inc_axis = k; }
+        }
+        S isign = dot(col(I.r, inc_axis), rn) > 0 ? -1 : 1;
+        const Slots poly = pts.clip_poly(), tmp = pts.clip_tmp();
+        box_face(I, inc_axis, isign, poly);
+        int np = 4;
+        int u = (best_i + 1) % 3, v = (best_i + 2) % 3;
+        for (int a = 0; a < 2 && np > 0; ++a) {
+            const int ax = a == 0 ? u : v;
+            V3 sn = col(R.r, ax);
+            S he = comp(R.he, ax);
+            np = clip_poly(poly, np, sn, dot(sn, R.c) + he, tmp);
+            np = clip_poly(tmp, np, -sn, -dot(sn, R.c) + he, poly);
+        }
+        S face_d = dot(rn, R.c) + comp(R.he, best_i) * 1.0;
+        for (int k = 0; k < np; ++k) {
+            const V3 pk = vget(poly, k);
+            S dist = dot(rn, pk) - face_d;
+            if (dist > max_dist) continue;
+            nearest = smin(nearest, dist);
+            V3 on_ref = pk - rn * dist;
+            bool dup = false;
+            for (int q = 0; q < pts.n; ++q) {
+                V3 e = (ref_is_a ? pts.b(q) : pts.a(q)) - pk;
+                if (dot(e, e) < 1e-12) { dup = true; break; }
+            }
+            if (dup) continue;
+            if (pts.n == MAX_RAW_POINTS) break;
+            if (ref_is_a) pts.push(on_ref, pk); else pts.push(pk, on_ref);
+        }
+        if (!(sep > 0 && nearest > sep + FACE_GAP_SLACK)) return pts.n != 0;
+    }
+    V3 on_a, on_b;
+    S dist = box_box_closest(A, B, on_a, on_b);
+    if (edge_end || nearest > dist + FACE_GAP_SLACK) return closest_pair(on_a, on_b, dist, max_dist, normal, pts);
     return pts.n != 0;
 }
 
 NM_HD inline void prune4(Contacts& pts, V3 n) {
     if (pts.n <= 4) return;
-    auto depth = [&](int i) { return dot(pts.p[i].a - pts.p[i].b, n); };
+    auto depth = [&](int i) { return dot(pts.a(i) - pts.b(i), n); };
     int p0 = 0;
     for (int i = 1; i < pts.n; ++i) if (depth(i) > depth(p0) + 1e-12) p0 = i;
     int p1 = p0;
     S best = -1;
-    for (int i = 0; i < pts.n; ++i) { V3 e = pts.p[i].a - pts.p[p0].a; S v = dot(e, e); if (v > best) { best = v; p1 = i; } }
-    V3 dir = cross(pts.p[p1].a - pts.p[p0].a, n);
+    const V3 a0 = pts.a(p0);
+    for (int i = 0; i < pts.n; ++i) { V3 e = pts.a(i) - a0; S v = dot(e, e); if (v > best) { best = v; p1 = i; } }
+    V3 dir = cross(pts.a(p1) - a0, n);
     int p2 = p0, p3 = p0;
     S mx = 0, mn = 0;
     for (int i = 0; i < pts.n; ++i) {
-        S v = dot(pts.p[i].a - pts.p[p0].a, dir);
+        S v = dot(pts.a(i) - a0, dir);
         if (v > mx) { mx = v; p2 = i; }
         if (v < mn) { mn = v; p3 = i; }
     }
-    bool keep[MAX_RAW_POINTS] = {false, false, false, false, false, false, false, false};
-    keep[p0] = keep[p1] = keep[p2] = keep[p3] = true;
+    const unsigned keep = (1u << p0) | (1u << p1) | (1u << p2) | (1u << p3);
     int m = 0;
     for (int i = 0; i < pts.n; ++i)
-        if (keep[i]) pts.p[m++] = pts.p[i];
+        if (keep >> i & 1u) { pts.set(m, pts.a(i), pts.b(i)); ++m; }
     pts.n = m;
 }
 
@@ -280,7 +314,7 @@
         int ax = 0; S best = 1e300;
         for (int k = 0; k < 3; ++k) { S v = comp(A.he, k) - fabs(comp(local, k)); if (v < best) { best = v; ax = k; } }
         S sgn = comp(local, ax) >= 0 ? 1 : -1;
-        normal = A.r.c[ax] * sgn;
+        normal = col(A.r, ax) * sgn;
         on_box = cs + normal * best;
     }
     pts.push(on_box, cs - normal * rs);
@@ -345,10 +379,10 @@
 NM_ROLLED
     for (int ei = 0; ei < 12; ++ei) {
         const int k = ei >> 2, m = ei & 3, u = (k + 1) % 3, v = (k + 2) % 3;
-        const V3 e = b.c + b.r.c[u] * (m & 1 ? comp(b.he, u) : -comp(b.he, u)) + b.r.c[v] * (m & 2 ? comp(b.he, v) : -comp(b.he, v));
+        const V3 e = b.c + col(b.r, u) * (m & 1 ? comp(b.he, u) : -comp(b.he, u)) + col(b.r, v) * (m & 2 ? comp(b.he, v) : -comp(b.he, v));
         S s, t;
-        segment_closest(C.c, C.u, C.h, e, b.r.c[k], comp(b.he, k), s, t);
-        const V3 qs = C.c + C.u * s, qe = e + b.r.c[k] * t, d = qs - qe;
+        segment_closest(C.c, C.u, C.h, e, col(b.r, k), comp(b.he, k), s, t);
+        const V3 qs = C.c + C.u * s, qe = e + col(b.r, k) * t, d = qs - qe;
         const S d2 = dot(d, d);
         if (d2 < best) { best = d2; on_seg = qs; on_box = qe; }
     }
@@ -360,7 +394,7 @@
 NM_ROLLED
     for (int i = 1; i < 3; ++i) {
         const int j = (k + i) % 3;
-        const S a = dot(b.r.c[j], C.c - b.c), g = dot(b.r.c[j], C.u), he = comp(b.he, j);
+        const S a = dot(col(b.r, j), C.c - b.c), g = dot(col(b.r, j), C.u), he = comp(b.he, j);
         if (fabs(g) < 1e-12) {
             if (fabs(a) > he) return false;
             continue;
@@ -380,7 +414,7 @@
     V3 best_n{0, 1, 0}, face_n{0, 1, 0};
 NM_ROLLED
     for (int i = 0; i < 6; ++i) {
-        V3 n = i < 3 ? b.r.c[i] : cross(b.r.c[i - 3], C.u);
+        V3 n = i < 3 ? col(b.r, i) : cross(col(b.r, i - 3), C.u);
         const S l = len(n);
         if (l < CAPSULE_EDGE_AXIS_MIN) continue;
         n = n * (1 / l);
@@ -399,23 +433,23 @@
         normal = (on_seg - on_box) * (1 / dist);
 NM_ROLLED
         for (int k = 0; k < 3; ++k)
-            if (fabs(dot(normal, b.r.c[k])) >= 1 - 0.5 * CAPSULE_PARALLEL_SIN * CAPSULE_PARALLEL_SIN) fk = k;
-        if (fk < 0 || fabs(dot(C.u, b.r.c[fk])) > CAPSULE_PARALLEL_SIN) {
+            if (fabs(dot(normal, col(b.r, k))) >= 1 - 0.5 * CAPSULE_PARALLEL_SIN * CAPSULE_PARALLEL_SIN) fk = k;
+        if (fk < 0 || fabs(dot(C.u, col(b.r, fk))) > CAPSULE_PARALLEL_SIN) {
             pts.push(on_box, on_seg - normal * C.r);
             return true;
         }
-        normal = b.r.c[fk] * (dot(normal, b.r.c[fk]) < 0 ? -1 : 1);
+        normal = col(b.r, fk) * (dot(normal, col(b.r, fk)) < 0 ? -1 : 1);
     } else {
         if (best_edge) {
             const V3 n = best_n;
             V3 e = b.c;
 NM_ROLLED
             for (int j = 0; j < 3; ++j)
-                if (j != best_k) e = e + b.r.c[j] * (comp(b.he, j) * (dot(b.r.c[j], n) > 0 ? 1 : -1));
+                if (j != best_k) e = e + col(b.r, j) * (comp(b.he, j) * (dot(col(b.r, j), n) > 0 ? 1 : -1));
             S s, t;
-            if (!segment_closest(C.c, C.u, C.h, e, b.r.c[best_k], comp(b.he, best_k), s, t)) {
+            if (!segment_closest(C.c, C.u, C.h, e, col(b.r, best_k), comp(b.he, best_k), s, t)) {
                 normal = n;
-                pts.push(e + b.r.c[best_k] * t, C.c + C.u * s - n * C.r);
+                pts.push(e + col(b.r, best_k) * t, C.c + C.u * s - n * C.r);
                 return true;
             }
         }
@@ -459,7 +493,7 @@
     if (flip) {
         normal = -normal;
 NM_ROLLED
-        for (int k = 0; k < pts.n; ++k) { V3 t = pts.p[k].a; pts.p[k].a = pts.p[k].b; pts.p[k].b = t; }
+        for (int k = 0; k < pts.n; ++k) pts.set(k, pts.b(k), pts.a(k));
     }
     return normal;
 }
@@ -486,7 +520,7 @@
         hit = box_sphere(B, pa, he_a.x, max_dist, normal, pts);
         if (hit) {
             normal = -normal;
-            for (int k = 0; k < pts.n; ++k) { V3 t = pts.p[k].a; pts.p[k].a = pts.p[k].b; pts.p[k].b = t; }
+            for (int k = 0; k < pts.n; ++k) pts.set(k, pts.b(k), pts.a(k));
         }
     }
     return hit;
@@ -500,20 +534,25 @@
 NM_HD inline int manifold_points_in(const Contacts& pts, V3 normal, V3 pa, V3 pb, V3 rel, V3 w1, V3 w2, S dt, S eff_margin, const PairFrames* fr,
                                     PointOut out[4]) {
     int m = 0;
-    for (int k = 0; k < pts.n && m < 4; ++k) {
+NM_UNROLLED
+    for (int k = 0; k < MAX_RAW_POINTS; ++k) {
+        if (k >= pts.n || m >= 4) break;
         PointOut pt;
-        pt.anchor1 = pts.p[k].a;
-        pt.anchor2 = pts.p[k].b - (pb - pa);
+        pt.anchor1 = pts.a(k);
+        pt.anchor2 = pts.b(k) - (pb - pa);
         if (FRAMES) {
             pt.anchor1 = (pt.anchor1 + fr->offset1) - fr->com1;
             pt.anchor2 = (pt.anchor2 + fr->offset2) - fr->com2;
         }
-        pt.penetration = dot(pts.p[k].a - pts.p[k].b, normal);
+        pt.penetration = dot(pts.a(k) - pts.b(k), normal);
         V3 rv = rel + cross(w2, pt.anchor2) - cross(w1, pt.anchor1);
         pt.normal_speed = dot(rv, normal);
         bool keep = -pt.penetration < eff_margin || (pt.normal_speed * dt - pt.penetration < eff_margin);
         if (!keep) continue;
-        out[m++] = pt;
+NM_UNROLLED
+        for (int j = 0; j < 4; ++j)
+            if (j == m) out[j] = pt;
+        ++m;
     }
     return m;
 }
@@ -525,8 +564,11 @@
     return manifold_points_in<true>(pts, normal, pa, pb, rel, w1, w2, dt, eff_margin, &fr, out);
 }
 
+template <int MAX_OLD>
 NM_HD inline int match_point(V3 anchor1, V3 anchor2, const V3* old_anchor1, const V3* old_anchor2, int n_old, S thr2) {
-    for (int k = 0; k < n_old; ++k) {
+NM_UNROLLED
+    for (int k = 0; k < MAX_OLD; ++k) {
+        if (k >= n_old) break;
         V3 e11 = anchor1 - old_anchor1[k], e22 = anchor2 - old_anchor2[k], e12 = anchor1 - old_anchor2[k], e21 = anchor2 - old_anchor1[k];
         if ((dot(e11, e11) < thr2 && dot(e22, e22) < thr2) || (dot(e12, e12) < thr2 && dot(e21, e21) < thr2)) return k;
     }
diff --git a/avian_b200/host/host_api.cpp b/avian_b200/host/host_api.cpp
--- a/avian_b200/host/host_api.cpp
+++ b/avian_b200/host/host_api.cpp
@@ -148,9 +148,10 @@
     a.lv = static_cast<const T*>(lv); a.av = static_cast<const T*>(av); a.amin = static_cast<const T*>(amin); a.amax = static_cast<const T*>(amax);
     a.dt = dt; a.tol = tol; a.thr2 = (0.1 * length_unit) * (0.1 * length_unit); a.match = match ? 1 : 0;
     const avn::BodyFrameCols<T> f{static_cast<const T*>(body_pos), static_cast<const T*>(body_rot), static_cast<const T*>(body_com)};
+    nm::LocalContacts pts;
     for (uint32_t e = 0; e < E; ++e) {
-        if (body_pos) avn::narrow_edge_row<T, true, true>(a, int(e), f);
-        else avn::narrow_edge_row<T>(a, int(e));
+        if (body_pos) avn::narrow_edge_row<T, true, true>(a, int(e), pts, f);
+        else avn::narrow_edge_row<T>(a, int(e), pts);
     }
 }
 
@@ -442,7 +443,7 @@
     std::vector<uint32_t> changed;
     std::vector<uint8_t> disjoint(P.pairs.size(), 0), started(P.pairs.size(), 0), stopped(P.pairs.size(), 0);
     std::vector<int> count_change(P.pairs.size(), 0);
-    Contacts pts;
+    LocalContacts pts;
     for (uint32_t id : P.active) {
         Pair& pr = P.pairs[id];
         if (pr.asleep) continue;
@@ -491,7 +492,7 @@
                     const int n_old = int(std::min<size_t>(om.pts.size(), 8));
                     for (int k = 0; k < n_old; ++k) { oa1[k] = om.pts[k].anchor1; oa2[k] = om.pts[k].anchor2; }
                     for (Point& c : m.pts) {
-                        const int k = match_point(c.anchor1, c.anchor2, oa1, oa2, n_old, thr2);
+                        const int k = match_point<8>(c.anchor1, c.anchor2, oa1, oa2, n_old, thr2);
                         if (k >= 0) { c.ws_normal = om.pts[k].ws_normal; c.ws_tx = om.pts[k].ws_tx; c.ws_ty = om.pts[k].ws_ty; }
                     }
                 }
@@ -577,7 +578,7 @@
         S eff_margin = dt * len(rel);
         S max_dist = smax(eff_margin, tol);
         V3 nrm;
-        Contacts pts;
+        LocalContacts pts;
         int ta = shape ? shape[a] : SHAPE_CUBOID, tb = shape ? shape[b] : SHAPE_CUBOID;
         if (!collide(ta, dm.v3(a), pa, rt.q(a), tb, dm.v3(b), pb, rt.q(b), max_dist, nrm, pts)) continue;
         PointOut out[4];
@@ -649,7 +650,7 @@
             if (k < nc) {
                 const V3 a1{new_a1[(size_t(i) * 4 + k) * 3], new_a1[(size_t(i) * 4 + k) * 3 + 1], new_a1[(size_t(i) * 4 + k) * 3 + 2]};
                 const V3 a2{new_a2[(size_t(i) * 4 + k) * 3], new_a2[(size_t(i) * 4 + k) * 3 + 1], new_a2[(size_t(i) * 4 + k) * 3 + 2]};
-                const int j = match_contacts ? match_point(a1, a2, oa1, oa2, oc, thr2) : -1;
+                const int j = match_contacts ? match_point<4>(a1, a2, oa1, oa2, oc, thr2) : -1;
                 if (j >= 0) { vn = on[j]; vx = otx[j]; vy = oty[j]; }
                 for (int c = 0; c < 3; ++c) { prev_a1[(e * 4 + k) * 3 + c] = comp(a1, c); prev_a2[(e * 4 + k) * 3 + c] = comp(a2, c); }
             }
```

New measurement: 449.1 (median of 6 runs). 1.02x the previous value.
